# antonburger/FuncTracer

Hardware: AMD Instinct MI355X
Metric: Mrays/s (primary+shadow+reflect) at 1920x1080x16spp; frame ms (higher is better)
Workload: dtype f64

## Files before the change

functracer_amd/__init__.py:

```python
import ctypes as C
import os

import numpy as np

from . import _capi
from ._capi import (CIRCLE, CONE, CUBE, CYLINDER, EXCLUDE, INTERSECT, PLANE, SOLID_CYLINDER, SPHERE, SQUARE, SUBTRACT, UNION,
                    FtError, SceneBuilder, make_camera)

__all__ = ["Context", "PinnedArray", "ParsedScene", "parse_scene", "parse_scene_file", "jitter_pattern", "quantise_rgba8", "write_png",
           "parse_colour", "parse_ply", "FtError", "make_camera", "HIP_LIB", "HOST_LIB", "DEFAULT_SEED"]

HIP_LIB = os.environ.get("FT_HIP_LIB") or os.path.join(_capi.LIB_DIR, "libfunctracer_hip.so")
HOST_LIB = os.environ.get("FT_HOST_LIB") or os.path.join(_capi.LIB_DIR, "libfunctracer_host.so")
DEFAULT_SEED = 20260104
MAX_DEPTH = 8

_hip = None
_host = None


def hip_lib():
    global _hip
    if _hip is None:
        lib = _capi.load_library(HIP_LIB)
# ... 534 lines not shown
                                               _capi.dptr(t), _capi.dptr(p), _capi.dptr(nr), _capi.dptr(col)))
        return hit, t, p, nr, col

    def blocked(self, origins, dirs, max_dist):
        o = _capi.as_f64(origins).reshape(-1, 3)
        d = _capi.as_f64(dirs).reshape(-1, 3)
        m = _capi.as_f64(max_dist).reshape(-1)
        out = np.zeros(o.shape[0], dtype=np.int32)
        self._check(self._lib.ft_debug_blocked(self._ctx, _capi.dptr(o), _capi.dptr(d), _capi.dptr(m), o.shape[0], out.ctypes.data_as(_capi.c_int32_p)))
        return out

    def colour_for_ray(self, origins, dirs, max_depth=MAX_DEPTH):
        o = _capi.as_f64(origins).reshape(-1, 3)
        d = _capi.as_f64(dirs).reshape(-1, 3)
        rgb = np.zeros((o.shape[0], 3))
        self._check(self._lib.ft_debug_colour(self._ctx, _capi.dptr(o), _capi.dptr(d), o.shape[0], max_depth, _capi.dptr(rgb)))
        return rgb

    def devices(self):
        out = (C.c_int32 * 64)()
        n = self._check(self._lib.ft_debug_devices(self._ctx, out, 64))
        return list(out[:n])

    def commit_times(self):
        ms = np.zeros(4)
        self._check(self._lib.ft_get_commit_times(self._ctx, _capi.dptr(ms)))
        return {"flatten_ms": float(ms[0]), "device_bvh_ms": float(ms[1]), "upload_ms": float(ms[2]), "device_bvh_height": int(ms[3])}

    def mesh_trees(self):
        sizes = (C.c_int64 * 12)()
        self._check(self._lib.ft_debug_mesh_trees(self._ctx, sizes, *([None] * 9)))
        n = list(sizes)
        out = {"nodes": np.zeros(n[0], dtype=_capi.BSP_NODE_DTYPE), "bsp_leaves": np.zeros((n[1], 2), dtype=np.uint32), "tris": np.zeros((n[2], 9)),
               "tri_orig": np.zeros(n[3], dtype=np.uint32), "tri_src": np.zeros(n[4], dtype=np.uint32), "wide": np.zeros((n[5], 28)),
               "coarse_boxes": np.zeros((n[6], 6), dtype=np.float32), "meshes": np.zeros((n[7], 6), dtype=np.int32)}
        jobs = np.zeros((n[8], 9), dtype=np.uint32)
        order = ["nodes", "bsp_leaves", "tris", "tri_orig", "tri_src", "wide", "coarse_boxes", "meshes"]
        self._check(self._lib.ft_debug_mesh_trees(self._ctx, sizes, *[out[k].ctypes.data for k in order], jobs.ctypes.data))
        out["jobs"] = [dict(zip(_capi.BVH_JOB_FIELDS, (int(v) for v in row))) for row in jobs]
        out["stack_capacity"], out["from_device"] = int(sizes[9]), bool(sizes[10])
        return out

    def block_lists(self):
        sizes = (C.c_int64 * 4)()
        plane = np.zeros(4)
        fn = self._lib.ft_debug_block_lists
        fn.argtypes = [C.c_void_p, C.POINTER(C.c_int64), C.c_void_p, C.c_void_p, C.c_void_p, C.c_void_p]
        self._check(fn(self._ctx, sizes, None, None, None, None))
        heads, pos_block = np.zeros(sizes[0], dtype=np.uint32), np.zeros(sizes[0], dtype=np.uint32)
        entries = np.zeros(sizes[1], dtype=_capi.LIST_ENTRY_DTYPE)
        self._check(fn(self._ctx, sizes, plane.ctypes.data, heads.ctypes.data, pos_block.ctypes.data, entries.ctypes.data))
        return {"leaf": int(sizes[2]), "heads": heads, "pos_block": pos_block, "entries": entries, "plane": plane, "capacity": int(sizes[3])}

    def classify_reuse(self):
        out = (C.c_int64 * 4)()
        self._check(self._lib.ft_debug_classify_reuse(self._ctx, out))
        return dict(zip(_capi.CLASSIFY_REUSE_FIELDS, (int(v) for v in out)))

    def primary_kernels(self):
        out = (C.c_int64 * 2)()
        self._check(self._lib.ft_debug_primary_kernels(self._ctx, out))
        return {"k_primary": int(out[0]), "k_primary_mesh": int(out[1])}

    def scene_info(self):
        out = (C.c_int64 * 12)()
        self._check(self._lib.ft_debug_scene_info(self._ctx, out))
        keys = ["leaves", "program_words", "meshes", "bsp_nodes", "bsp_leaves", "triangles", "csg_capacity", "stack_capacity", "items", "bounded_items",
                "unbounded", "face_directions"]
        return dict(zip(keys, list(out)))


def rays_handled_by(kernel, st):
    generated = st["rays_primary"] - st["rays_primary_culled"]
    if kernel == "primary":
        return generated + st["rays_shadow_primary"]
    return st["rays_reflect"] + st["rays_shadow"] - st["rays_shadow_primary"]


def debug_slice(p0, n, tri):
    above, below = np.zeros(18), np.zeros(18)
    na, nb = C.c_int32(), C.c_int32()
    tri = _capi.as_f64(tri, (9,))
    rc = hip_lib().ft_debug_slice(_capi.dptr(_capi.as_f64(p0)), _capi.dptr(_capi.as_f64(n)), _capi.dptr(tri), _capi.dptr(above), C.byref(na),
                                  _capi.dptr(below), C.byref(nb))
    if rc < 0:
        raise FtError(rc, "slice")
    return above[:9 * na.value].reshape(-1, 3, 3), below[:9 * nb.value].reshape(-1, 3, 3)
```

functracer_amd/_capi.py:

```python
import ctypes as C
import os

import numpy as np

_HERE = os.path.dirname(os.path.abspath(__file__))
LIB_DIR = os.path.join(_HERE, "lib")

FT_OK = 0
STATUS_NAMES = {0: "FT_OK", -1: "FT_ERR_INVALID", -2: "FT_ERR_NO_DEVICE", -3: "FT_ERR_HIP", -4: "FT_ERR_UNSUPPORTED",
                -5: "FT_ERR_STATE", -6: "FT_ERR_OVERFLOW", -7: "FT_ERR_BUILD"}

CIRCLE, SQUARE, CUBE, SPHERE, PLANE, CONE, SOLID_CYLINDER, CYLINDER = range(8)
UNION, INTERSECT, SUBTRACT, EXCLUDE = range(4)
TRANSLATE, SCALE, ROTATE = range(3)

c_double_p = C.POINTER(C.c_double)
c_int32_p = C.POINTER(C.c_int32)


class FtError(RuntimeError):
    def __init__(self, status, message=""):
        self.status = status
        super().__init__(f"{STATUS_NAMES.get(status, status)}: {message}")

# ... 80 lines not shown
    ("ft_sg_set_transform", C.c_int32, [C.c_void_p, C.c_int32, C.POINTER(ft_transform), C.c_int32]),
    ("ft_scene_commit_moved", C.c_int32, [C.c_void_p]),
    ("ft_debug_leaf_matrices", C.c_int32, [C.c_void_p, C.POINTER(C.c_int64), c_double_p, c_double_p]),
]


DEFORM_SIGNATURES = [
    ("ft_sg_set_mesh_triangles", C.c_int32, [C.c_void_p, C.c_int32, c_double_p, C.c_int64]),
    ("ft_scene_commit_deformed", C.c_int32, [C.c_void_p]),
    ("ft_scene_tree_quality", C.c_int32, [C.c_void_p, C.c_int32, c_double_p]),
]


LIGHT_SIGNATURES = [
    ("ft_scene_set_directional", C.c_int32, [C.c_void_p, C.c_int32, c_double_p, c_double_p]),
    ("ft_scene_set_soft_directional", C.c_int32, [C.c_void_p, C.c_int32, c_double_p, C.c_double, c_double_p]),
    ("ft_scene_set_positional", C.c_int32, [C.c_void_p, C.c_int32, c_double_p, c_double_p, c_double_p]),
    ("ft_scene_commit_lights", C.c_int32, [C.c_void_p]),
]


MESH_TREES_SIGNATURE = [C.c_void_p, C.POINTER(C.c_int64)] + [C.c_void_p] * 9
BSP_NODE_DTYPE = np.dtype([("bmin", np.float64, 3), ("bmax", np.float64, 3), ("left", np.int32), ("right", np.int32), ("axis", np.uint32), ("pad", np.uint32)])
BVH_JOB_FIELDS = ["mesh", "first_global", "n", "node_base", "leaf_base", "tri_base", "wide_base", "coarse_first", "coarse_count"]


class ft_temporal_filter_params(C.Structure):
    _fields_ = [("iterations", C.c_int32), ("demodulate", C.c_int32), ("min_history", C.c_int32), ("to_frame", C.c_int32),
                ("sigma_colour", C.c_double), ("sigma_normal", C.c_double), ("sigma_position", C.c_double),
                ("albedo_floor", C.c_double), ("variance_floor", C.c_double)]


TEMPORAL_FILTER_DEFAULTS = dict(iterations=4, demodulate=1, min_history=4, to_frame=0, sigma_colour=2.0, sigma_normal=0.3, sigma_position=0.0,
                                albedo_floor=1e-3, variance_floor=1e-6)

TEMPORAL_FILTER_SIGNATURE = [C.c_void_p, C.POINTER(ft_camera), C.c_int32, c_double_p, C.c_int32, C.c_uint64, C.POINTER(ft_temporal_filter_params),
                             C.c_int32, C.c_void_p, c_double_p, C.POINTER(ft_stats)]

TEMPORAL_QUEUE_DEPTH = 4
TEMPORAL_QUEUE_SIGNATURES = [
    ("ft_temporal_enqueue", C.c_int32, [C.c_void_p, C.POINTER(ft_camera), C.c_int32, c_double_p, C.c_int32, C.c_uint64, C.POINTER(ft_temporal_params),
                                        C.POINTER(ft_temporal_filter_params), C.c_int32, C.c_void_p]),
    ("ft_temporal_wait", C.c_int32, [C.c_void_p, C.POINTER(ft_stats)]),
]


AOV_CHANNELS = [("t", np.float64, 1, np.inf), ("p", np.float64, 3, 0.0), ("n", np.float64, 3, 0.0), ("colour", np.float64, 3, 0.0),
                ("material", np.float64, 3, 0.0), ("leaf", np.int32, 1, -1), ("node", np.int32, 1, -1), ("triangle", np.int32, 1, -1)]


CLASSIFY_REUSE_FIELDS = ("classified", "reused", "windows_launched", "windows_skipped")
LIST_ENTRY_DTYPE = np.dtype([("tri", np.uint32), ("orig", np.uint32), ("x0", np.float32), ("x1", np.float32), ("y0", np.float32), ("y1", np.float32)])
LIST_NONE = 0xFFFFFFFF


class fth_options(C.Structure):
    _fields_ = [("camera", ft_camera), ("res_h", C.c_int32), ("res_v", C.c_int32), ("samples", C.c_int32), ("corner", C.c_int32)]


BUILDER_SIGNATURES = [
    ("sg_primitive", C.c_int32, [C.c_void_p, C.c_int32]),
    ("sg_triangle", C.c_int32, [C.c_void_p, c_double_p]),
    ("sg_bsp_mesh", C.c_int32, [C.c_void_p, C.c_int32, c_double_p, C.c_int64]),
    ("sg_transform", C.c_int32, [C.c_void_p, C.POINTER(ft_transform), C.c_int32, C.c_int32]),
    ("sg_material", C.c_int32, [C.c_void_p, C.POINTER(ft_material), C.c_int32]),
    ("sg_hue_shift", C.c_int32, [C.c_void_p, C.c_double, C.c_int32]),
    ("sg_ignore_light", C.c_int32, [C.c_void_p, C.c_int32]),
    ("sg_group", C.c_int32, [C.c_void_p, c_int32_p, C.c_int32]),
    ("sg_csg", C.c_int32, [C.c_void_p, C.c_int32, C.c_int32, C.c_int32]),
    ("sg_texture_grid", C.c_int32, [C.c_void_p, c_double_p, c_double_p, c_double_p, C.c_int32, C.c_int32]),
    ("sg_texture_image", C.c_int32, [C.c_void_p, C.POINTER(C.c_uint8), C.c_int32, C.c_int32, c_double_p, C.c_int32, C.c_int32]),
    ("scene_clear", C.c_int32, [C.c_void_p]),
    ("scene_set_objects", C.c_int32, [C.c_void_p, C.c_int32]),
    ("scene_add_directional", C.c_int32, [C.c_void_p, c_double_p, c_double_p]),
    ("scene_add_soft_directional", C.c_int32, [C.c_void_p, c_double_p, C.c_int32, C.c_double, c_double_p]),
    ("scene_add_positional", C.c_int32, [C.c_void_p, c_double_p, c_double_p, c_double_p]),
    ("scene_commit", C.c_int32, [C.c_void_p]),
]


PROGRESSIVE_SIGNATURES = [
    ("ft_progressive_begin", C.c_int32, [C.c_void_p, C.POINTER(ft_camera), C.c_int32, C.c_int32, C.c_int32, C.POINTER(ft_rect), C.c_int32,
                                         C.c_double, C.c_int32]),
    ("ft_progressive_pass", C.c_int32, [C.c_void_p, C.c_int32, c_double_p, C.c_uint64, C.c_int32, C.c_void_p, C.POINTER(ft_stats)]),
    ("ft_progressive_fetch", C.c_int32, [C.c_void_p, c_double_p, c_double_p, C.POINTER(C.c_uint32)]),
    ("ft_progressive_status", C.c_int32, [C.c_void_p, C.POINTER(C.c_int64)]),
    ("ft_progressive_end", C.c_int32, [C.c_void_p]),
]


class fth_builder(C.Structure):
    _fields_ = [(name, C.CFUNCTYPE(res, *args)) for name, res, args in BUILDER_SIGNATURES]


def dptr(a):
    return a.ctypes.data_as(c_double_p)


def as_f64(a, shape=None):
    a = np.ascontiguousarray(a, dtype=np.float64)
    if shape is not None:
        a = a.reshape(shape)
    return a


def vec3(v):
# ... 155 lines not shown
```

functracer_amd/csrc/ft_capi.cpp:

```cpp
#include "ft_context.h"
#include "ft_refit_cost.h"

namespace ftc {

bool need_device(ft_context* c) {
    if (!c) return false;
    if (c->host_only) { c->err = "host-only context: no HIP device bound (there is no CPU fallback for rendering)"; return false; }
    return true;
}

bool need_committed(ft_context* c) {
    if (!c->committed) c->err = "scene not committed (ft_scene_commit)";
    return c->committed;
}

static void norm3(double v[3]) {
    double l = std::sqrt(v[0] * v[0] + v[1] * v[1] + v[2] * v[2]);
    if (!(l < 0.0000001)) { double s = 1.0 / l; v[0] = s * v[0]; v[1] = s * v[1]; v[2] = s * v[2]; }
}
ftk::Camera make_camera(const ft_camera& cam, int res_h, int res_v) {
    ftk::Camera out{};
    double k[3] = {cam.look_at[0] - cam.o[0], cam.look_at[1] - cam.o[1], cam.look_at[2] - cam.o[2]};
    norm3(k);
    const double* u = cam.up;
// ... 98 lines not shown
    if (!c) return;
    for (DeviceWorker* w : c->workers) { w->stop(); delete w; }
    c->workers.clear();
    for (ft_context* p : c->peers) ft_destroy(p);
    c->peers.clear();
    if (!c->host_only) {
        (void)hipSetDevice(c->device);
        (void)drain_frame_streams(c);
        if (c->side) (void)hipStreamSynchronize(c->side);
        for (DeviceBuf& b : c->d_scene) b.release();
        for (DeviceBuf& b : c->d_rays) b.release();
        for (DeviceBuf& b : c->d_acc) b.release();
        for (DeviceBuf* b : {&c->d_out, &c->d_out8, &c->d_out_index, &c->d_pixels, &c->d_jitter, &c->d_wave_counts, &c->d_dbg_in, &c->d_dbg_out}) b->release();
        for (auto& f : c->slots) f.release();
        c->prog.release(); c->aov.release(); c->denoise.release(); c->temporal.release(); c->refit.release(); c->lightspace.release();
        if (c->classified) (void)hipEventDestroy(c->classified);
        for (hipEvent_t& e : c->acc_free) if (e) { (void)hipEventDestroy(e); e = nullptr; }
        if (c->side) (void)hipStreamDestroy(c->side);
        if (c->tail) (void)hipStreamDestroy(c->tail);
        for (hipStream_t m : c->more_mains) if (m) (void)hipStreamDestroy(m);
        if (c->stream) (void)hipStreamDestroy(c->stream);
    }
    delete c;
}

const char* ft_last_error(const ft_context* c) { return c ? c->err.c_str() : "null context"; }

enum { kFlag = 1, kPowerOfTwo = 2, kCommit = 4, kLevelHint = 8, kZeroFill = 16, kOrZero = 32, kClassified = 64 };
struct OptionSpec {
    const char* key;
    int64_t lo, hi;
    int64_t Options::* field;
    void (*to_graph)(fth::SceneGraph&, int64_t);
    int rules;
};
constexpr int64_t kNoLimit = std::numeric_limits<int64_t>::max();
const OptionSpec kOptions[] = {
    {"chunk_samples", 64, kNoLimit, &Options::chunk_samples, nullptr, 0},
    {"wave_samples", 0, 16, &Options::wave_samples, nullptr, kPowerOfTwo},
    {"coherent_waves", 0, 1, &Options::coherent_waves, nullptr, kFlag},
    {"timing", 0, 2, &Options::timing, nullptr, 0},
    {"classify_pixels", 0, 1, &Options::classify_pixels, nullptr, kFlag | kClassified},
    {"follow_below", -1, kNoLimit, &Options::follow_below, nullptr, kLevelHint},
    {"level_hint", 0, 1, &Options::level_hint, nullptr, kFlag},
    {"classify_ahead", 0, 1, &Options::classify_ahead, nullptr, kFlag},
    {"resolve_aside", 0, 1, &Options::resolve_aside, nullptr, kFlag},
    {"zero_fill_skip", 0, 1, &Options::zero_fill_skip, nullptr, kFlag | kZeroFill},
    {"classify_reuse", 0, 1, &Options::classify_reuse, nullptr, kFlag | kClassified},
    {"mains", 1, ft_context::kMains, &Options::mains, nullptr, 0},
    {"bvh_builder", 0, 3, &Options::bvh_builder, nullptr, kCommit},
    {"csg_auto_grow", 0, 1, &Options::csg_auto_grow, nullptr, kFlag},
    {"primary_block_lists", 0, 1, &Options::primary_block_lists, nullptr, kFlag | kClassified},
    {"uniform_surface", 0, 1, &Options::uniform_surface, nullptr, kFlag},
    {"primary_mesh_kernel", 0, 1, &Options::primary_mesh_kernel, nullptr, kFlag},
    {"temporal_follow_deformed", 0, 1, &Options::temporal_follow_deformed, nullptr, kFlag},
    {"refit_rebuild_percent", 100, 1000000, &Options::refit_rebuild_percent, nullptr, kOrZero},
    {"csg_mesh_capacity", 1, 255, nullptr, [](fth::SceneGraph& g, int64_t v) { g.csg_mesh_capacity = (int32_t)v; }, kCommit},
    {"light_space_shadows", std::numeric_limits<int64_t>::min(), kNoLimit, nullptr,
     [](fth::SceneGraph& g, int64_t v) { g.light_space_shadows = v == 0 || v == 1 ? (int32_t)v : 2; }, kCommit},
    {"mesh_unclipped_bvh", 0, 1, nullptr, [](fth::SceneGraph& g, int64_t v) { g.mesh_unclipped_bvh = v != 0; }, kFlag | kCommit},
};

int32_t ft_set_option(ft_context* c, const char* key, int64_t value) {
    if (!c || !key) return FT_ERR_INVALID;
    for (const OptionSpec& o : kOptions) {
        if (std::strcmp(key, o.key)) continue;
        if (o.rules & kFlag) value = value != 0;
        else if (!((o.rules & kOrZero) && value == 0) && (value < o.lo || value > o.hi || ((o.rules & kPowerOfTwo) && (value & (value - 1))))) return FT_ERR_INVALID;
        if (o.to_graph) { o.to_graph(c->graph, value); c->committed = false; c->options_pending = true; return FT_OK; }
        for (ft_context* d : devices(c)) {
            d->opt.*o.field = value;
            for (hipStream_t m : d->more_mains) if (!m) d->opt.mains = 1;
            d->dev_scene.coherent_waves = d->opt.coherent_waves ? 1 : 0;
            d->dev_scene.uniform_surface = d->opt.uniform_surface ? 1 : 0;
            if (!d->opt.temporal_follow_deformed) temporal_drop_snapshots(d);
            if (o.rules & kCommit) { d->committed = false; c->options_pending = true; }
            if (o.rules & kLevelHint) d->staged_hint = -1;
            if (o.rules & kZeroFill) d->zero_signature[0] = d->zero_signature[1] = 0;
            if (o.rules & kClassified) for (auto& F : d->slots) { F.kept.valid = false; F.keeps = false; }
        }
        return FT_OK;
    }
    c->err = std::string("unknown option: ") + key;
    return FT_ERR_INVALID;
}

static ft_node add_node(ft_context* c, fth::GraphNode&& n) { c->graph.nodes.push_back(std::move(n)); c->committed = false; c->restructured = true; return (ft_node)c->graph.nodes.size() - 1; }

ft_node ft_sg_primitive(ft_context* c, int32_t kind) {
    if (!c || kind < 0 || kind > FT_PRIM_CYLINDER) return FT_ERR_INVALID;
    fth::GraphNode n; n.kind = fth::GraphNode::Prim; n.prim = kind; return add_node(c, std::move(n));
}
ft_node ft_sg_triangle(ft_context* c, const double v[9]) {
    if (!c || !v) return FT_ERR_INVALID;
    fth::GraphNode n; n.kind = fth::GraphNode::TriangleP; std::memcpy(n.tri, v, sizeof n.tri); return add_node(c, std::move(n));
}
ft_node ft_sg_bsp_mesh(ft_context* c, int32_t depth, const double* tris, int64_t n_tris) {
    if (!c || n_tris < 0 || (n_tris > 0 && !tris) || depth < 0) return FT_ERR_INVALID;
    fth::GraphNode n; n.kind = fth::GraphNode::Mesh; n.depth = depth; n.tris.assign(tris, tris + 9 * n_tris); return add_node(c, std::move(n));
}
ft_node ft_sg_transform(ft_context* c, const ft_transform* ts, int32_t n_ts, ft_node child) {
    if (!c || !c->graph.valid(child) || !ts || n_ts < 1) return FT_ERR_INVALID;
    fth::GraphNode n; n.kind = fth::GraphNode::Transform;
    for (int i = 0; i < n_ts; ++i) { if (ts[i].kind < FT_TRANSLATE || ts[i].kind > FT_ROTATE) return FT_ERR_INVALID; n.xf.push_back(ts[i]); }
    n.children = {child};
    return add_node(c, std::move(n));
}
int32_t ft_sg_set_transform(ft_context* c, ft_node node, const ft_transform* ts, int32_t n_ts) {
    if (!c) return FT_ERR_INVALID;
    if (!c->graph.valid(node) || c->graph.nodes[node].kind != fth::GraphNode::Transform) { c->err = "ft_sg_set_transform: not a transform node"; return FT_ERR_INVALID; }
    if (!ts || n_ts < 1) { c->err = "ft_sg_set_transform: no transforms"; return FT_ERR_INVALID; }
    for (int i = 0; i < n_ts; ++i) if (ts[i].kind < FT_TRANSLATE || ts[i].kind > FT_ROTATE) { c->err = "ft_sg_set_transform: bad transform kind"; return FT_ERR_INVALID; }
    c->graph.nodes[node].xf.assign(ts, ts + n_ts);
    c->committed = false; c->moved_pending = true;
    return FT_OK;
}
int32_t ft_sg_set_mesh_triangles(ft_context* c, ft_node node, const double* tris, int64_t n_tris) {
    if (!c) return FT_ERR_INVALID;
    if (!c->graph.valid(node) || c->graph.nodes[node].kind != fth::GraphNode::Mesh) { c->err = "ft_sg_set_mesh_triangles: not a bspMesh node"; return FT_ERR_INVALID; }
    if (!tris) { c->err = "ft_sg_set_mesh_triangles: no triangles"; return FT_ERR_INVALID; }
    fth::GraphNode& n = c->graph.nodes[node];
    if (n_tris < 0 || (uint64_t)n_tris != n.tris.size() / 9) { c->err = "ft_sg_set_mesh_triangles: the triangle count differs from the node's"; return FT_ERR_INVALID; }
    n.tris.assign(tris, tris + 9 * n_tris);
    n.deformed = true;
    c->committed = false;
    return FT_OK;
}
// ... 116 lines not shown
        float lf = (float)len; while ((double)lf < len) lf = std::nextafter(lf, std::numeric_limits<float>::infinity());
        v.push_back((float)f.cull_rows[k]); v.push_back((float)f.cull_rows[k + 1]); v.push_back((float)f.cull_rows[k + 2]); v.push_back(lf);
    }
}

static ftk::LbvhTarget lbvh_target(ft_context* c, const fth::FlatScene::BvhJob& j) {
    const DeviceBuf* B = c->d_scene;
    return ftk::LbvhTarget{B[kTris].as<double>(), j.first_global, j.n, B[kNodes].as<ftd::BspNode>(), j.node_base, B[kBspLeaves].as<ftd::BspLeaf>(), j.leaf_base,
                           B[kTriOrig].as<uint32_t>(), j.tri_base, B[kWide].as<double>(), j.wide_base, B[kCoarse].as<float>() + 6 * (size_t)j.coarse_first, j.coarse_count,
                           B[kTriSrc].as<uint32_t>()};
}

static int32_t fit_stacks(ft_context* c, uint32_t height) {
    if ((int32_t)height + 1 > c->flat.stack_capacity) c->flat.stack_capacity = (int32_t)height + 1;
    return lds_fits(c);
}

static bool mesh_kernel_scene(const fth::FlatScene& f, int variant) {
    if (variant != 4 || f.item_pc.size() != 2 || f.leaves.size() != 1 || f.any_reflective) return false;
    size_t pc = f.item_pc[0] & 0x7FFFFFFFu;
    if (pc < f.program.size() && (f.program[pc] & 0xFFu) == ftd::OP_CULL) pc += 2;
    if (pc + 1 >= f.program.size() || f.program[pc] != (uint32_t)ftd::OP_LEAF_FOLD || (f.program[pc + 1] & 0xFFu) != ftd::OP_END) return false;
    const ftd::Leaf& L = f.leaves[0];
    if (L.kind != ftd::LK_MESH || !(L.flags & ftd::LF_LIT) || L.mesh >= f.meshes.size() || f.meshes[L.mesh].bvh_root < 0) return false;
    for (auto& l : f.lights) if (l.kind != ftd::LT_DIRECTIONAL) return false;
    for (auto& m : f.materials) if (m.reflectance > 0.0) return false;
    return true;
}

static void derive_launch_shape(ft_context* c) {
    const fth::FlatScene& f = c->flat;
    ftk::DevScene& S = c->dev_scene;
    S.coherent_waves = c->opt.coherent_waves ? 1 : 0;
    S.uniform_surface = c->opt.uniform_surface ? 1 : 0;
    S.n_simd = c->n_cu * 4;
    S.n_items = (int32_t)f.item_pc.size() - 1; S.n_cull_rows = f.cull_bundle ? (int32_t)(f.cull_rows.size() / 3) : -1;
    S.n_leaves = (int32_t)f.leaves.size(); S.n_lights = (int32_t)f.lights.size();
    S.csg_cap = f.csg_capacity; S.stack_cap = f.stack_capacity;
    S.lane_fold = lane_fold_for(f); S.csg_rows = (f.csg_capacity + S.lane_fold - 1) / S.lane_fold;
    S.shadow_rays_per_hit = 0;
    for (auto& l : f.lights) S.shadow_rays_per_hit += (l.kind == ftd::LT_SOFT) ? l.samples : 1;
    c->variant = 0;
    for (auto& m : f.materials) if (needs_fancy(m)) c->variant |= 1;
    for (auto& l : f.lights) if (l.kind == ftd::LT_SOFT) c->variant |= 2;
    if (!f.meshes.empty()) c->variant |= 4;
    const size_t lds = lds_bytes_for(c->flat);
    c->variant_primary = c->variant;
    c->blocks_primary = ftk::occupancy_blocks_primary(lds, &c->variant_primary);
    c->blocks_bounce = ftk::occupancy_blocks_bounce(lds, c->variant);
    c->blocks_resolve = ftk::occupancy_blocks_resolve();
    c->blocks_aov = ftk::occupancy_blocks_aov(lds, c->variant);
    c->mesh_kernel_scene = mesh_kernel_scene(f, c->variant);
    c->blocks_primary_mesh = ftk::occupancy_blocks_primary_mesh();
}

static int32_t upload_scene(ft_context* c) {
    int32_t rc;
    FT_HIP(c, hipSetDevice(c->device));
    if (any_queued(c)) { if ((rc = retire_queued(c)) != FT_OK) return rc; c->accum_open = false; }
    const fth::FlatScene& f = c->flat;
    if ((rc = lds_fits(c)) != FT_OK) return rc;
    c->refit.ready = false;
    c->lightspace.reset();
    ftk::DevScene& S = c->dev_scene;
    rc = FT_OK;
    auto put = [&](SceneArray k, const auto& v, auto*& ptr) {
        if (rc == FT_OK) rc = upload(c, c->d_scene[k], v);
        ptr = static_cast<std::remove_reference_t<decltype(ptr)>>(c->d_scene[k].p);
    };
    put(kLeaves, f.leaves, S.leaves); put(kM2w, f.m2w, S.m2w); put(kMaterials, f.materials, S.materials); put(kLights, f.lights, S.lights);
    put(kTextures, f.textures, S.textures); put(kTexPixels, f.tex_pixels, S.tex_pixels); put(kProgram, f.program, S.program);
    put(kMeshes, f.meshes, S.meshes); put(kNodes, f.nodes, S.nodes); put(kBspLeaves, f.bsp_leaves, S.bsp_leaves); put(kTris, f.tris, S.tris);
    put(kCulls, f.culls, S.culls);
    cull_items_image(f, c->cull_items_and_rows);
    put(kCullItems, c->cull_items_and_rows, S.cull_items);
    put(kCullRows, f.cull_rows, S.cull_rows); put(kItemPc, f.item_pc, S.item_pc); put(kWide, f.wide, S.wide); put(kMeshWide, f.mesh_wide, S.mesh_wide);
    put(kCoarse, f.coarse_boxes, S.coarse_boxes); put(kTriOrig, f.tri_orig, S.tri_orig);
    put(kLsPairs, f.ls_pairs, S.ls_pairs); put(kLsNodes, f.ls_nodes, S.ls_nodes); put(kLsTris, f.ls_tris, S.ls_tris);
    if (rc == FT_OK) rc = upload(c, c->d_scene[kTriSrc], f.tri_src);
    if (rc == FT_OK) rc = upload(c, c->d_scene[kRunNodes], f.run_nodes);
    if (rc != FT_OK) return rc;
    for (auto& F : c->slots) { if ((rc = ensure(c, F.d_fc, sizeof(ftk::SlotCounters))) != FT_OK) return rc; F.fc_clean = false; }
    c->zero_signature[0] = c->zero_signature[1] = 0;
    FT_HIP(c, hipStreamSynchronize(c->stream));
    {
        const auto t0 = std::chrono::steady_clock::now();
        uint32_t tallest = 0;
        for (const fth::FlatScene::BvhJob& j : f.bvh_jobs) {
            uint32_t height = 0;
            FT_HIP(c, ftk::build_lbvh(c->stream, lbvh_target(c, j), &height, c->opt.bvh_builder == 1 ? 0 : 1));
            if (height == 0 || height > 40) { c->err = "device BVH build refused (non-finite vertex or a tree deeper than 40 levels): the host builder takes over"; return FT_ERR_BUILD; }
            tallest = std::max(tallest, height);
        }
        if (!f.bvh_jobs.empty()) {
            c->commit_ms[1] = std::chrono::duration<double, std::milli>(std::chrono::steady_clock::now() - t0).count();
            c->commit_ms[3] = tallest;
            if ((rc = fit_stacks(c, tallest)) != FT_OK) return rc;
        }
    }
    derive_launch_shape(c);
    c->committed = true;
    ++c->commit_serial; c->staged_hint = -1;
    return FT_OK;
}

int32_t commit_scene(ft_context* c) {
    using clock = std::chrono::steady_clock;
    auto ms_since = [](clock::time_point t0) { return std::chrono::duration<double, std::milli>(clock::now() - t0).count(); };
    for (double& v : c->commit_ms) v = 0.0;
    const bool held = c->holds_commit;
    const auto done = [c](int32_t rc) {
        if (rc == FT_OK) { c->holds_commit = true; c->restructured = false; c->moved_pending = false; c->options_pending = false; c->lights_pending = false; for (fth::GraphNode& n : c->graph.nodes) n.deformed = false; }
        return rc;
    };
    for (int attempt = 0; attempt < 2; ++attempt) {
        c->graph.device_bvh = !c->host_only && c->opt.bvh_builder >= 1 && attempt == 0;
        c->graph.device_bvh_min_tris = c->opt.bvh_builder == 2 ? kDeviceBvhMinTris : 0;
        auto t0 = clock::now();
        fth::FlatScene fresh;
        int32_t rc = c->graph.flatten(fresh, c->err);
        if (rc == FT_OK && !c->host_only && lane_fold_for(fresh) == 0) { rc = FT_ERR_UNSUPPORTED; c->err = kLdsRefusal; }
        c->commit_ms[0] += ms_since(t0);
        if (rc != FT_OK) {
            if (attempt == 0 && held) for (ft_context* d : devices(c)) d->committed = true;
            return rc;
        }
        c->holds_commit = false;
        c->tree_quality.clear();
        c->flat = std::move(fresh);
        if (c->host_only) { c->committed = true; return done(FT_OK); }
        t0 = clock::now();
        rc = upload_scene(c);
        for (ft_context* p : c->peers) {
            if (rc != FT_OK) break;
            p->flat = c->flat;
            if ((rc = upload_scene(p)) != FT_OK) c->err = p->err;
            c->commit_ms[1] += p->commit_ms[1];
        }
        c->commit_ms[2] += ms_since(t0) - c->commit_ms[1];
        if (rc == FT_ERR_BUILD && c->graph.device_bvh) continue;
        return done(rc);
    }
    return FT_ERR_BUILD;
}

struct DeformedMesh { uint32_t mesh; int32_t node; fth::MeshScan scan; };

using ftk::refit::refit_ranges;

static bool refittable(const fth::FlatScene& f, uint32_t mesh) { return f.meshes[mesh].root < 0 && f.meshes[mesh].bvh_root != INT32_MIN; }
static const fth::FlatScene::BvhJob* job_of(const fth::FlatScene& f, uint32_t mesh) {
    for (const fth::FlatScene::BvhJob& j : f.bvh_jobs) if (j.mesh == mesh) return &j;
// ... 330 lines not shown
        for (const LightJob& j : jobs) {
            if (!j.grid) continue;
            const size_t own = 4 * (size_t)j.nu * j.nv + 5 * (size_t)j.entries;
            words = std::max(words, (size_t)j.at + (own + ftd::kLsNodeWords - 1) / ftd::kLsNodeWords * ftd::kLsNodeWords);
            doubles = std::max(doubles, 9 * ((size_t)j.tri_at + j.entries));
        }
        if (words == T.base_node_words && doubles == T.base_tri_doubles && words == L.node_words && doubles == L.tri_doubles) regrid = false;
    }
    if (regrid) {
        DeviceBuf nodes, tris;
        if ((rc = ensure(c, nodes, words * 4)) != FT_OK || (rc = ensure(c, tris, doubles * 8)) != FT_OK) { nodes.release(); tris.release(); return rc; }
        const auto fail = [&](int32_t code) { nodes.release(); tris.release(); return code; };
        if (hipMemcpyAsync(nodes.p, B[kLsNodes].p, T.base_node_words * 4, hipMemcpyDeviceToDevice, c->stream) != hipSuccess ||
            hipMemcpyAsync(tris.p, B[kLsTris].p, T.base_tri_doubles * 8, hipMemcpyDeviceToDevice, c->stream) != hipSuccess ||
            (words > T.base_node_words && hipMemsetAsync(nodes.as<uint32_t>() + T.base_node_words, 0, (words - T.base_node_words) * 4, c->stream) != hipSuccess) ||
            (doubles > T.base_tri_doubles && hipMemsetAsync(tris.as<double>() + T.base_tri_doubles, 0, (doubles - T.base_tri_doubles) * 8, c->stream) != hipSuccess)) {
            c->err = "ft_scene_commit_lights: copying the light-space arrays failed"; return fail(FT_ERR_HIP);
        }
        for (const LightJob& j : jobs) {
            if (!j.grid) continue;
            const uint32_t n = j.pair->n_tris, cells = j.nu * j.nv;
            const double* mesh = B[kTris].as<double>() + 9 * (size_t)j.pair->first_tri;
            size_t scan_bytes = 0;
            if (ftk::ls_grid_scan(c->stream, nullptr, nullptr, cells, nullptr, &scan_bytes) != hipSuccess) { c->err = "ft_scene_commit_lights: sizing the scan failed"; return fail(FT_ERR_HIP); }
            DeviceBuf& ebox = L.d_ebox[j.slot];
            DeviceBuf& counts = L.d_counts[j.slot];
            if ((rc = ensure(c, ebox, (size_t)n * 20)) != FT_OK || (rc = ensure(c, counts, (size_t)cells * 4)) != FT_OK || (rc = ensure(c, L.d_first, (size_t)cells * 4)) != FT_OK ||
                (rc = ensure(c, L.d_cursor, (size_t)cells * 4)) != FT_OK || (rc = ensure(c, L.d_idx, (size_t)j.entries * 4)) != FT_OK || (rc = ensure(c, L.d_scan, scan_bytes)) != FT_OK) return fail(rc);
            if (hipMemsetAsync(L.d_cursor.p, 0, (size_t)cells * 4, c->stream) != hipSuccess) { c->err = "ft_scene_commit_lights: hipMemsetAsync failed"; return fail(FT_ERR_HIP); }
            if (!lead) {
                if (hipMemsetAsync(counts.p, 0, (size_t)cells * 4, c->stream) != hipSuccess) { c->err = "ft_scene_commit_lights: hipMemsetAsync failed"; return fail(FT_ERR_HIP); }
                ftk::ls_grid_entries(c->stream, mesh, n, j.frame, ebox.as<float>(), nullptr);
                ftk::ls_grid_cell_counts(c->stream, ebox.as<float>(), n, j.s, j.nu, j.nv, counts.as<uint32_t>(), nullptr);
            }
            if (ftk::ls_grid_scan(c->stream, counts.as<uint32_t>(), L.d_first.as<uint32_t>(), cells, L.d_scan.p, &scan_bytes) != hipSuccess) { c->err = "ft_scene_commit_lights: the scan failed"; return fail(FT_ERR_HIP); }
            ftk::ls_grid_emit(c->stream, ebox.as<float>(), mesh, n, j.s, j.nu, j.nv, counts.as<uint32_t>(), L.d_first.as<uint32_t>(), L.d_cursor.as<uint32_t>(), L.d_idx.as<uint32_t>(),
                              j.entries, nodes.as<uint32_t>(), j.at, tris.as<double>(), j.tri_at);
        }
        if (hipGetLastError() != hipSuccess || hipStreamSynchronize(c->stream) != hipSuccess) { c->err = "ft_scene_commit_lights: the grid kernels failed"; return fail(FT_ERR_HIP); }
        B[kLsNodes].release(); B[kLsTris].release();
        B[kLsNodes] = nodes; B[kLsTris] = tris;
        ftk::DevScene& S = c->dev_scene;
        S.ls_nodes = static_cast<std::remove_reference_t<decltype(S.ls_nodes)>>(nodes.p);
        S.ls_tris = static_cast<std::remove_reference_t<decltype(S.ls_tris)>>(tris.p);
        L.node_words = words; L.tri_doubles = doubles;
        L.rewritten = true;
    }
    FT_HIP(c, hipStreamSynchronize(c->stream));
    ms[1] += since(t1);
    const auto t2 = clock::now();
    if ((rc = upload(c, B[kLsPairs], f.ls_pairs)) != FT_OK) return rc;
    FT_HIP(c, hipStreamSynchronize(c->stream));
    ms[0] += since(t2);
    c->zero_signature[0] = c->zero_signature[1] = 0;
    c->committed = true;
    ++c->commit_serial; c->staged_hint = -1;
    return FT_OK;
}

}

extern "C" {

int32_t ft_scene_commit(ft_context* c) {
    if (!c) return FT_ERR_INVALID;
    progressive_close(c);
    temporal_close(c);
    return commit_scene(c);
}

int32_t ft_scene_commit_moved(ft_context* c) {
    if (!c) return FT_ERR_INVALID;
    if (!c->holds_commit) { c->err = "ft_scene_commit_moved: no committed scene to move (ft_scene_commit)"; return FT_ERR_STATE; }
    if (c->restructured) { c->err = "ft_scene_commit_moved: the graph, the root or the lights changed since the commit (ft_scene_commit)"; return FT_ERR_STATE; }
    progressive_close(c);
    const int32_t rc = commit_scene(c);
    if (rc == FT_OK) ++c->pose_serial;
    return rc;
}

int32_t ft_scene_commit_deformed(ft_context* c) {
    if (!c) return FT_ERR_INVALID;
    if (!c->holds_commit) { c->err = "ft_scene_commit_deformed: no committed scene to deform (ft_scene_commit)"; return FT_ERR_STATE; }
    if (c->restructured) { c->err = "ft_scene_commit_deformed: the graph, the root or the lights changed since the commit (ft_scene_commit)"; return FT_ERR_STATE; }
    if (c->moved_pending) { c->err = "ft_scene_commit_deformed: an ft_sg_set_transform is pending (ft_scene_commit_moved first)"; return FT_ERR_STATE; }
    if (c->options_pending) { c->err = "ft_scene_commit_deformed: a commit-time option changed since the commit (ft_scene_commit)"; return FT_ERR_STATE; }
    if (c->lights_pending) { c->err = "ft_scene_commit_deformed: a light setter is pending (ft_scene_commit_lights first)"; return FT_ERR_STATE; }
    using clock = std::chrono::steady_clock;
    const auto t0 = clock::now();
    fth::FlatScene& f = c->flat;
    std::vector<DeformedMesh> edits;
    for (uint32_t m = 0; m < (uint32_t)f.meshes.size(); ++m) {
        const int32_t id = f.mesh_node[m];
        if (id < 0 || !c->graph.valid(id) || !c->graph.nodes[(size_t)id].deformed) continue;
        const fth::GraphNode& n = c->graph.nodes[(size_t)id];
        const bool refuse_depth = n.depth > 0 && !c->graph.mesh_unclipped_bvh;
        const fth::MeshScan scan = refuse_depth ? fth::MeshScan{} : fth::scan_mesh(n.tris.data(), (int64_t)(n.tris.size() / 9));
        if (refuse_depth || !scan.finite || f.meshes[m].root >= 0) {
            c->err = refuse_depth || f.meshes[m].root >= 0 ? "ft_scene_commit_deformed: an edited mesh has depth above 0 - its clipped BSP depends on the positions (ft_scene_commit)"
                                                            : "ft_scene_commit_deformed: an edited mesh holds a non-finite coordinate (ft_scene_commit)";
            c->committed = true;
            return FT_ERR_UNSUPPORTED;
        }
        edits.push_back(DeformedMesh{m, id, scan});
    }
    if (c->host_only) {
// ... 225 lines not shown
```

functracer_amd/csrc/ft_context.h:

```cpp
#pragma once
#include <hip/hip_runtime.h>

#include <chrono>
#include <condition_variable>
#include <mutex>
#include <cmath>
#include <cstddef>
#include <cstdio>
#include <cstring>
#include <functional>
#include <limits>
#include <string>
#include <thread>
#include <type_traits>
#include <vector>

#include "../../include/functracer_hip.h"
#include "ft_device.h"
#include "ft_scene.h"

struct DeviceBuf {
    void* p = nullptr; size_t bytes = 0;
    template <class T> T* as() const { return reinterpret_cast<T*>(p); }
    void release() { if (p) (void)hipFree(p); p = nullptr; bytes = 0; }
// ... 8 lines not shown
};

enum { kStageOther = 0, kStageClosest = 1, kStageShade = 2, kStageResolve = 3, kStagePrimary = 4, kStages = 5 };
static_assert(sizeof(ftk::FrameCounters) % 16 == 0 && offsetof(ftk::RenderCounters, ref_equiv) == 32, "the hand-over at the end of a frame copies words and clears 16 bytes at a time");

struct DeviceWorker {
    std::thread th;
    std::mutex m;
    std::condition_variable cv;
    std::function<void()> job;
    bool has_job = false, done = true, quit = false;
    void start() {
        th = std::thread([this] {
            std::unique_lock<std::mutex> lk(m);
            for (;;) {
                cv.wait(lk, [this] { return has_job || quit; });
                if (quit) return;
                std::function<void()> fn = std::move(job);
                has_job = false;
                lk.unlock();
                fn();
                lk.lock();
                done = true;
                cv.notify_all();
            }
        });
    }
    void post(std::function<void()> fn) { std::lock_guard<std::mutex> lk(m); job = std::move(fn); has_job = true; done = false; cv.notify_all(); }
    void wait() { std::unique_lock<std::mutex> lk(m); cv.wait(lk, [this] { return done; }); }
    void stop() { { std::lock_guard<std::mutex> lk(m); quit = true; cv.notify_all(); } if (th.joinable()) th.join(); }
};

constexpr int64_t kDeviceBvhMinTris = 4096;

struct Options {
    int64_t chunk_samples = 16ll << 20;
    int64_t wave_samples = 0;
    int64_t coherent_waves = 1;
    int64_t timing = 1;
    int64_t classify_pixels = 1;
    int64_t follow_below = -1;
    int64_t level_hint = 1;
    int64_t classify_ahead = 1;
    int64_t resolve_aside = 1;
    int64_t zero_fill_skip = 1;
    int64_t classify_reuse = 1;
    int64_t mains = 2;
    int64_t bvh_builder = 2;
    int64_t csg_auto_grow = 1;
    int64_t primary_block_lists = 1;
    int64_t refit_rebuild_percent = 0;
    int64_t temporal_follow_deformed = 0;
    int64_t primary_mesh_kernel = 1;
    int64_t uniform_surface = 1;
};

enum SceneArray { kLeaves, kM2w, kMaterials, kLights, kTextures, kTexPixels, kProgram, kMeshes, kNodes, kBspLeaves, kTris, kCulls, kCullItems,
                  kCullRows, kItemPc, kWide, kMeshWide, kCoarse, kTriOrig, kLsPairs, kLsNodes, kLsTris,
                  kTriSrc, kRunNodes,
                  kSceneArrays };

struct Brackets {
    std::vector<hipEvent_t> events; size_t used = 0;
    struct Span { hipEvent_t a, b; int kind; };
    std::vector<Span> spans;
    hipStream_t ms = nullptr;
    int timing = 1;
    hipEvent_t ev0 = nullptr, ev1 = nullptr;
    hipEvent_t boundary = nullptr;
    bool fresh = false;
    void begin(hipStream_t s, int t) { used = 0; spans.clear(); ms = s; timing = t; ev0 = ev1 = boundary = nullptr; fresh = false; }
    hipEvent_t next() {
        if (used == events.size()) { hipEvent_t e; if (hipEventCreate(&e) != hipSuccess) return nullptr; events.push_back(e); }
        return events[used++];
    }
    hipEvent_t record(hipStream_t s) { hipEvent_t e = next(); if (e) (void)hipEventRecord(e, s); return e; }
    void open() { if (ev0) return; ev0 = record(ms); boundary = ev0; fresh = true; }
    template <class Fn> void timed(int kind, Fn&& fn) {
        const bool bracket = timing >= 2 || (timing == 1 && (kind == kStageClosest || kind == kStageShade || kind == kStagePrimary));
        open();
        if (bracket && !fresh) boundary = record(ms);
        fn();
        if (!bracket) { fresh = false; return; }
        hipEvent_t b = record(ms);
        if (boundary && b) spans.push_back(Span{boundary, b, kind});
        boundary = b; fresh = true;
    }
    void release() { for (hipEvent_t e : events) (void)hipEventDestroy(e); events.clear(); used = 0; }
};

struct ClassifyKey {
    uint64_t commit_serial = 0;
    int32_t res_h = 0, res_v = 0, list_leaf = -1;
    double jitter_extent = 0.0;
    ftk::Camera cam{};
    std::vector<ft_rect> rects;
    bool operator==(const ClassifyKey& o) const {
        return commit_serial == o.commit_serial && res_h == o.res_h && res_v == o.res_v && list_leaf == o.list_leaf &&
               std::memcmp(&jitter_extent, &o.jitter_extent, sizeof jitter_extent) == 0 && std::memcmp(&cam, &o.cam, sizeof cam) == 0 &&
               rects.size() == o.rects.size() && (rects.empty() || std::memcmp(rects.data(), o.rects.data(), rects.size() * sizeof(ft_rect)) == 0);
    }
};

struct ft_context {
    static constexpr int kMains = 3;
    static constexpr int kAcc = kMains;
    static constexpr int kSlots = kMains + 1;
    std::vector<ft_context*> peers;
    std::vector<DeviceWorker*> workers;
    bool host_only = false;
    int device = -1;
    int n_cu = 0;
    hipStream_t stream = nullptr;
    hipStream_t more_mains[kMains - 1] = {};
    std::string err;
    Options opt;

    fth::SceneGraph graph;
    fth::FlatScene flat;
    std::vector<float> cull_items_and_rows;
    bool committed = false;
    bool holds_commit = false, restructured = false;
    bool moved_pending = false, options_pending = false;
    bool lights_pending = false;
    uint64_t pose_serial = 0;
    double commit_ms[4] = {0, 0, 0, 0};

    DeviceBuf d_scene[kSceneArrays];
    hipStream_t side = nullptr;
    int variant = 0, variant_primary = 0, blocks_primary = 1, blocks_bounce = 1, blocks_resolve = 2, blocks_aov = 1;
    bool mesh_kernel_scene = false;
    int blocks_primary_mesh = 1;
    hipEvent_t classified = nullptr;
    ftk::DevScene dev_scene{};
    DeviceBuf d_rays[2 * kMains], d_acc[kAcc], d_out, d_out8, d_out_index, d_pixels, d_jitter, d_wave_counts, d_dbg_in, d_dbg_out;
    struct Aov {
        DeviceBuf d_pixels, d_jitter, d_out, d_ctr;
        bool ctr_clean = false;
        TimedLaunch timer;
        void release() { for (DeviceBuf* b : {&d_pixels, &d_jitter, &d_out, &d_ctr}) b->release(); timer.release(); }
    } aov;
    struct Denoise {
        DeviceBuf d_guides, d_u[2], d_out8;
        TimedLaunch timer;
        void release() { for (DeviceBuf* b : {&d_guides, &d_u[0], &d_u[1], &d_out8}) b->release(); timer.release(); }
    } denoise;
    int acc_turn = 0;
    hipStream_t tail = nullptr;
    hipEvent_t acc_free[kAcc] = {};
    bool acc_busy[kAcc] = {};
    uint64_t zero_signature[2] = {0, 0};
    uint32_t classify_epoch = 0;
    int64_t ray_capacity = 0, acc_capacity = 0;
    struct FrameSlot {
        DeviceBuf d_block_pos, d_pos_block, d_fc;
        DeviceBuf d_list_heads, d_list_pool;
        int32_t list_leaf = -1;
        ftk::Camera list_cam{};
        struct Classified { bool valid = false; ClassifyKey key; int64_t n_active = 0; uint64_t culled = 0; } kept;
        bool keeps = false, reuses = false;
        bool fc_clean = false;
        Brackets ev;
        bool simple = false;
        int main_ix = 0;
        ftk::FrameReport* h_report = nullptr;
        ftk::FrameReport* d_report = nullptr;
        uint64_t signature = 0;
        bool pending = false;
        uint64_t rays_primary = 0; int64_t n_pix_total = 0; int32_t spp = 0, n_launches = 0, n_chunks = 0, format = 0; bool classify = false;
        std::chrono::steady_clock::time_point wall0;
        void release() {
            d_block_pos.release(); d_pos_block.release(); d_fc.release(); d_list_heads.release(); d_list_pool.release();
            if (h_report) (void)hipHostFree(h_report);
            h_report = nullptr; d_report = nullptr;
            ev.release();
        }
    };
    FrameSlot slots[kSlots];
    struct Refit {
        DeviceBuf d_verts, d_parent_node, d_parent_leaf, d_arrived, d_leaf_boxes, d_wide_node;
        DeviceBuf d_cost;
        bool ready = false;
        void release() { for (DeviceBuf* b : {&d_verts, &d_parent_node, &d_parent_leaf, &d_arrived, &d_leaf_boxes, &d_wide_node, &d_cost}) b->release(); ready = false; }
    } refit;
    struct LightSpace {
        struct Pair {
            uint32_t rec, leaf, light; int32_t root; double c[3], R; uint32_t first_tri, n_tris; double v0[3], rec0[ftd::kLsPairDoubles];
            std::vector<std::pair<uint32_t, uint32_t>> levels;
        };
        std::vector<Pair> pairs;
        std::vector<uint32_t> order;
        size_t base_node_words = 0, base_tri_doubles = 0;
        bool ready = false;
        DeviceBuf d_order, d_first, d_cursor, d_idx, d_small, d_scan;
        std::vector<DeviceBuf> d_ebox, d_counts;
        size_t node_words = 0, tri_doubles = 0;
        bool order_uploaded = false, rewritten = false;
        void reset() { pairs.clear(); order.clear(); ready = order_uploaded = rewritten = false; node_words = tri_doubles = base_node_words = base_tri_doubles = 0; }
        void release() {
            for (DeviceBuf* b : {&d_order, &d_first, &d_cursor, &d_idx, &d_small, &d_scan}) b->release();
            for (DeviceBuf& b : d_ebox) b.release();
            for (DeviceBuf& b : d_counts) b.release();
            d_ebox.clear(); d_counts.clear(); reset();
        }
    } lightspace;
    struct TreeQuality { double cost_built = 0.0; bool known = false; uint32_t rebuilds = 0; };
    std::vector<TreeQuality> tree_quality;
    int slot_turn = 0;
    int64_t reuse_counts[4] = {0, 0, 0, 0};
    int64_t primary_launches[2] = {0, 0};
    int last_classified_slot = -1;
    int staged_hint = -1;
    uint64_t staged_signature = 0;
    int ray_sets = 0;
    uint64_t commit_serial = 0;
    bool accum_open = false;
    std::vector<uint32_t> pixels;
    std::vector<double> jitter_on_device;
    std::vector<ft_rect> pixel_rects;
    bool pixels_corner = false, pixels_tiled = false;
    int last_format = 0;
    int64_t last_n_pix = 0;
    int32_t last_res_h = 0, last_res_v = 0;
    double k_ms[kStages] = {0, 0, 0, 0, 0};
    int32_t k_launches[kStages] = {0, 0, 0, 0, 0};
    int64_t last_active_pix = 0;
    struct Progressive {
        bool open = false;
        ft_camera cam{};
        int32_t res_h = 0, res_v = 0, max_depth = 0, min_samples = 0;
        double tolerance = 0.0;
        std::vector<ft_rect> tiles;
        int64_t n_pix = 0, n_blocks = 0, passes = 0, samples = 0, traced = 0;
        DeviceBuf d_sum[2], d_sq[2], d_blk[2];
        int cur = 0;
        void release() { for (int k = 0; k < 2; ++k) { d_sum[k].release(); d_sq[k].release(); d_blk[k].release(); } *this = Progressive(); }
    } prog;
    struct Temporal {
        bool open = false;
        int32_t res_h = 0, res_v = 0;
        std::vector<ft_rect> rects;
        int64_t n_pix = 0, calls = 0, with_history = 0, at_max = 0;
        ftk::Camera cam{};
        DeviceBuf d_set[2], d_rgb, d_rgba8, d_ctr;
        TimedLaunch timer;
        int prev = 0;
        uint64_t pose = 0;
        std::vector<double> h_m2w, h_w2m;
        DeviceBuf d_motion;
        struct Snapshot { uint32_t mesh, first, n; };
        std::vector<Snapshot> snaps;
        size_t snap_used = 0;
        DeviceBuf d_snap, d_deform;
// ... 127 lines not shown
```

functracer_amd/csrc/ft_debug.cpp:

```cpp
#include "ft_context.h"
using namespace ftc;

extern "C" {

static int32_t debug_rays_in(ft_context* c, const double* origins, const double* dirs, const double* max_dist, int64_t n, size_t out_bytes) {
    if (!need_device(c)) return FT_ERR_NO_DEVICE;
    if (!c->committed) { c->err = "scene not committed"; return FT_ERR_STATE; }
    if (n == 0) return FT_OK;
    FT_HIP(c, hipSetDevice(c->device));
    int32_t rc;
    const size_t N = (size_t)n;
    if ((rc = ensure(c, c->d_dbg_in, N * (max_dist ? 56 : 48))) != FT_OK) return rc;
    if ((rc = ensure(c, c->d_dbg_out, N * out_bytes)) != FT_OK) return rc;
    double* din = c->d_dbg_in.as<double>();
    FT_HIP(c, hipMemcpyAsync(din, origins, N * 24, hipMemcpyHostToDevice, c->stream));
    FT_HIP(c, hipMemcpyAsync(din + 3 * N, dirs, N * 24, hipMemcpyHostToDevice, c->stream));
    if (max_dist) FT_HIP(c, hipMemcpyAsync(din + 6 * N, max_dist, N * 8, hipMemcpyHostToDevice, c->stream));
    c->slots[0].fc_clean = false;
    FT_HIP(c, hipMemsetAsync(c->slots[0].d_fc.p, 0, sizeof(unsigned long long), c->stream));
    return FT_OK;
}
static int32_t debug_rays_done(ft_context* c) {
    unsigned long long n_overflow = 0;
    FT_HIP(c, hipMemcpyAsync(&n_overflow, c->slots[0].d_fc.p, sizeof n_overflow, hipMemcpyDeviceToHost, c->stream));
// ... 161 lines not shown
        if (rc != FT_OK) return rc;
    }
    auto get = [&](void* dst, SceneArray k, const void* host, size_t bytes) -> int32_t {
        if (!dst || bytes == 0) return FT_OK;
        if (c->host_only) { std::memcpy(dst, host, bytes); return FT_OK; }
        if (c->d_scene[k].bytes < bytes) { c->err = "ft_debug_mesh_trees: a scene array in device memory is smaller than the flattened one"; return FT_ERR_STATE; }
        FT_HIP(c, hipMemcpy(dst, c->d_scene[k].p, bytes, hipMemcpyDeviceToHost));
        return FT_OK;
    };
    int32_t rc;
    if ((rc = get(nodes, kNodes, f.nodes.data(), f.nodes.size() * sizeof(ftd::BspNode))) != FT_OK) return rc;
    if ((rc = get(bsp_leaves, kBspLeaves, f.bsp_leaves.data(), f.bsp_leaves.size() * sizeof(ftd::BspLeaf))) != FT_OK) return rc;
    if ((rc = get(tris, kTris, f.tris.data(), f.tris.size() * sizeof(double))) != FT_OK) return rc;
    if ((rc = get(tri_orig, kTriOrig, f.tri_orig.data(), f.tri_orig.size() * sizeof(uint32_t))) != FT_OK) return rc;
    if ((rc = get(tri_src, kTriSrc, f.tri_src.data(), f.tri_src.size() * sizeof(uint32_t))) != FT_OK) return rc;
    if ((rc = get(wide, kWide, f.wide.data(), f.wide.size() * sizeof(double))) != FT_OK) return rc;
    if ((rc = get(coarse_boxes, kCoarse, f.coarse_boxes.data(), f.coarse_boxes.size() * sizeof(float))) != FT_OK) return rc;
    if (meshes) for (size_t m = 0; m < f.meshes.size(); ++m) {
        int32_t* r = meshes + 6 * m;
        r[0] = f.meshes[m].root; r[1] = f.meshes[m].bvh_root; r[2] = (int32_t)f.meshes[m].n_source_tris; r[3] = f.mesh_wide[m];
        r[4] = (int32_t)f.mesh_coarse[2 * m]; r[5] = (int32_t)f.mesh_coarse[2 * m + 1];
    }
    static_assert(sizeof(fth::FlatScene::BvhJob) == 9 * sizeof(uint32_t), "a job goes out as nine words");
    if (jobs && !f.bvh_jobs.empty()) std::memcpy(jobs, f.bvh_jobs.data(), f.bvh_jobs.size() * sizeof(fth::FlatScene::BvhJob));
    return FT_OK;
}

int32_t ft_debug_block_lists(ft_context* c, int64_t sizes[4], double plane[4], uint32_t* heads, uint32_t* pos_block, uint32_t* entries) {
    if (!c || !sizes) return FT_ERR_INVALID;
    if (c->host_only) return FT_ERR_NO_DEVICE;
    sizes[0] = sizes[1] = sizes[3] = 0; sizes[2] = -1;
    if (c->last_classified_slot < 0) return FT_OK;
    FT_HIP(c, hipSetDevice(c->device));
    int32_t rc = retire_queued(c);
    if (rc != FT_OK) return rc;
    if ((rc = drain_frame_streams(c)) != FT_OK) return rc;
    const ft_context::FrameSlot& F = c->slots[c->last_classified_slot];
    if (F.list_leaf < 0 || !F.h_report) return FT_OK;
    const size_t n_active = std::min<size_t>(F.h_report->n_pix_active / 64u, F.d_list_heads.bytes / 4);
    std::vector<uint32_t> h(n_active);
    if (n_active) FT_HIP(c, hipMemcpy(h.data(), F.d_list_heads.p, n_active * 4, hipMemcpyDeviceToHost));
    size_t used = 0;
    for (uint32_t v : h) if (v != ftk::kListNone) used = std::max<size_t>(used, (size_t)(v >> 7) + (v & 127u));
    const size_t cap = F.d_list_pool.bytes / (ftk::kListEntryWords * 4);
    if (used > cap) { c->err = "ft_debug_block_lists: a header points past the pool"; return FT_ERR_STATE; }
    sizes[0] = (int64_t)n_active; sizes[1] = (int64_t)used; sizes[2] = F.list_leaf; sizes[3] = (int64_t)cap;
    if (plane) { plane[0] = F.list_cam.tlx; plane[1] = F.list_cam.tly; plane[2] = F.list_cam.pw; plane[3] = F.list_cam.ph; }
    if (heads && n_active) std::memcpy(heads, h.data(), n_active * 4);
    if (pos_block && n_active) FT_HIP(c, hipMemcpy(pos_block, F.d_pos_block.p, n_active * 4, hipMemcpyDeviceToHost));
    if (entries && used) FT_HIP(c, hipMemcpy(entries, F.d_list_pool.p, used * ftk::kListEntryWords * 4, hipMemcpyDeviceToHost));
    return FT_OK;
}

int32_t ft_debug_classify_reuse(ft_context* c, int64_t out[4]) {
    if (!c || !out) return FT_ERR_INVALID;
    if (c->host_only) return FT_ERR_NO_DEVICE;
    for (int k = 0; k < 4; ++k) out[k] = 0;
    for (const ft_context* d : devices(c)) for (int k = 0; k < 4; ++k) out[k] += d->reuse_counts[k];
    return FT_OK;
}

int32_t ft_debug_primary_kernels(ft_context* c, int64_t out[2]) {
    if (!c || !out) return FT_ERR_INVALID;
    if (c->host_only) return FT_ERR_NO_DEVICE;
    out[0] = out[1] = 0;
    for (const ft_context* d : devices(c)) for (int k = 0; k < 2; ++k) out[k] += d->primary_launches[k];
    return FT_OK;
}

int32_t ft_debug_slice(const double p0[3], const double n[3], const double tri[9], double above[18], int32_t* n_above, double below[18], int32_t* n_below) {
    if (!p0 || !n || !tri || !above || !below || !n_above || !n_below) return FT_ERR_INVALID;
    std::vector<double> a, b; std::string err;
    int32_t rc = fth::slice_triangle(p0, n, tri, a, b, err);
    if (rc != FT_OK) return rc;
    *n_above = (int32_t)(a.size() / 9); *n_below = (int32_t)(b.size() / 9);
    if (!a.empty()) std::memcpy(above, a.data(), a.size() * 8);
    if (!b.empty()) std::memcpy(below, b.data(), b.size() * 8);
    return FT_OK;
}

int32_t ft_debug_devices(ft_context* c, int32_t* ordinals, int32_t capacity) {
    if (!c || capacity < 0 || (capacity > 0 && !ordinals)) return FT_ERR_INVALID;
    if (c->host_only) return 0;
    int32_t n = 0;
    if (n < capacity) ordinals[n] = c->device;
    ++n;
    for (ft_context* p : c->peers) { if (n < capacity) ordinals[n] = p->device; ++n; }
    return n;
}

}
```

functracer_amd/csrc/ft_device.h:

```cpp
#ifndef FT_DEVICE_H
#define FT_DEVICE_H
#include <hip/hip_runtime_api.h>
#include <stdint.h>

#include "ft_flat.h"

namespace ftk {

constexpr int kBlock = 256;
constexpr int kMaxBounce = 16;
constexpr int kWorkGroups = 64;

struct DevScene {
    const double* leaves;
    const double* m2w;
    const ftd::Material* materials;
    const ftd::Light* lights;
    const ftd::Texture* textures;
    const uint32_t* program;
    const ftd::Mesh* meshes;
    const ftd::BspNode* nodes;
    const ftd::BspLeaf* bsp_leaves;
    const double* tris;
    const double* culls;
    const uint32_t* tri_orig;
    const double* wide;
    const int32_t* mesh_wide;
    const double* ls_pairs;
    const uint32_t* ls_nodes;
    const double* ls_tris;
    const uint8_t* tex_pixels;
    const float* cull_items;
    const float* coarse_boxes;
    const uint32_t* item_pc;
    const double* cull_rows;
    int32_t n_leaves, n_lights, csg_cap, stack_cap;
    int32_t shadow_rays_per_hit;
    int32_t n_items, n_cull_rows;
    int32_t csg_rows, lane_fold;
    int32_t n_simd;
    int32_t coherent_waves;
    int32_t uniform_surface;
};

struct RayBuf { double *ox, *oy, *oz, *dx, *dy, *dz, *w; uint32_t* slot; };
constexpr uint64_t kRayRecBytes = 60;
constexpr uint64_t kPixelIdBytes = 4, kAccBytes = 24;

struct PixCount { uint32_t n_pix, pad[3]; };
struct ChunkCounters {
    uint32_t n_rays[kMaxBounce + 2];
    uint32_t pad[14];
    uint32_t work_trace[kMaxBounce + 2][kWorkGroups * 16];
};
struct RenderCounters {
    unsigned long long rays_shadow, rays_reflect, hits_primary, csg_overflow;
    double ref_equiv;
    unsigned long long hits_total;
    unsigned long long unused[3];
    unsigned long long pixels_culled;
    unsigned long long rays_shadow_primary, rays_reflect_primary;
    unsigned long long pad[4];
};
constexpr int kStatStripes = 64;
struct FrameCounters {
    ChunkCounters cc;
    RenderCounters stats[kStatStripes];
    uint32_t classify_ticket;
    uint32_t classify_error;
    uint32_t report_ticket;
    uint32_t list_cursor;
    uint32_t report_stripe[64];
};
struct SlotCounters { FrameCounters fc; PixCount kept; };
struct FrameReport {
    RenderCounters total;
    uint32_t n_rays[kMaxBounce + 2];
    uint32_t n_pix_active;
    uint32_t classify_error;
    uint32_t pad[12];
};
static_assert(sizeof(FrameReport) == 256, "FrameReport is written as 64 words");

struct Camera {
    double o[3], k[3], i[3], j[3];
    double pw, ph, tlx, tly;
    double focal_length, tan_half_aperture;
    int32_t res_h, res_v;
    int32_t has_focus, pad;
};

struct Launch {
    hipStream_t stream;
    int grid;
    size_t lds_bytes;
    int variant;
};

struct Primary {
    Camera cam;
    const uint32_t* pixel_ids;
    const double* jitter;
    uint32_t pix_base, n_pix;
    int32_t spp;
    uint32_t stride;
    unsigned long long seed;
    double inv_n_pix, inv_stride;
    const PixCount* counts;
    const uint32_t* block_map;
    int32_t group_log2;
    const uint32_t* list_heads; const uint32_t* list_pool; int32_t list_leaf;
};
void launch_primary(const Launch& L, const DevScene& S, const Primary& gen, RayBuf next, double* acc, uint32_t acc_stride, int max_depth, FrameCounters* fc);
int occupancy_blocks_primary(size_t lds_bytes, int* variant);
constexpr int kVariantMeshKernel = 16;
int occupancy_blocks_primary_mesh();
void launch_bounce(const Launch& L, const DevScene& S, const Primary& gen, RayBuf rays, RayBuf next, double* acc, uint32_t acc_stride, int bounce, int max_depth, bool follow, FrameCounters* fc);
int occupancy_blocks_bounce(size_t lds_bytes, int variant);
struct ClassifyOut { int32_t* block_pos; uint32_t* pos_block; uint32_t* wave_counts; PixCount* kept; };
constexpr int32_t kBlockRetired = -2;
void launch_classify(const Launch& L, const DevScene& S, const Primary& gen_list, const ClassifyOut& out, double jitter_extent, uint32_t epoch, FrameCounters* fc,
                     const uint32_t* retired = nullptr, bool mask_only = false);
constexpr uint32_t kListNone = 0xFFFFFFFFu, kListCap = 64, kListEntryWords = 6;
struct BlockLists { uint32_t* heads; uint32_t* pool; uint32_t pool_entries; int32_t leaf; };
void launch_block_lists(const Launch& L, const DevScene& S, const Primary& gen_list, const uint32_t* pos_block, const BlockLists& out, double jitter_extent, FrameCounters* fc, const PixCount* counts);
struct ResolveArgs {
    const double* acc; uint32_t acc_stride; const PixCount* counts; uint32_t first, n_pix_host; int32_t spp;
    const uint32_t* pos_block;
    const int32_t* block_pos;
    uint32_t n_blocks_total;
    const uint32_t* pixel_ids;
    double* out_rgb; uint8_t* out_rgba;
    uint32_t group_log2;
    FrameCounters* fc; FrameReport* report;
};
void launch_resolve(const Launch& L, const ResolveArgs& a);
int occupancy_blocks_resolve();
struct ProgressiveArgs {
    const double* sum_in; double* sum_out;
    const double* sq_in; double* sq_out;
    const uint32_t* blk_in; uint32_t* blk_out;
    uint32_t n_list, min_samples;
    double tolerance;
};
constexpr uint32_t kRetired = 0x80000000u;
void launch_resolve_progressive(const Launch& L, const ResolveArgs& a, const ProgressiveArgs& pa);
void launch_report(const Launch& L, FrameCounters* fc, FrameReport* report);
void launch_resolve_corner(const Launch& L, const double* acc, uint32_t acc_stride, uint32_t w, uint32_t h, const uint32_t* out_index, double* out_rgb, uint8_t* out_rgba);
struct LbvhTarget {
    double* tris; uint32_t first_global, n;
    ftd::BspNode* nodes; uint32_t node_base;
    ftd::BspLeaf* leaves; uint32_t leaf_base;
    uint32_t* tri_orig; uint32_t tri_base;
    double* wide; uint32_t wide_base;
    float* coarse; uint32_t coarse_count;
    uint32_t* tri_src;
};
hipError_t build_lbvh(hipStream_t stream, const LbvhTarget& t, uint32_t* height, int kind = 1);

struct RefitArrays {
    double* tris; ftd::BspNode* nodes; const ftd::BspLeaf* leaves; const uint32_t* tri_orig; double* wide; float* coarse;
    const int32_t* wide_node; int32_t* parent_node; int32_t* parent_leaf; uint32_t* arrived; double* leaf_boxes;
};
struct RefitMesh {
    uint32_t first_global, n;
    uint32_t node_first, node_count, leaf_first, leaf_count, tri_first, tri_count, wide_first, wide_count;
    int32_t bvh_root;
    uint32_t device_built;
    uint32_t coarse_first, coarse_count;
    double pad;
};
void refit_parents(hipStream_t stream, const RefitArrays& A, const RefitMesh& m);
void refit_mesh(hipStream_t stream, const RefitArrays& A, const RefitMesh& m, const double* verts);
inline uint32_t refit_cost_blocks(const RefitMesh& m) { return (m.node_count + 255u) / 256u; }
void refit_cost(hipStream_t stream, const RefitArrays& A, const RefitMesh& m, double* partials, double* cost);

struct LsFrame { double U[3], V[3], D[3], c[3], pad; };
void ls_refit_level(hipStream_t stream, uint32_t* ls_nodes, uint32_t n_nodes, const double* ls_tris, uint32_t n_tris, const uint32_t* order, uint32_t count, const LsFrame& F);
struct LsGridCandidates { int n; float s[8]; uint32_t nu[8], nv[8]; };
void ls_grid_entries(hipStream_t stream, const double* tris, uint32_t n, const LsFrame& F, float* ebox, uint32_t* ruv);
void ls_grid_count(hipStream_t stream, const float* ebox, uint32_t n, const LsGridCandidates& C, unsigned long long* sums);
void ls_grid_cell_counts(hipStream_t stream, const float* ebox, uint32_t n, float s, uint32_t nu, uint32_t nv, uint32_t* counts, uint32_t* max_count);
hipError_t ls_grid_scan(hipStream_t stream, const uint32_t* counts, uint32_t* first, uint32_t n_cells, void* tmp, size_t* tmp_bytes);
void ls_grid_emit(hipStream_t stream, const float* ebox, const double* tris, uint32_t n, float s, uint32_t nu, uint32_t nv, const uint32_t* counts, const uint32_t* first,
                  uint32_t* cursor, uint32_t* idx, uint32_t n_entries, uint32_t* ls_nodes, uint32_t at, double* ls_tris, uint32_t tri_at);

struct AovOut {
    double *t, *p, *n, *colour, *material;
    int32_t *leaf, *node, *triangle;
    uint32_t stride;
};
struct AovSource { const uint32_t* tri_src; const int32_t* run_nodes; };
void launch_aov(const Launch& L, const DevScene& S, const Primary& gen, uint32_t sample, const AovSource& src, const AovOut& out, unsigned long long* counters);
int occupancy_blocks_aov(size_t lds_bytes, int variant);

struct GuideWindow { const int32_t* triangle; const uint32_t* pixel_ids; uint32_t first, n; const double *p_plane, *n_plane, *colour; const int32_t* leaf; uint32_t stride; };

enum : uint8_t { kDenoiseMiss = 0, kDenoiseHit = 1, kDenoiseOutside = 2 };
struct DenoiseGuides { double* n[3]; double* p[3]; double* d[3]; double* v; uint8_t* cls; };
constexpr size_t kDenoiseGuideBytes = 10 * 8 + 1;
struct DenoiseScatterArgs {
    GuideWindow win;
    const double* frame; double* u0;
    DenoiseGuides g;
    int32_t demodulate; double albedo_floor;
    const double *sum, *sq; const uint32_t* blk; uint32_t n_list; double variance_floor;
};
void launch_denoise_scatter(hipStream_t stream, const DenoiseScatterArgs& a);
struct DenoiseArgs {
    const double* u_in; double* u_out; uint8_t* out8;
    DenoiseGuides g;
    int32_t res_h, res_v, step;
    double inv_sn2, inv_sp2, inv_sc2;
};
void launch_denoise(hipStream_t stream, const DenoiseArgs& a, bool last);
void launch_denoise_quantise(hipStream_t stream, const double* rgb, uint8_t* out8, uint32_t n_px);

struct TemporalSet { double* m[3]; double* q[3]; double* len; double* p[3]; double* n[3]; int32_t* leaf; };
constexpr size_t kTemporalSetBytes = 13 * 8 + 4;
constexpr double kTemporalMinWeight = 1.0 / 16.0;
constexpr int kTemporalMotionDoubles = 24;
struct TemporalDeformLeaf { double W[12], H[12], Wh[9]; uint32_t first_live, snap_first, n, pad; };
struct TemporalBox { double* lo[3]; double* hi[3]; };
constexpr size_t kTemporalBoxBytes = 6 * 8;
constexpr int kTemporalClampMaxRadius = 3;
struct TemporalArgs {
    GuideWindow win;
    const double* frame;
    TemporalSet prev, cur;
    double o[3], i[3], j[3], k[3], tlx, tly, pw, ph;
    int32_t res_h, res_v, has_prev;
    double max_history, min_normal_dot, tol_scale;
    double* out_rgb; uint8_t* out8;
    unsigned long long* counters;
    const double* motion; uint32_t n_leaves;
    const TemporalDeformLeaf* deform; const double *tris, *snap;
    TemporalBox box; double clamped_history;
};
// ... 40 lines not shown
```

functracer_amd/csrc/ft_flat.h:

```cpp
#ifndef FT_FLAT_H
#define FT_FLAT_H
#include <stdint.h>

namespace ftd {

enum LeafKind : uint32_t {
    LK_SPHERE = 0,
    LK_PLANE = 1,
    LK_SQUARE = 2,
    LK_CIRCLE = 3,
    LK_CUBE = 4,
    LK_CONE = 5,
    LK_CYLINDER = 6,
    LK_SOLIDCYL = 7,
    LK_MESH = 8
};

enum LeafFlags : uint32_t {
    LF_FLIP = 1u,
    LF_XFORM = 2u,
    LF_LIT = 4u
};

struct Leaf {
    double w2m[12];
    uint32_t kind;
    uint32_t flags;
    uint32_t material;
    uint32_t mesh;
    uint32_t ls_pairs;
    uint32_t pad[3];

};

struct Material {
    double colour[3];
    double roughness, reflectance, shineyness;
    uint32_t apply_lighting;
    int32_t texture;
    uint32_t hue_rot;
    uint32_t pad;
};

constexpr int kMaxUvOps = 13;
struct Texture {
    double c1[3], c2[3];
    double n_ops;
    double kind;
    double pixel_base;
    double ops[kMaxUvOps][3];
};

constexpr bool small_whole_exponent(double s) { return s <= 64.0 && s == __builtin_floor(s); }

enum LightKind : uint32_t { LT_DIRECTIONAL = 0, LT_SOFT = 1, LT_POINT = 2 };
struct Light {
    double v[3];
    double falloff[3];
    double colour[3];
    double scatter;
    uint32_t kind;
    int32_t samples;
    double tan_half_scatter;
};

struct Mesh {
    int32_t root;
    uint32_t n_source_tris;
    uint32_t max_depth;
    int32_t bvh_root;
};
constexpr int kWideNodeDoubles = 28;
constexpr int kLsPairDoubles = 16;
constexpr int kLsNodeWords = 24;
constexpr uint32_t kLsMaxPairs = 64;
constexpr uint32_t kLsMaxTris = 1u << 20;
constexpr uint64_t kLsMaxBytes = 256ull << 20;
constexpr uint32_t kLsGridEntriesPerTri = 16;
constexpr uint32_t kLsGridMaxCell = 256;
constexpr uint32_t kLsGridWaveCells = 4;
struct BspNode {
    double bmin[3], bmax[3];
    int32_t left, right;
    uint32_t axis;
    uint32_t pad;
};
struct BspLeaf { uint32_t first_tri, n_tris; };

enum Op : uint32_t {
    OP_END = 0,
    OP_LEAF_FOLD = 1,
    OP_LEAF_PUSH = 2,
    OP_MARK = 3,
    OP_CSG = 4,
    OP_FOLD_LIST = 5,
    OP_CULL = 6,
    OP_SKIP_IF_EMPTY = 7,
    OP_CSG_PAIR = 8
};

struct CullRecord {
    double centre[3];
    double radius2;
    double n_rows;
    double rows[6][3];
    double pad;
};
inline uint32_t make_op(uint32_t op, uint32_t arg) { return op | (arg << 8); }

enum : uint32_t { ID_LEAF_MASK = 0x00FFFFFFu, ID_SUB_SHIFT = 24, ID_SUB_MASK = 0x7u, ID_LIT = 1u << 29, ID_FLIP = 1u << 30, ID_SIDE_B = 1u << 31, ID_MISS = 0xFFFFFFFFu };

}
#endif
```

functracer_amd/csrc/ft_frame.cpp:

```cpp
#include "ft_context.h"

namespace ftc {

ftk::RayBuf ray_view(const DeviceBuf& b, int64_t cap) {
    double* d = b.as<double>();
    ftk::RayBuf r;
    r.ox = d; r.oy = d + cap; r.oz = d + 2 * cap; r.dx = d + 3 * cap; r.dy = d + 4 * cap; r.dz = d + 5 * cap; r.w = d + 6 * cap;
    r.slot = reinterpret_cast<uint32_t*>(d + 7 * cap);
    return r;
}

int32_t ensure_frame_buffers(ft_context* c, int64_t cap, bool reflective) {
    int32_t rc;
    if (cap > c->acc_capacity) { for (int k = 0; k < ft_context::kAcc; ++k) if ((rc = ensure(c, c->d_acc[k], (size_t)cap * 24)) != FT_OK) return rc; c->acc_capacity = cap; }
    if (!reflective || (cap <= c->ray_capacity && c->ray_sets >= c->opt.mains)) return FT_OK;
    const int64_t want = std::max(cap, c->ray_capacity);
    for (int i = 0; i < 2 * c->opt.mains; ++i) if ((rc = ensure(c, c->d_rays[i], (size_t)want * (7 * 8 + 4))) != FT_OK) return rc;
    c->ray_capacity = want; c->ray_sets = (int)c->opt.mains;
    return FT_OK;
}


std::vector<std::vector<ft_rect>> band_shares(const RenderRequest& q, size_t n_devs) {
    std::vector<std::vector<ft_rect>> share(n_devs);
// ... 234 lines not shown
        p.key.commit_serial = c->commit_serial; p.key.res_h = q.res_h; p.key.res_v = q.res_v; p.key.list_leaf = p.list_leaf;
        p.key.jitter_extent = p.jitter_extent; p.key.cam = p.cam; p.key.rects = p.rects;
        p.reuse = c->opt.classify_reuse && !F.pending && F.kept.valid && F.kept.key == p.key;
    }
    if (p.reuse) {
        const int64_t n_active = std::max<int64_t>(F.kept.n_active, std::min<int64_t>(64, n_pix_total));
        int64_t per = p.pix_per_chunk;
        if (per > 64) {
            const int64_t n_chunks = (n_active + per - 1) / per;
            per = std::min(per, ((n_active + n_chunks - 1) / n_chunks + 63) / 64 * 64);
        }
        p.jobs.clear();
        for (int64_t p0 = 0; p0 < n_active; p0 += per) {
            const uint32_t n = (uint32_t)std::min<int64_t>(per, n_active - p0);
            p.jobs.push_back(FramePlan::Job{(uint32_t)p0, n, 0, 0, (uint32_t)p0, n});
        }
    }
    p.simple = defer && c->opt.resolve_aside && !p.corner && c->opt.timing < 2 && p.jobs.size() == 1;
}

static int32_t upload_frame_inputs(ft_context* c, const RenderRequest& q, const FramePlan& p, bool& queued) {
    int32_t rc;
    if ((rc = ensure_frame_buffers(c, p.cap, p.last_bounce > 0)) != FT_OK) return rc;
    DeviceBuf& ob = q.format == 1 ? c->d_out8 : c->d_out;
    const void* before = ob.p;
    if ((rc = ensure(c, ob, (size_t)q.res_h * (size_t)q.res_v * (q.format == 1 ? 4 : 24))) != FT_OK) return rc;
    if (ob.p != before) c->zero_signature[q.format] = 0;
    const bool new_jitter = p.jitter != c->jitter_on_device;
    queued = p.corner || !p.same_list || new_jitter;
    if (queued && any_pending(c) && (rc = retire_pending(c, nullptr)) != FT_OK) return rc;
    if (p.corner) {
        if ((rc = upload(c, c->d_pixels, p.corner_ids)) != FT_OK) return rc;
        if ((rc = upload(c, c->d_out_index, c->pixels)) != FT_OK) return rc;
    } else if (!p.same_list && (rc = upload(c, c->d_pixels, c->pixels)) != FT_OK) return rc;
    if (new_jitter) {
        c->jitter_on_device = p.jitter;
        if ((rc = upload(c, c->d_jitter, c->jitter_on_device)) != FT_OK) return rc;
    }
    return FT_OK;
}

static int32_t queue_classify(ft_context* c, const RenderRequest& q, const FramePlan& p, ft_context::FrameSlot& F, bool ahead) {
    const ftk::Primary all{p.cam, c->d_pixels.as<uint32_t>(), c->d_jitter.as<double>(), 0u, (uint32_t)p.n_pix_total, p.spp, (uint32_t)q.res_h,
                           (unsigned long long)q.seed, 1.0 / (double)p.n_pix_total, 1.0 / (double)q.res_h, nullptr, nullptr};
    ftk::PixCount* const kept = &F.d_fc.as<ftk::SlotCounters>()->kept;
    const ftk::ClassifyOut cls{F.d_block_pos.as<int32_t>(), F.d_pos_block.as<uint32_t>(), c->d_wave_counts.as<uint32_t>(), kept};
    const uint32_t* retired = p.progressive ? c->prog.d_blk[c->prog.cur].as<uint32_t>() : nullptr;
    auto* fc = F.d_fc.as<ftk::FrameCounters>();
    const uint32_t epoch = ++c->classify_epoch;
    const hipStream_t cs = ahead ? c->side : F.ev.ms;
    const ftk::Launch Lg{cs, c->n_cu * 8, 0, 0};
    if (!c->classified) FT_HIP(c, hipEventCreateWithFlags(&c->classified, hipEventDisableTiming));
    else FT_HIP(c, hipStreamWaitEvent(cs, c->classified, 0));
    const ftk::BlockLists lists{F.d_list_heads.as<uint32_t>(), F.d_list_pool.as<uint32_t>(), (uint32_t)(F.d_list_pool.bytes / (ftk::kListEntryWords * 4)), p.list_leaf};
    auto queue_lists = [&] { if (p.list_leaf >= 0) ftk::launch_block_lists(Lg, c->dev_scene, all, cls.pos_block, lists, p.jitter_extent, fc, kept); };
    if (ahead) {
        ftk::launch_classify(Lg, c->dev_scene, all, cls, p.jitter_extent, epoch, fc, retired, p.mask_only);
        queue_lists();
        FT_HIP(c, hipEventRecord(c->classified, c->side));
        FT_HIP(c, hipStreamWaitEvent(F.ev.ms, c->classified, 0));
    } else {
        F.ev.timed(kStageOther, [&] { ftk::launch_classify(Lg, c->dev_scene, all, cls, p.jitter_extent, epoch, fc, retired, p.mask_only); queue_lists(); });
        FT_HIP(c, hipEventRecord(c->classified, F.ev.ms));
    }
    F.ev.fresh = false;
    return FT_OK;
}

static int32_t queue_chunks(ft_context* c, const RenderRequest& q, const FramePlan& p, ft_context::FrameSlot& F, int main_ix, int32_t& n_launches) {
    Brackets& E = F.ev;
    const hipStream_t ms = E.ms;
    auto* fc = F.d_fc.as<ftk::FrameCounters>();
    const ftk::PixCount* const kept = &F.d_fc.as<ftk::SlotCounters>()->kept;
    const size_t lds = lds_bytes_for(c->flat);
    const ftk::Launch Lp{ms, c->n_cu * c->blocks_primary, lds, c->variant_primary};
    const ftk::Launch Lb{ms, c->n_cu * c->blocks_bounce, lds, c->variant};
    const ftk::Launch Lg{ms, c->n_cu * 8, 0, 0};
    const ftk::Launch Lr{ms, c->n_cu * c->blocks_resolve, 0, 0};
    const ftk::RayBuf rb[2] = {ray_view(c->d_rays[2 * main_ix], c->ray_capacity), ray_view(c->d_rays[2 * main_ix + 1], c->ray_capacity)};
    const bool zeros_in_place = p.classify && !p.progressive && c->opt.zero_fill_skip && c->zero_signature[q.format] == p.zsig;
    c->zero_signature[q.format] = p.classify && !p.progressive ? p.zsig : 0;
    double* const out_rgb = q.format == 1 ? nullptr : c->d_out.as<double>();
    uint8_t* const out_rgba = q.format == 1 ? c->d_out8.as<uint8_t>() : nullptr;
    const uint32_t stride = (uint32_t)(p.corner ? q.res_h + 1 : q.res_h);
    const bool hinted = c->opt.level_hint && c->staged_hint >= 0 && c->staged_signature == p.signature;
    const int n_levels = hinted ? std::min(p.last_bounce, c->staged_hint + 1) : p.last_bounce;
    for (const FramePlan::Job& job : p.jobs) {
        const bool first = &job == &p.jobs.front(), last = &job == &p.jobs.back();
        const uint32_t n_pix = job.n_ids, n_samples = n_pix * (uint32_t)p.spp;
        if (!first) E.timed(kStageOther, [&] { (void)hipMemsetAsync(&fc->cc, 0, sizeof(ftk::ChunkCounters), ms); });
        ftk::Primary gen{p.cam, c->d_pixels.as<uint32_t>(), c->d_jitter.as<double>(), job.id_base, n_pix, p.spp, stride, (unsigned long long)q.seed,
                         1.0 / (double)n_pix, 1.0 / (double)stride, nullptr, nullptr};
        if (p.classify) { gen.counts = kept; gen.block_map = F.d_pos_block.as<uint32_t>(); }
        if (p.list_leaf >= 0) { gen.list_heads = F.d_list_heads.as<uint32_t>(); gen.list_pool = F.d_list_pool.as<uint32_t>(); gen.list_leaf = p.list_leaf; }
        gen.group_log2 = (n_pix % 64u == 0u) ? p.group_log2 : 0;
        const int at = c->acc_turn;
        double* const acc = c->d_acc[at].as<double>();
        if (c->acc_busy[at]) { FT_HIP(c, hipStreamWaitEvent(ms, c->acc_free[at], 0)); c->acc_busy[at] = false; E.fresh = false; }
        const bool mesh_kernel = c->opt.primary_mesh_kernel && c->mesh_kernel_scene && c->opt.coherent_waves && c->opt.uniform_surface && !p.progressive && !p.corner &&
                                 gen.group_log2 > 0 && !p.cam.has_focus;
        ftk::Launch Lj = Lp;
        if (mesh_kernel) { Lj.grid = c->n_cu * c->blocks_primary_mesh; Lj.lds_bytes = 0; Lj.variant |= ftk::kVariantMeshKernel; }
        ++c->primary_launches[mesh_kernel ? 1 : 0];
        E.timed(kStagePrimary, [&] { ftk::launch_primary(Lj, c->dev_scene, gen, rb[1], acc, n_samples, q.max_depth, fc); });
        auto bounce = [&](int b) { ftk::launch_bounce(Lb, c->dev_scene, gen, rb[b & 1], rb[(b + 1) & 1], acc, n_samples, b, q.max_depth, b == n_levels && n_levels < p.last_bounce, fc); };
        if (E.timing >= 2) for (int b = 1; b <= n_levels; ++b) E.timed(kStageShade, [&] { bounce(b); });
        else if (n_levels >= 1) E.timed(kStageShade, [&] { for (int b = 1; b <= n_levels; ++b) bounce(b); });
        n_launches += 2 + n_levels;
        if (!p.simple) for (int k = 0; k < ft_context::kAcc; ++k) if (c->acc_busy[k]) {
            FT_HIP(c, hipStreamWaitEvent(ms, c->acc_free[k], 0)); c->acc_busy[k] = false; E.fresh = false;
        }
        if (p.corner) { E.timed(kStageResolve, [&] { ftk::launch_resolve_corner(Lg, acc, n_samples, job.w, job.h, c->d_out_index.as<uint32_t>() + job.out_base, out_rgb, out_rgba); }); continue; }
        const ftk::ResolveArgs ra{acc, n_samples, p.classify ? kept : nullptr, job.id_base, n_pix, p.spp,
                                  p.classify ? F.d_pos_block.as<uint32_t>() : nullptr, (p.classify && first && !zeros_in_place) ? F.d_block_pos.as<int32_t>() : nullptr,
                                  (uint32_t)(p.n_pix_total / 64), c->d_pixels.as<uint32_t>(), out_rgb, out_rgba, (uint32_t)gen.group_log2, fc, last ? F.d_report : nullptr};
        if (p.progressive) {
            ft_context::Progressive& P = c->prog;
            const int in = P.cur, out = P.cur ^ 1;
            const ftk::ProgressiveArgs pa{P.d_sum[in].as<double>(), P.d_sum[out].as<double>(), P.d_sq[in].as<double>(), P.d_sq[out].as<double>(),
                                          P.d_blk[in].as<uint32_t>(), P.d_blk[out].as<uint32_t>(), (uint32_t)P.n_pix, (uint32_t)P.min_samples, P.tolerance};
            ftk::ResolveArgs rp = ra;
            rp.block_pos = p.classify && first ? F.d_block_pos.as<int32_t>() : nullptr;
            E.timed(kStageResolve, [&] { ftk::launch_resolve_progressive(Lr, rp, pa); });
        } else if (p.simple) {
            hipEvent_t traced = E.fresh ? E.boundary : nullptr;
            if (!traced) { if (!(traced = E.next())) { c->err = "hipEventCreate failed"; return FT_ERR_HIP; } FT_HIP(c, hipEventRecord(traced, ms)); }
            FT_HIP(c, hipStreamWaitEvent(c->tail, traced, 0));
            ftk::Launch La = Lr; La.stream = c->tail;
            ftk::launch_resolve(La, ra);
            if (!c->acc_free[at]) FT_HIP(c, hipEventCreateWithFlags(&c->acc_free[at], hipEventDisableTiming));
            FT_HIP(c, hipEventRecord(c->acc_free[at], c->tail));
            c->acc_busy[at] = true;
            c->acc_turn = (c->acc_turn + 1) % ft_context::kAcc;
            E.fresh = false;
        } else E.timed(kStageResolve, [&] { ftk::launch_resolve(Lr, ra); });
        if (last) F.fc_clean = true;
    }
    if (!F.fc_clean) { ftk::launch_report(Lg, fc, F.d_report); F.fc_clean = true; }
    n_launches += (p.n_planned - (int32_t)p.jobs.size()) * (2 + n_levels);
    return FT_OK;
}

static int32_t queue_frame(ft_context* c, const RenderRequest& q, const FramePlan& p, void* out, ft_stats* stats, bool defer,
                           std::chrono::steady_clock::time_point wall0) {
    int32_t rc;
    bool uploads_queued = false;
    if ((rc = upload_frame_inputs(c, q, p, uploads_queued)) != FT_OK) return rc;
    if (!defer && (rc = retire_pending(c, nullptr)) != FT_OK) return rc;
    const int turn = c->slot_turn;
    ft_context::FrameSlot& F = c->slots[turn];
    if (!defer || !c->accum_open) { for (int k = 0; k < kStages; ++k) { c->k_ms[k] = 0; c->k_launches[k] = 0; } c->accum_open = defer; }
    F.keeps = p.keepable && !p.reuse; F.reuses = p.reuse;
    if (!p.reuse) F.kept.valid = false;
    if (F.keeps) F.kept.key = p.key;
    c->reuse_counts[p.reuse ? 1 : 0] += p.classify ? 1 : 0;
    c->reuse_counts[2] += (int64_t)p.jobs.size(); c->reuse_counts[3] += p.n_planned - (int64_t)p.jobs.size();
    if (p.reuse) {
        F.list_leaf = p.list_leaf; F.list_cam = p.cam;
        c->last_classified_slot = turn;
    } else if (p.classify) {
        const size_t n_blocks = (size_t)p.n_pix_total / 64, n_waves = (n_blocks + 255) / 256;
        if ((rc = ensure(c, F.d_block_pos, n_blocks * 4)) != FT_OK) return rc;
        if ((rc = ensure(c, F.d_pos_block, n_blocks * 4)) != FT_OK) return rc;
        if (p.list_leaf >= 0) {
            if ((rc = ensure(c, F.d_list_heads, n_blocks * 4)) != FT_OK) return rc;
            if ((rc = ensure(c, F.d_list_pool, (16 * n_blocks + 4096) * ftk::kListEntryWords * 4)) != FT_OK) return rc;
        }
        F.list_leaf = p.list_leaf; F.list_cam = p.cam;
        c->last_classified_slot = turn;
        if (c->d_wave_counts.bytes < n_waves * 4 || c->classify_epoch >= 0x3FFFFEu) {
            if ((rc = ensure(c, c->d_wave_counts, std::max<size_t>(n_waves * 4, 4096) + 4096 * 4 + 2048 * 64)) != FT_OK) return rc;
            FT_HIP(c, hipStreamSynchronize(c->side));
            FT_HIP(c, hipMemsetAsync(c->d_wave_counts.p, 0, c->d_wave_counts.bytes, c->stream));
            c->classify_epoch = 0;
            uploads_queued = true;
        }
    } else {
        F.list_leaf = -1;
        c->last_classified_slot = -1;
    }
    const ft_context::FrameSlot& prev = c->slots[(turn + ft_context::kSlots - 1) % ft_context::kSlots];
    if (!p.simple && any_pending(c, true) && (rc = retire_pending(c, nullptr)) != FT_OK) return rc;
    const int main_ix = (p.simple && c->opt.mains > 1 && !uploads_queued && prev.pending && prev.simple) ? (prev.main_ix + 1) % (int)c->opt.mains : 0;
    const hipStream_t ms = main_ix ? c->more_mains[main_ix - 1] : c->stream;
    if (c->temporal.fork_owed && q.format == 0) {
        FT_HIP(c, hipStreamWaitEvent(p.simple ? c->tail : ms, c->temporal.fork, 0));
        c->temporal.fork_owed = false;
    }
    if (!F.fc_clean) { FT_HIP(c, hipMemsetAsync(F.d_fc.p, 0, sizeof(ftk::FrameCounters), ms)); uploads_queued = true; }
    F.fc_clean = false;
    F.ev.begin(ms, (int)c->opt.timing);
    if (p.classify && !p.reuse && (rc = queue_classify(c, q, p, F, defer && c->opt.classify_ahead && !uploads_queued)) != FT_OK) return rc;
    if (!F.h_report) {
        FT_HIP(c, hipHostMalloc(reinterpret_cast<void**>(&F.h_report), sizeof(ftk::FrameReport), hipHostMallocDefault));
        FT_HIP(c, hipHostGetDevicePointer(reinterpret_cast<void**>(&F.d_report), F.h_report, 0));
    }
    int32_t n_launches = p.classify ? 1 : 0;
    if ((rc = queue_chunks(c, q, p, F, main_ix, n_launches)) != FT_OK) return rc;
    c->last_n_pix = p.n_pix_total; c->last_res_h = q.res_h; c->last_res_v = q.res_v; c->last_format = q.format;
    if (defer && out) {
        if ((rc = copy_frame_out(c, out, q.format, p.simple ? c->tail : ms)) != FT_OK) return rc;
        F.ev.fresh = false;
    }
    F.ev.open();
    if (p.simple) F.ev.ev1 = F.ev.record(c->tail);
    else F.ev.ev1 = F.ev.fresh ? F.ev.boundary : F.ev.record(ms);
    FT_HIP(c, hipGetLastError());
    F.signature = p.signature; F.simple = p.simple; F.main_ix = main_ix;
    F.pending = true; F.wall0 = wall0;
    F.rays_primary = 0;
    if (p.corner) for (auto& j : p.jobs) F.rays_primary += (uint64_t)j.n_ids * (uint64_t)p.spp;
    else F.rays_primary = (uint64_t)p.n_pix_total * (uint64_t)p.spp;
    F.n_pix_total = p.n_pix_total; F.spp = p.spp; F.n_launches = n_launches; F.n_chunks = p.n_planned; F.classify = p.classify; F.format = q.format;
    c->slot_turn = (c->slot_turn + 1) % ft_context::kSlots;
    if (defer) return FT_OK;
    if ((rc = retire_frame(c, F, stats)) != FT_OK) return rc;
    if (out && (rc = fetch_single(c, out, q.format)) != FT_OK) return rc;
    if (stats) stats->wall_ms = std::chrono::duration<double, std::milli>(std::chrono::steady_clock::now() - wall0).count();
    return FT_OK;
// ... 146 lines not shown
```

functracer_amd/csrc/ft_kernels.hip:

```cpp
#define FT_UNIT_MESH_FRAME 1
#define FT_UNIT_PRIMARY 2
#define FT_UNIT_BOUNCE 4
#ifndef FT_UNIT
#define FT_UNIT 7
#endif
#include <hip/hip_runtime.h>
#include <math.h>
#include <stdint.h>

#include "ft_device.h"
#include "ft_filter.h"

using namespace ftd;

namespace ftk {
namespace {

#define FT_DEV __device__ __forceinline__

constexpr double kEps = 0.0000001;
constexpr int kDone = INT32_MIN;

#define FT_CONST __attribute__((address_space(4)))
typedef const FT_CONST double* cdp;
typedef const FT_CONST uint32_t* cup;
typedef const FT_CONST int32_t* cip;
template <class T> FT_DEV const FT_CONST T* to_const_as(const T* p) {
#pragma clang diagnostic push
#pragma clang diagnostic ignored "-Wold-style-cast"
    return (const FT_CONST T*)p;
#pragma clang diagnostic pop
}
FT_DEV uint32_t opaque_zero() { uint32_t z; asm volatile("s_mov_b32 %0, 0" : "=s"(z)); return z; }
template <class T> FT_DEV const FT_CONST T* kernel_args() {
#pragma clang diagnostic push
#pragma clang diagnostic ignored "-Wold-style-cast"
    return (const FT_CONST T*)__builtin_amdgcn_kernarg_segment_ptr();
#pragma clang diagnostic pop
}
template <class T> FT_DEV const FT_CONST T* fresh(const FT_CONST T* p) {
#pragma clang diagnostic push
#pragma clang diagnostic ignored "-Wold-style-cast"
    return (const FT_CONST T*)((const FT_CONST char*)p + opaque_zero());
#pragma clang diagnostic pop
}
typedef const FT_CONST Primary* PrimaryArg;

struct Scene {
    cdp leaves;
    cdp m2w;
    cdp materials;
    cdp lights;
    cdp textures;
    cup program;
    cip meshes;
    cdp nodes;
    cup bsp_leaves;
    cdp tris;
    cdp culls;
    cup tri_orig;
    cdp wide;
    cip mesh_wide;
    cdp ls_pairs;
    cup ls_nodes;
    cdp ls_tris;
    const uint8_t* tex_pixels;
    const float* cull_items;
    const float* coarse_boxes;
    cdp cull_rows;
    cup item_pc;
    int32_t n_leaves, n_lights, csg_cap, stack_cap, n_items, n_cull_rows, csg_rows, lane_fold, n_simd;
};
static_assert(sizeof(Texture) == 384 && sizeof(CullRecord) == 192 && sizeof(Leaf) == 128 && sizeof(Material) == 64 && sizeof(Light) == 96 && sizeof(Mesh) == 16 && sizeof(BspNode) == 64 && sizeof(BspLeaf) == 8, "flat layout");
template <class DS> FT_DEV Scene scene_view(const DS& g) {
    Scene s;
    s.leaves = to_const_as(g.leaves); s.m2w = to_const_as(g.m2w);
    s.materials = to_const_as(reinterpret_cast<const double*>(g.materials)); s.lights = to_const_as(reinterpret_cast<const double*>(g.lights));
    s.textures = to_const_as(reinterpret_cast<const double*>(g.textures));
    s.program = to_const_as(g.program); s.meshes = to_const_as(reinterpret_cast<const int32_t*>(g.meshes));
    s.nodes = to_const_as(reinterpret_cast<const double*>(g.nodes)); s.bsp_leaves = to_const_as(reinterpret_cast<const uint32_t*>(g.bsp_leaves));
    s.tris = to_const_as(g.tris); s.culls = to_const_as(g.culls); s.tri_orig = to_const_as(g.tri_orig); s.wide = to_const_as(g.wide); s.mesh_wide = to_const_as(g.mesh_wide);
    s.ls_pairs = to_const_as(g.ls_pairs); s.ls_nodes = to_const_as(g.ls_nodes); s.ls_tris = to_const_as(g.ls_tris);
    s.tex_pixels = g.tex_pixels; s.cull_items = g.cull_items; s.coarse_boxes = g.coarse_boxes; s.cull_rows = to_const_as(g.cull_rows); s.item_pc = to_const_as(g.item_pc); s.n_items = g.n_items; s.n_cull_rows = g.n_cull_rows;
    s.n_leaves = g.n_leaves; s.n_lights = g.n_lights; s.csg_cap = g.csg_cap; s.stack_cap = g.stack_cap; s.csg_rows = g.csg_rows; s.lane_fold = g.lane_fold; s.n_simd = g.n_simd;
    return s;
}
struct MaterialV { double colour[3]; double roughness, reflectance, shineyness; uint32_t apply_lighting; int32_t texture; uint32_t hue_rot; };
FT_DEV MaterialV material_at(const Scene& S, uint32_t i) {
    cdp m = S.materials + 8ull * i;
    MaterialV v;
    v.colour[0] = m[0]; v.colour[1] = m[1]; v.colour[2] = m[2]; v.roughness = m[3]; v.reflectance = m[4]; v.shineyness = m[5];
    v.apply_lighting = reinterpret_cast<cup>(m + 6)[0]; v.texture = reinterpret_cast<cip>(m + 6)[1]; v.hue_rot = reinterpret_cast<cup>(m + 7)[0];
    return v;
}
FT_DEV bool material_lit(const Scene& S, uint32_t i) { return reinterpret_cast<cup>(S.materials + 8ull * i + 6)[0] != 0; }
FT_DEV int32_t material_texture(const Scene& S, uint32_t i) { return reinterpret_cast<cip>(S.materials + 8ull * i + 6)[1]; }
FT_DEV uint32_t light_kind(const Scene& S, uint32_t l) { return reinterpret_cast<cup>(S.lights + 12ull * l + 10)[0]; }
FT_DEV int32_t light_samples(const Scene& S, uint32_t l) { return reinterpret_cast<cip>(S.lights + 12ull * l + 10)[1]; }

struct Ray { double ox, oy, oz, dx, dy, dz; };
struct V3 { double x, y, z; };

FT_DEV double dot3(double ax, double ay, double az, double bx, double by, double bz) { return ax * bx + ay * by + az * bz; }
FT_DEV V3 normalise(V3 v) {
    const double l2 = v.x * v.x + v.y * v.y + v.z * v.z;
    if (!(l2 >= kEps * kEps) || !(l2 < 1e300)) {
        const double l = sqrt(l2);
        if (l < kEps) return v;
        const double s = 1.0 / l;
        return {s * v.x, s * v.y, s * v.z};
    }
    double y = __builtin_amdgcn_rsq(l2);
    const double h = 0.5 * l2;
    y = __builtin_fma(y, __builtin_fma(-(h * y), y, 0.5), y);
    y = __builtin_fma(y, __builtin_fma(-(h * y), y, 0.5), y);
    return {y * v.x, y * v.y, y * v.z};
}
FT_DEV double fs_max(double a, double b) { return (a != a || b != b) ? __builtin_nan("") : (a < b ? b : a); }
FT_DEV double fs_min(double a, double b) { return (a != a || b != b) ? __builtin_nan("") : (a < b ? a : b); }

FT_DEV uint32_t lane_id() { return __lane_id(); }
FT_DEV double uniform_f64(double v) {
    const unsigned long long b = (unsigned long long)__double_as_longlong(v);
    const uint32_t lo = (uint32_t)__builtin_amdgcn_readfirstlane((int)(uint32_t)b), hi = (uint32_t)__builtin_amdgcn_readfirstlane((int)(uint32_t)(b >> 32));
    return __longlong_as_double((long long)(((unsigned long long)hi << 32) | lo));
}
FT_DEV uint32_t lanes_below(unsigned long long mask) { return __builtin_amdgcn_mbcnt_hi((uint32_t)(mask >> 32), __builtin_amdgcn_mbcnt_lo((uint32_t)mask, 0u)); }

constexpr uint32_t kClkWaves = 8192, kClkWords = 48, kClkSection = 16, kClkWalk = kClkSection + 28;
#ifdef FT_ITEM_COUNTS
__device__ unsigned long long g_clk[kClkWaves * kClkWords];
#define FT_CLK_SLOT() (((blockIdx.x * (kBlock / 64) + threadIdx.x / 64) & (kClkWaves - 1u)) * kClkWords)
#define FT_LANE0_ADD(base, k, v) if (lane_id() == 0) atomicAdd(&g_clk[FT_CLK_SLOT() + (base) + (k)], (v))
#define FT_SLOT_ADD(base, k, v) do { const unsigned long long v_ = (unsigned long long)(v); FT_LANE0_ADD(base, k, v_); } while (0)
#define FT_CLK_NOW() __builtin_amdgcn_s_memtime()
// ... 661 lines not shown
            st.push(ch[3], m[3]); st.push(ch[2], m[2]); st.push(ch[1], m[1]);
            if (m[0]) { cur = ch[0]; continue; }
        } else {
            const uint32_t first = (uint32_t)(~cur) >> 3, count = (uint32_t)(~cur) & 7u;
            const unsigned long long clk_leaf = FT_WALK_NOW();
            any_hit_leaf(S.ls_tris, first, count, r, bound, q, alive);
            b.wL = alive ? b.wL : __builtin_inff();
            FT_WALK_ADD(1, count); FT_WALK_ADD(2, FT_WALK_NOW() - clk_leaf);
            if (!__any(alive)) break;
        }
        if (!st.pop(cur)) break;
    }
}

FT_DEV void mesh_shadow_packet(const Scene& S, cdp P, const Ray& r, Query<true>& q) {
    bool alive = q.active && !q.blocked;
    if (!__any(alive)) return;
    LsLane b = ls_project(P, r, alive);
    FT_WALK_ADD(3, 1);
    ls_tree_walk(S, reinterpret_cast<cip>(P + 14)[0], b, r, q, alive);
}

FT_DEV uint32_t ls_cell(float x, float s, uint32_t n) {
    const float f = __builtin_floorf(__builtin_fmaf(x, s, 0.5f * (float)n));
    return (uint32_t)__builtin_amdgcn_readfirstlane((int)(uint32_t)fminf(fmaxf(f, 0.0f), (float)(n - 1)));
}
FT_DEV void mesh_shadow_grid(const Scene& S, cdp P, const Ray& r, Query<true>& q) {
    bool alive = q.active && !q.blocked;
    if (!__any(alive)) return;
    LsLane b = ls_project(P, r, alive);
    FT_WALK_ADD(3, 1);
    const uint32_t cells = reinterpret_cast<cup>(P + 14)[1], dims = reinterpret_cast<cup>(P + 15)[1];
    const float s = __uint_as_float(reinterpret_cast<cup>(P + 15)[0]);
    const uint32_t nu = dims & 0xFFFFu, nv = dims >> 16;
    const float inf = __builtin_inff();
    const float u_min = wave_min(alive ? b.uL : inf), u_max = wave_max(alive ? b.uH : -inf);
    const float v_min = wave_min(alive ? b.vL : inf), v_max = wave_max(alive ? b.vH : -inf);
    const uint32_t i0 = ls_cell(u_min, s, nu), i1 = ls_cell(u_max, s, nu), j0 = ls_cell(v_min, s, nv), j1 = ls_cell(v_max, s, nv);
    if ((i1 - i0 + 1) * (j1 - j0 + 1) > kLsGridWaveCells) { ls_tree_walk(S, reinterpret_cast<cip>(P + 14)[0], b, r, q, alive); return; }
    const double bound = q.max_dist;
    for (uint32_t j = j0; j <= j1; ++j) {
        for (uint32_t i = i0; i <= i1; ++i) {
            FT_WALK_ADD(0, 1);
            cup C = S.ls_nodes + cells + 4u * (j * nu + i);
            const uint32_t first = C[0], count = C[2];
            const FT_CONST float* bx = reinterpret_cast<const FT_CONST float*>(S.ls_nodes + C[1]);
            const float w_min = wave_min(b.wL);
            const unsigned long long clk_leaf = FT_WALK_NOW();
            uint32_t tested = 0;
            for (uint32_t base = 0; base < count; base += 64) {
                const uint32_t e = base + lane_id();
                const FT_CONST float* eb = bx + 5u * min(e, count - 1u);
                const float eu0 = eb[0], eu1 = eb[1], ev0 = eb[2], ev1 = eb[3], ew = eb[4];
                unsigned long long m = __ballot((e < count) & (eu0 <= u_max) & (eu1 >= u_min) & (ev0 <= v_max) & (ev1 >= v_min) & (ew >= w_min));
                while (m) {
                    const int k = (int)__builtin_ctzll(m);
                    m &= m - 1ull;
                    const float bu0 = __int_as_float(__builtin_amdgcn_readlane(__float_as_int(eu0), k)), bu1 = __int_as_float(__builtin_amdgcn_readlane(__float_as_int(eu1), k));
                    const float bv0 = __int_as_float(__builtin_amdgcn_readlane(__float_as_int(ev0), k)), bv1 = __int_as_float(__builtin_amdgcn_readlane(__float_as_int(ev1), k));
                    const float bw = __int_as_float(__builtin_amdgcn_readlane(__float_as_int(ew), k));
                    if (!__any((bu0 <= b.uH) & (bu1 >= b.uL) & (bv0 <= b.vH) & (bv1 >= b.vL) & (bw >= b.wL))) continue;
                    any_hit_leaf(S.ls_tris, first + base + (uint32_t)k, 1, r, bound, q, alive);
                    b.wL = alive ? b.wL : inf;
                    ++tested;
                    if (!__any(alive)) break;
                }
                if (!__any(alive)) break;
            }
            FT_WALK_ADD(1, tested); FT_WALK_ADD(2, FT_WALK_NOW() - clk_leaf);
            if (!__any(alive)) return;
        }
    }
}

struct ListQuery { const uint32_t* pool; uint32_t head; uint32_t leaf; float x0, x1, y0, y1; };
FT_DEV void mesh_list_closest(const Scene& S, const ListQuery& Lq, const Ray& r, Query<false>& q, uint32_t leaf, bool lit) {
    const bool alive = q.active;
    const uint32_t count = Lq.head & 127u, first = Lq.head >> 7;
    FT_LIST_ADD(7, 1); FT_LIST_ADD(2, count);
    if (count == 0u || !__any(alive)) return;
    const uint32_t* E = Lq.pool + (size_t)kListEntryWords * (first + min(lane_id(), count - 1u));
    const uint32_t tri_v = E[0], orig_v = E[1];
    const float ex0 = __uint_as_float(E[2]), ex1 = __uint_as_float(E[3]), ey0 = __uint_as_float(E[4]), ey1 = __uint_as_float(E[5]);
    unsigned long long m = __ballot((lane_id() < count) & (ex0 <= Lq.x1) & (ex1 >= Lq.x0) & (ey0 <= Lq.y1) & (ey1 >= Lq.y0));
    FT_LIST_ADD(3, __popcll(m));
    double reach = alive ? q.best_t : -__builtin_inf();
    uint32_t best_tri = 0xFFFFFFFFu;
    bool found = false;
    while (m) {
        const int k = (int)__builtin_ctzll(m);
        m &= m - 1ull;
        const uint32_t tri = (uint32_t)__builtin_amdgcn_readlane((int)tri_v, k);
        double t = 0.0;
        const bool h = tri_hit_wave(S.tris + 9ull * tri, r, alive, t);
        if (__any(h)) {
            const uint32_t orig = (uint32_t)__builtin_amdgcn_readlane((int)orig_v, k);
            const bool nearer = h & ((t < reach) | (found & (t == reach) & (orig < best_tri)));
            reach = nearer ? t : reach; best_tri = nearer ? orig : best_tri; found = found | nearer;
        }
    }
    if (found) q.hit(reach, leaf, best_tri, lit);
}

constexpr int kSparseLanes = 8;
struct ItemMask { unsigned long long lo, hi; bool valid; };
struct Cone { float ax, ay, az, cx, cy, cz, cos_t, sin_t, rho; uint32_t par_rows; float far; };
FT_DEV bool cone_may_reach(float ix, float iy, float iz, float radius, uint32_t rows, const Cone& B, float origin_mag) {
    const float vx = ix - B.cx, vy = iy - B.cy, vz = iz - B.cz;
    const float slack = 1e-5f * (1.0f + origin_mag + fabsf(ix) + fabsf(iy) + fabsf(iz));
    const float reach = radius * 1.0001f + B.rho + slack;
    const float h = vx * B.ax + vy * B.ay + vz * B.az;
    const float v2 = vx * vx + vy * vy + vz * vz;
    const float w = sqrtf(fmaxf(0.0f, v2 - h * h));
    const float out_of_range = B.far + reach;
    if (v2 > out_of_range * out_of_range * 1.0001f && !((rows & B.par_rows) != 0u)) return false;
    const float beyond = h > 0.0f ? w * B.cos_t - h * B.sin_t : fmaxf(w * B.cos_t, -h);
    return !(beyond > reach) || (rows & B.par_rows) != 0u;
}
struct ItemRecs { float x[2], y[2], z[2], r[2]; uint32_t rows[2]; };
FT_DEV ItemRecs item_recs(const Scene& S) {
    ItemRecs R{{0.0f, 0.0f}, {0.0f, 0.0f}, {0.0f, 0.0f}, {0.0f, 0.0f}, {0u, 0u}};
    const int n_pass = S.n_items > 64 ? 2 : 1;
    for (int pass = 0; pass < n_pass; ++pass) {
        const int item = pass * 64 + (int)lane_id();
        if (item < S.n_items) {
            const float* I = S.cull_items + 8 * (item + (int)opaque_zero());
            R.x[pass] = I[0]; R.y[pass] = I[1]; R.z[pass] = I[2]; R.r[pass] = I[3]; R.rows[pass] = __float_as_uint(I[4]);
        }
    }
    return R;
}
FT_DEV ItemMask items_in_cone(const Scene& S, const Cone& B, const ItemRecs& R) {
    ItemMask M{~0ull, ~0ull, true};
    const float origin_mag = fabsf(B.cx) + fabsf(B.cy) + fabsf(B.cz);
    const int n_pass = S.n_items > 64 ? 2 : 1;
    for (int pass = 0; pass < n_pass; ++pass) {
        const int item = pass * 64 + (int)lane_id();
        bool keep = true;
// ... 662 lines not shown
    return to_const_as(Kx->gen.list_heads)[blk];
}
FT_DEV Ray offset_ray(const Ray& r) { return {r.ox + 0.0001 * r.dx, r.oy + 0.0001 * r.dy, r.oz + 0.0001 * r.dz, r.dx, r.dy, r.dz}; }
FT_DEV void wave_rect(ListQuery& lq, const double (&jxy)[2], bool active) {
    const float inf = __builtin_inff();
    const float fx = (float)jxy[0], fy = (float)jxy[1], sx = 2.4e-7f * fabsf(fx) + 1e-37f, sy = 2.4e-7f * fabsf(fy) + 1e-37f;
    lq.x0 = wave_min(active ? fx - sx : inf); lq.x1 = wave_max(active ? fx + sx : -inf);
    lq.y0 = wave_min(active ? fy - sy : inf); lq.y1 = wave_max(active ? fy + sy : -inf);
}
FT_DEV void store_first(const FT_CONST PrimaryArgs* Ka, uint32_t i, double cr, double cg, double cb) {
    double* acc = Ka->acc; const uint32_t acc_stride = Ka->acc_stride;
    acc[i] = 1.0 * cr; acc[(size_t)acc_stride + i] = 1.0 * cg; acc[2 * (size_t)acc_stride + i] = 1.0 * cb;
}
template <bool FANCY, bool SOFT, bool MESH, int BLOCKS>
__global__ __launch_bounds__(kBlock, BLOCKS) void k_primary(PrimaryArgs) {
    extern __shared__ __attribute__((aligned(16))) uint32_t lds[];
    const FT_CONST PrimaryArgs* K = kernel_args<PrimaryArgs>();
    const Scene S = scene_view(K->S);
    ChunkCounters* cc = &K->fc->cc;
    const Pix px = pix_count(&K->gen);
    const uint32_t n_pix = px.n;
    const uint32_t n = n_pix * (uint32_t)K->gen.spp;
    const int n_lights = S.n_lights;
    unsigned long long n_shadow_wave = 0, n_refl_wave = 0, n_ovf_wave = 0, n_hit_wave = 0;
    const uint32_t B = px.group_log2 ? 64u : batch_lanes_for(n, S.lane_fold, S.n_simd);
    const uint32_t n_batches = (n + B - 1) / B;
    const bool coherent = K->S.coherent_waves != 0;
    constexpr bool kOneLeaf = MESH && !FANCY && !SOFT;
    auto at_of = [&](uint32_t batch) -> SlotAt { return px.group_log2 ? slot_at(px, batch, lane_id()) : slot_at(px, batch * B + lane_id()); };
    BatchCursor cursor(&cc->work_trace[0][0]);
    uint32_t bi = cursor.grab(), bi_next = cursor.grab();
    uint32_t pid_next = 0;
    if (bi < n_batches && bi * B + lane_id() < n && lane_id() < B) pid_next = primary_pixel(&K->gen, at_of(bi));
    const bool use_lists = MESH && coherent && px.group_log2 != 0u && K->gen.list_heads != nullptr;
    uint32_t head_next = kListNone;
    if (use_lists && bi < n_batches) head_next = list_head_of(K, px, bi);
    for (; bi < n_batches; bi = bi_next, bi_next = cursor.grab()) {
        const uint32_t i = bi * B + lane_id();
        const uint32_t pid = pid_next;
        ListQuery lq{nullptr, head_next, 0u, 0.f, 0.f, 0.f, 0.f};
        const bool active = i < n && lane_id() < B;
        const unsigned long long clk_batch = FT_CLK_NOW();
        Ray ro{0, 0, 0, 0, 0, 0};
        bool empty = false;
        {
            const FT_CONST PrimaryArgs* Kb = fresh(K);
            if (bi_next < n_batches && bi_next * B + lane_id() < n && lane_id() < B) pid_next = primary_pixel(&Kb->gen, at_of(bi_next));
            if (use_lists && bi_next < n_batches) head_next = list_head_of(Kb, px, bi_next);
            empty = use_lists && lq.head != kListNone && (lq.head & 127u) == 0u && Kb->S.uniform_surface != 0 && Kb->S.n_items == 1 && Kb->gen.cam.has_focus == 0;
            double jxy[2] = {0.0, 0.0};
            if (active && !empty) ro = offset_ray(primary_ray_from(&Kb->gen, at_of(bi).s, pid, jxy));
            if (MESH && lq.head != kListNone && !empty) {
                wave_rect(lq, jxy, active);
                lq.pool = Kb->gen.list_pool; lq.leaf = (uint32_t)Kb->gen.list_leaf;
            }
        }
        Query<false> q = Query<false>::closest(active);
        bool overflow = false;
        const unsigned long long clk_a = FT_CLK_NOW();
        FT_CLK_ADD(22, clk_batch);
        if (!empty) trace<false, MESH>(S, ro, q, lds, overflow, coherent, nullptr, -1, MESH ? &lq : nullptr);
        else FT_LIST_ADD(6, 1);
        FT_CLK_ADD(23, clk_a);
        n_ovf_wave += (unsigned long long)__popcll(__ballot(overflow && active));
        const bool hit = active && q.id0 != ID_MISS;
        const unsigned long long hit_mask = __ballot(hit);
        double cr = 0.0, cg = 0.0, cb = 0.0;
        if (hit_mask) {
            Surface sf{{0, 0, 0}, {0, 1, 0}, 0, 0.0, 0.0};
            bool lit = false;
            unsigned long long sample = 0ull;
            const unsigned long long clk_s = FT_CLK_NOW();
            bool one_leaf = false;
            uint32_t wave_leaf = 0u;
            if (kOneLeaf && coherent && fresh(K)->S.uniform_surface != 0) {
                wave_leaf = (uint32_t)__builtin_amdgcn_readlane((int)(q.id0 & ID_LEAF_MASK), (int)__builtin_ctzll(hit_mask));
                one_leaf = __ballot(hit && (q.id0 & ID_LEAF_MASK) != wave_leaf) == 0ull;
                if (one_leaf) FT_CLK_INC(27);
            }
            if (hit) {
                if (kOneLeaf && one_leaf) {
                    sf = surface_at<FANCY, true>(S, ro, q.best_t, q.id0, q.id1, wave_leaf);
                    lit = material_lit(S, leaf_head(S, wave_leaf).material);
                } else {
                    sf = surface_at<FANCY>(S, ro, q.best_t, q.id0, q.id1);
                    lit = material_lit(S, sf.material);
                }
                if (SOFT) sample = (unsigned long long)pid * (unsigned long long)fresh(K)->gen.spp + at_of(bi).s;
            }
            unsigned long long vis_lo, vis_hi;
            const unsigned long long clk_b = FT_CLK_NOW();
            FT_CLK_ADD(10, clk_s);
            light_visibility<SOFT, MESH>(S, sf, lit, sample, [&]() { return fresh(K)->gen.seed; }, 0, coherent, lds, vis_lo, vis_hi, n_shadow_wave, n_ovf_wave);
            FT_CLK_ADD(24, clk_b);
            const bool uniform = coherent && fresh(K)->S.uniform_surface != 0;
            const uint32_t wave_mat = (uint32_t)__builtin_amdgcn_readlane((int)sf.material, (int)__builtin_ctzll(hit_mask));
            MaterialV mat;
            if (kOneLeaf && uniform && __ballot(hit && sf.material != wave_mat) == 0ull) mat = material_at(S, wave_mat);
            else mat = material_at(S, sf.material);
            if (FANCY) { if (hit && mat.texture >= 0) textured_colour(S, mat, sf.u, sf.v, mat.colour); }
            const FT_CONST PrimaryArgs* K2 = fresh(K);
            const bool spawn = lit && mat.reflectance > 0.0 && 0 < K2->max_depth;
            const bool reads_view = spawn || (lit && (mat.shineyness > 0.0 || (FANCY && mat.roughness != 0.0)));
            Ray rv{0, 0, 0, 0, 0, 0};
            if (!uniform || __any(reads_view)) { if (hit) rv = primary_ray_from(&K2->gen, at_of(bi).s, pid); }
            shade_lights<FANCY, SOFT, !FANCY>(S, sf, mat, rv, hit, lit, vis_lo, vis_hi, cr, cg, cb, uniform);
            const unsigned long long m = __ballot(spawn);
// ... 17 lines not shown
        }
        if (active) store_first(fresh(K), i, cr, cg, cb);
        FT_CLK_ADD(25, clk_batch); FT_CLK_INC(26);
    }
    RenderCounters* mine = my_stats(fresh(K)->fc);
    wave_add(&mine->rays_shadow, n_shadow_wave);
    wave_add(&mine->rays_shadow_primary, n_shadow_wave);
    wave_add(&mine->rays_reflect, n_refl_wave);
    wave_add(&mine->rays_reflect_primary, n_refl_wave);
    wave_add(&mine->hits_total, n_hit_wave);
    wave_add(&mine->hits_primary, n_hit_wave);
    wave_add(&mine->csg_overflow, n_ovf_wave);
    wave_add(&mine->ref_equiv, uniform_f64((double)fresh(K)->S.shadow_rays_per_hit * (double)n_hit_wave + (double)n_lights * (double)n_refl_wave));
}

template <int BLOCKS>
__global__ __launch_bounds__(kBlock, BLOCKS) void k_primary_mesh(PrimaryArgs) {
    const FT_CONST PrimaryArgs* K = kernel_args<PrimaryArgs>();
    constexpr uint32_t kLeaf = 0u;
    Pix px = pix_count(&K->gen);
    {
        const unsigned long long b = (unsigned long long)__double_as_longlong(px.inv_blocks);
        const uint32_t veil = lane_id() * opaque_zero();
        const uint32_t lo = (uint32_t)__builtin_amdgcn_readfirstlane((int)((uint32_t)b + veil)), hi = (uint32_t)__builtin_amdgcn_readfirstlane((int)((uint32_t)(b >> 32) + veil));
        px.inv_blocks = __longlong_as_double((long long)(((unsigned long long)hi << 32) | lo));
    }
    const uint32_t n = px.n * (uint32_t)K->gen.spp;
    const uint32_t n_batches = (n + 63u) / 64u;
    unsigned long long n_shadow_wave = 0, n_hit_wave = 0;
    BatchCursor cursor(&K->fc->cc.work_trace[0][0]);
    uint32_t bi = cursor.grab(), bi_next = cursor.grab();
    uint32_t pid_next = 0;
    if (bi < n_batches && bi * 64u + lane_id() < n) pid_next = primary_pixel(&K->gen, slot_at(px, bi, lane_id()));
    const bool use_lists = px.group_log2 != 0u && K->gen.list_heads != nullptr;
    uint32_t head_next = kListNone;
    if (use_lists && bi < n_batches) head_next = list_head_of(K, px, bi);
    for (; bi < n_batches; bi = bi_next, bi_next = cursor.grab()) {
        const uint32_t i = bi * 64u + lane_id();
        const uint32_t pid = pid_next;
        ListQuery lq{nullptr, head_next, kLeaf, 0.f, 0.f, 0.f, 0.f};
        const bool active = i < n;
        const unsigned long long clk_batch = FT_CLK_NOW();
        Ray ro{0, 0, 0, 0, 0, 0};
        bool empty = false;
        {
            const FT_CONST PrimaryArgs* Kb = fresh(K);
            if (bi_next < n_batches && bi_next * 64u + lane_id() < n) pid_next = primary_pixel(&Kb->gen, slot_at(px, bi_next, lane_id()));
            if (use_lists && bi_next < n_batches) head_next = list_head_of(Kb, px, bi_next);
            empty = use_lists && lq.head != kListNone && (lq.head & 127u) == 0u;
            double jxy[2] = {0.0, 0.0};
            if (active && !empty) ro = offset_ray(primary_ray_from(&Kb->gen, slot_at(px, bi, lane_id()).s, pid, jxy));
            if (lq.head != kListNone && !empty) {
                wave_rect(lq, jxy, active);
                lq.pool = Kb->gen.list_pool;
            }
        }
        Query<false> q = Query<false>::closest(active);
        const unsigned long long clk_a = FT_CLK_NOW();
        FT_CLK_ADD(22, clk_batch);
        if (!empty) {
            const Scene S = scene_view(fresh(K)->S);
            const LeafHead H = leaf_head(S, kLeaf);
            Ray rm;
            to_model(S.leaves + 16ull * kLeaf, (H.flags & LF_XFORM) != 0, ro, rm);
            FT_MESH_COUNT(0, 0, 1); FT_MESH_COUNT(0, 1, 1); FT_MESH_COUNT(0, 2, __popcll(__ballot(active))); FT_MESH_COUNT(0, 3, 1);
            if (lq.head != kListNone) mesh_list_closest(S, lq, rm, q, kLeaf, (H.flags & LF_LIT) != 0);
            else mesh_bvh_packet<false>(S, S.mesh_wide[H.mesh], rm, q, kLeaf, (H.flags & LF_LIT) != 0);
            FT_CLK_ADD(1, clk_a);
        } else FT_LIST_ADD(6, 1);
        FT_CLK_ADD(23, clk_a);
        const bool hit = active && q.id0 != ID_MISS;
        const unsigned long long hit_mask = __ballot(hit);
        double cr = 0.0, cg = 0.0, cb = 0.0;
        if (hit_mask) {
            Surface sf{{0, 0, 0}, {0, 1, 0}, 0, 0.0, 0.0};
            bool lit = false;
            const unsigned long long clk_s = FT_CLK_NOW();
            FT_CLK_INC(27);
            if (hit) {
                const Scene S = scene_view(fresh(K)->S);
                sf = surface_at<false, true>(S, ro, q.best_t, q.id0, q.id1, kLeaf);
                lit = material_lit(S, leaf_head(S, kLeaf).material);
            }
            unsigned long long vis_lo = 0ull, vis_hi = 0ull;
            const unsigned long long clk_b = FT_CLK_NOW();
            FT_CLK_ADD(10, clk_s);
            {
                const Scene S = scene_view(fresh(K)->S);
                const int n_lights = S.n_lights;
                for (int l = 0; l < n_lights; ++l) {
                    cdp lp = S.lights + 12ull * (uint32_t)l;
                    const double sox = sf.p.x + 0.0001 * sf.n.x, soy = sf.p.y + 0.0001 * sf.n.y, soz = sf.p.z + 0.0001 * sf.n.z;
                    Query<true> qs = Query<true>::any(lit, 1.7976931348623157e308);
                    if (__any(lit)) {
                        const unsigned long long clk_q = FT_CLK_NOW();
                        FT_MESH_COUNT(2, 0, 1); FT_MESH_COUNT(2, 1, 1); FT_MESH_COUNT(2, 2, __popcll(__ballot(lit))); FT_MESH_COUNT(2, 3, 1);
                        const LeafHead H = leaf_head(S, kLeaf);
                        const Ray sr{sox, soy, soz, -lp[0], -lp[1], -lp[2]};
                        Ray rm;
                        to_model(S.leaves + 16ull * kLeaf, (H.flags & LF_XFORM) != 0, sr, rm);
                        const uint32_t pairs = reinterpret_cast<cup>(S.leaves + 16ull * kLeaf + 12)[4];
                        cdp P = S.ls_pairs + (unsigned long long)kLsPairDoubles * (pairs + (uint32_t)l);
                        if (pairs != ~0u && reinterpret_cast<cip>(P + 14)[0] != INT32_MIN) {
                            if (reinterpret_cast<cup>(P + 15)[1] != 0u) mesh_shadow_grid(S, P, rm, qs);
                            else mesh_shadow_packet(S, P, rm, qs);
                        } else mesh_bvh_packet<true>(S, S.mesh_wide[H.mesh], rm, qs, kLeaf, true);
                        FT_CLK_ADD(9, clk_q);
// ... 297 lines not shown
    const uint32_t n_keep = (uint32_t)__popcll(km);
    if (lane_id() == 0) sh_wave_keep[wave] = n_keep;
    __syncthreads();
    uint32_t n_keep_wg = 0, before_wave = 0;
    for (uint32_t w = 0; w < kClassifyBlock / 64; ++w) { if (w < wave) before_wave += sh_wave_keep[w]; n_keep_wg += sh_wave_keep[w]; }
    const uint32_t epoch = K->epoch;
    if (threadIdx.x == 0) __hip_atomic_store(&out.wave_counts[ticket], (epoch << 10) | (n_keep_wg + 1u), __ATOMIC_RELAXED, __HIP_MEMORY_SCOPE_AGENT);
    if (wave == 0) {
        uint32_t before = 0;
        bool timed_out = false;
        for (uint32_t j0 = 0; j0 < ticket; j0 += 64u) {
            const uint32_t j = j0 + lane_id();
            uint32_t v = (epoch << 10) | 1u;
            if (j < ticket) {
                uint32_t polls = 0;
                for (;;) {
                    v = __hip_atomic_load(&out.wave_counts[j], __ATOMIC_RELAXED, __HIP_MEMORY_SCOPE_AGENT);
                    if ((v >> 10) == epoch || ++polls > kClassifyPollLimit) break;
                    __builtin_amdgcn_s_sleep(2);
                }
                if ((v >> 10) != epoch) { timed_out = true; v = (epoch << 10) | 1u; }
            }
            uint32_t c = (v & 0x3FFu) - 1u;
            for (int off = 32; off > 0; off >>= 1) c += __shfl_xor(c, off);
            before += c;
        }
        if (__any(timed_out) && lane_id() == 0) atomicOr(&K->fc->classify_error, 1u);
        if (lane_id() == 0) sh_before = before;
    }
    __syncthreads();
    FT_STAMP(4);
    const uint32_t before = sh_before + before_wave;
    const uint32_t pos = before + lanes_below(km);
    if (valid) out.block_pos[blk] = keep ? (int32_t)pos : (gone ? kBlockRetired : -1);
    if (keep) out.pos_block[pos] = blk;
    if (threadIdx.x == 0 && (ticket + 1u) * kClassifyBlock >= n_blocks && ticket * kClassifyBlock < n_blocks)
        out.kept->n_pix = 64u * (sh_before + n_keep_wg);
    const unsigned long long n_valid = (unsigned long long)__popcll(__ballot(valid));
    wave_add(&K->fc->stats[(ticket * (kClassifyBlock / 64) + wave) % (uint32_t)kStatStripes].pixels_culled, 64ull * (n_valid - (unsigned long long)n_keep));
    FT_STAMP(5);
}

struct BlockListArgs {
    DevScene S; Primary gen;
    const uint32_t* pos_block; BlockLists out; FrameCounters* fc;
    double jitter_extent;
    const PixCount* counts;
};
constexpr double kProjEps = 1e-12;
FT_DEV float round_down(double x) { return (float)(x - (2.4e-7 * fabs(x) + 1e-37)); }
FT_DEV float round_up(double x) { return (float)(x + (2.4e-7 * fabs(x) + 1e-37)); }
__global__ __launch_bounds__(kBlock) void k_block_lists(BlockListArgs) {
    __shared__ uint32_t sh_entries[kBlock / 64][kListCap * kListEntryWords];
    const FT_CONST BlockListArgs* K = kernel_args<BlockListArgs>();
    const Scene S = scene_view(K->S);
    const PrimaryArg g = &K->gen;
    const uint32_t wave = (uint32_t)__builtin_amdgcn_readfirstlane((int)(threadIdx.x / 64u));
    uint32_t* mine = sh_entries[wave];
    const uint32_t n_active = to_const_as(K->counts)->n_pix / 64u;
    const uint32_t leaf = (uint32_t)K->out.leaf;
    const LeafHead Hm = leaf_head(S, leaf);
    cdp Mw = S.leaves + 16ull * leaf;
    const bool xform = (Hm.flags & LF_XFORM) != 0;
    const int32_t root = S.mesh_wide[Hm.mesh];
    Ray mk, mi, mj;
    to_model(Mw, xform, Ray{g->cam.o[0], g->cam.o[1], g->cam.o[2], g->cam.k[0], g->cam.k[1], g->cam.k[2]}, mk);
    to_model(Mw, xform, Ray{g->cam.o[0], g->cam.o[1], g->cam.o[2], g->cam.i[0], g->cam.i[1], g->cam.i[2]}, mi);
    to_model(Mw, xform, Ray{g->cam.o[0], g->cam.o[1], g->cam.o[2], g->cam.j[0], g->cam.j[1], g->cam.j[2]}, mj);
    const double c0x = mi.dy * mj.dz - mi.dz * mj.dy, c0y = mi.dz * mj.dx - mi.dx * mj.dz, c0z = mi.dx * mj.dy - mi.dy * mj.dx;
    const double c1x = mj.dy * mk.dz - mj.dz * mk.dy, c1y = mj.dz * mk.dx - mj.dx * mk.dz, c1z = mj.dx * mk.dy - mj.dy * mk.dx;
    const double c2x = mk.dy * mi.dz - mk.dz * mi.dy, c2y = mk.dz * mi.dx - mk.dx * mi.dz, c2z = mk.dx * mi.dy - mk.dy * mi.dx;
    const double det = mk.dx * c0x + mk.dy * c0y + mk.dz * c0z, inv_det = 1.0 / det;
    const double r0x = c0x * inv_det, r0y = c0y * inv_det, r0z = c0z * inv_det, r1x = c1x * inv_det, r1y = c1y * inv_det, r1z = c1z * inv_det,
                 r2x = c2x * inv_det, r2y = c2y * inv_det, r2z = c2z * inv_det;
    const double omx = mk.ox, omy = mk.oy, omz = mk.oz;
    const bool usable = root != INT32_MIN && fabs(det) > 1e-300 &&
                        fabs(r0x) + fabs(r0y) + fabs(r0z) + fabs(r1x) + fabs(r1y) + fabs(r1z) + fabs(r2x) + fabs(r2y) + fabs(r2z) + fabs(omx) + fabs(omy) + fabs(omz) < 1e300;
    const uint32_t side = lane_id() & 3u, child = (lane_id() >> 2) & 3u;
    for (uint32_t pos = blockIdx.x * (kBlock / 64u) + wave; pos < n_active; pos += gridDim.x * (kBlock / 64u)) {
        const uint32_t blk = to_const_as(K->pos_block)[pos];
        const uint32_t pid0 = to_const_as(g->pixel_ids)[(size_t)blk * 64u], pid1 = to_const_as(g->pixel_ids)[(size_t)blk * 64u + 63u];
        const uint32_t y0 = div_by(pid0, g->inv_stride), x0 = pid0 - y0 * g->stride, y1 = div_by(pid1, g->inv_stride), x1 = pid1 - y1 * g->stride;
        const BlockRect R = block_rect(g, x0, y0, x1, y1, K->jitter_extent);
        double d[5][3];
        block_corner_dirs(g, R, d);
        const Pyramid Py = block_pyramid(Mw, xform, g, d);
        const float bx0 = round_down(R.jxa), bx1 = round_up(R.jxb), by0 = round_down(R.jya), by1 = round_up(R.jyb);
        const float nx = side == 0u ? Py.pn[0][0] : side == 1u ? Py.pn[1][0] : side == 2u ? Py.pn[2][0] : Py.pn[3][0];
        const float ny = side == 0u ? Py.pn[0][1] : side == 1u ? Py.pn[1][1] : side == 2u ? Py.pn[2][1] : Py.pn[3][1];
        const float nz = side == 0u ? Py.pn[0][2] : side == 1u ? Py.pn[1][2] : side == 2u ? Py.pn[2][2] : Py.pn[3][2];
        const bool sided = ((Py.sided >> side) & 1u) != 0u;
        bool whole = usable && Py.sided == 0xFu && bx0 <= bx1 && by0 <= by1;
        uint32_t n = 0;
        WaveStack st;
        int cur = root;
        while (whole) {
            cur = __builtin_amdgcn_readfirstlane(cur);
            st.sp = __builtin_amdgcn_readfirstlane(st.sp);
            if (cur >= 0) {
                cdp nd = S.wide + (unsigned long long)kWideNodeDoubles * (uint32_t)cur;
                const int32_t ch[4] = {reinterpret_cast<cip>(nd + 24)[0], reinterpret_cast<cip>(nd + 24)[1], reinterpret_cast<cip>(nd + 24)[2], reinterpret_cast<cip>(nd + 24)[3]};
                cdp bx = nd + 6u * child;
                const float qx = (float)((nx > 0.0f ? bx[3] : bx[0]) - Py.ox), qy = (float)((ny > 0.0f ? bx[4] : bx[1]) - Py.oy), qz = (float)((nz > 0.0f ? bx[5] : bx[2]) - Py.oz);
                const uint32_t cut = (uint32_t)(__ballot(lane_id() < 16u && beyond_side(nx, ny, nz, sided, qx, qy, qz)) & 0xFFFFull);
#pragma unroll
                for (int c = 3; c >= 0; --c) st.push(ch[c], __builtin_amdgcn_ballot_w64(ch[c] != INT32_MIN && ((cut >> (4 * c)) & 0xFu) == 0u));
            } else {
                const uint32_t first = S.bsp_leaves[2 * (~cur)], count = S.bsp_leaves[2 * (~cur) + 1];
                for (uint32_t base = 0; base < count && whole; base += 64u) {
                    const uint32_t k = base + lane_id(), tri = first + (k < count ? k : count - 1u);
                    cdp T = S.tris + 9ull * tri;
                    const double vx[3] = {T[0], T[0] + T[3], T[0] + T[6]}, vy[3] = {T[1], T[1] + T[4], T[1] + T[7]}, vz[3] = {T[2], T[2] + T[5], T[2] + T[8]};
                    double xl = __builtin_inf(), xh = -__builtin_inf(), yl = __builtin_inf(), yh = -__builtin_inf();
                    bool bounded = true;
#pragma unroll
                    for (int v = 0; v < 3; ++v) {
                        const double px = vx[v] - omx, py = vy[v] - omy, pz = vz[v] - omz;
                        const double mx = fabs(vx[v]) + fabs(omx), my = fabs(vy[v]) + fabs(omy), mz = fabs(vz[v]) + fabs(omz);
                        const double a = r0x * px + r0y * py + r0z * pz, b = r1x * px + r1y * py + r1z * pz, c = r2x * px + r2y * py + r2z * pz;
                        const double ea = kProjEps * (fabs(r0x) * mx + fabs(r0y) * my + fabs(r0z) * mz), eb = kProjEps * (fabs(r1x) * mx + fabs(r1y) * my + fabs(r1z) * mz),
                                     ec = kProjEps * (fabs(r2x) * mx + fabs(r2y) * my + fabs(r2z) * mz);
                        const double am = a - ea;
                        const double jx = b / a, jy = c / a, ex = (eb + fabs(jx) * ea) / am, ey = (ec + fabs(jy) * ea) / am;
                        bounded = bounded && am > 0.0 && fabs(jx) + fabs(jy) + ex + ey < 1e300;
                        xl = fmin(xl, jx - ex); xh = fmax(xh, jx + ex); yl = fmin(yl, jy - ey); yh = fmax(yh, jy + ey);
                    }
                    const double grow = 1e-3 * ((xh - xl) + (yh - yl));
                    const float inf = __builtin_inff();
                    const float tx0 = bounded ? round_down(xl - grow) : -inf, tx1 = bounded ? round_up(xh + grow) : inf;
                    const float ty0 = bounded ? round_down(yl - grow) : -inf, ty1 = bounded ? round_up(yh + grow) : inf;
                    const bool keep = k < count && tx0 <= bx1 && tx1 >= bx0 && ty0 <= by1 && ty1 >= by0;
                    const unsigned long long km = __ballot(keep);
                    const uint32_t n_keep = (uint32_t)__popcll(km);
                    if (n + n_keep > kListCap) { whole = false; break; }
                    if (keep) {
                        uint32_t* e = mine + kListEntryWords * (n + lanes_below(km));
                        e[0] = tri; e[1] = S.tri_orig[tri]; e[2] = __float_as_uint(tx0); e[3] = __float_as_uint(tx1); e[4] = __float_as_uint(ty0); e[5] = __float_as_uint(ty1);
                    }
                    n += n_keep;
                }
            }
            if (!st.pop(cur)) break;
        }
        uint32_t head = kListNone;
        if (whole) {
            uint32_t at = 0;
            if (lane_id() == 0 && n) at = atomicAdd(&K->fc->list_cursor, n);
            at = (uint32_t)__builtin_amdgcn_readfirstlane((int)at);
            if (at <= K->out.pool_entries && n <= K->out.pool_entries - at && at + n < (1u << 25)) {
                __builtin_amdgcn_wave_barrier();
                uint32_t* dst = K->out.pool + (size_t)kListEntryWords * at;
                for (uint32_t w = lane_id(); w < kListEntryWords * n; w += 64u) dst[w] = mine[w];
                head = (at << 7) | n;
            }
        }
        if (lane_id() == 0) K->out.heads[pos] = head;
        __builtin_amdgcn_wave_barrier();
    }
}

FT_DEV void write_pixel(double* out_rgb, uint8_t* out_rgba, size_t o, double r, double g, double b) {
    if (out_rgb) { out_rgb[3 * o] = r; out_rgb[3 * o + 1] = g; out_rgb[3 * o + 2] = b; }
    if (out_rgba) store_rgba8(out_rgba, o, r, g, b);
}

FT_DEV void hand_over_frame(FrameCounters* fc, const PixCount* counts, FrameReport* report, unsigned long long* cells) {
    __shared__ uint32_t last;
    const uint32_t t = threadIdx.x;
    __syncthreads();
    if (t == 0) {
        const uint32_t stripe = blockIdx.x & 63u, in_stripe = (gridDim.x - stripe + 63u) / 64u, n_stripes = gridDim.x < 64u ? gridDim.x : 64u;
        last = 0u;
        if (atomicAdd(&fc->report_stripe[stripe], 1u) == in_stripe - 1u) last = atomicAdd(&fc->report_ticket, 1u) == n_stripes - 1u ? 1u : 0u;
    }
    __syncthreads();
    if (!last) return;
    __builtin_amdgcn_fence(__ATOMIC_ACQUIRE, "agent");
    static_assert(sizeof(RenderCounters) == 128 && kStatStripes * 16 == 4 * kBlock, "the stripes are read as 4 x 256 eight-byte cells");
    const unsigned long long* src = reinterpret_cast<const unsigned long long*>(&fc->stats[0]);
    for (uint32_t k = 0; k < 4; ++k) cells[k * kBlock + t] = src[k * kBlock + t];
    unsigned long long* rep = cells;
    __syncthreads();
    unsigned long long sum = 0ull;
    if (t < 16) {
        if (t == 4) { double s = 0.0; for (int k = 0; k < kStatStripes; ++k) s += __longlong_as_double((long long)cells[16 * k + 4]); sum = (unsigned long long)__double_as_longlong(s); }
        else for (int k = 0; k < kStatStripes; ++k) sum += cells[16 * k + t];
    }
    uint32_t word = 0u;
    if (t >= 64 && t < 64 + kMaxBounce + 2) word = fc->cc.n_rays[t - 64];
    else if (t == 128) word = counts ? counts->n_pix : 0u;
    else if (t == 129) word = fc->classify_error;
    __syncthreads();
    uint32_t* words = reinterpret_cast<uint32_t*>(rep);
    if (t < 16) rep[t] = sum;
    else if (t >= 64 && t < 64 + kMaxBounce + 2) words[32 + (t - 64)] = word;
    else if (t == 128 || t == 129) words[32 + kMaxBounce + 2 + (t - 128)] = word;
    else if (t >= 130 && t < 142) words[34 + kMaxBounce + 2 + (t - 130)] = 0u;
    __syncthreads();
    if (t < 64) reinterpret_cast<uint32_t*>(report)[t] = words[t];
    __syncthreads();
    uint4* z = reinterpret_cast<uint4*>(fc);
    for (uint32_t w = threadIdx.x; w < sizeof(FrameCounters) / 16; w += kBlock) z[w] = uint4{0u, 0u, 0u, 0u};
}
__global__ __launch_bounds__(kBlock) void k_report(FrameCounters* fc, FrameReport* report) {
    __shared__ unsigned long long cells[kStatStripes * 16];
// ... 376 lines not shown
```

functracer_amd/csrc/ft_lightspace.hip:

```cpp
#include <hip/hip_runtime.h>
#include <rocprim/device/device_scan.hpp>

#include <math.h>
#include <stdint.h>

#include "ft_device.h"

using namespace ftd;

namespace ftk {
namespace {

__device__ __forceinline__ float f_down(double v) { float f = (float)v; if ((double)f > v) f = __uint_as_float(f > 0.0f ? __float_as_uint(f) - 1u : (f < 0.0f ? __float_as_uint(f) + 1u : 0x80000001u)); return f; }
__device__ __forceinline__ float f_up(double v) { return -f_down(-v); }
__device__ __forceinline__ double dot_lr(const double p[3], const double a[3]) { return __dadd_rn(__dadd_rn(__dmul_rn(p[0], a[0]), __dmul_rn(p[1], a[1])), __dmul_rn(p[2], a[2])); }

__device__ __forceinline__ void grow_by_tri(const double* __restrict__ T, const LsFrame& F, double lo[2], double hi[2], double& wmax) {
    for (int v = 0; v < 3; ++v) {
        double p[3];
        for (int q = 0; q < 3; ++q) p[q] = __dadd_rn(__dsub_rn(T[q], F.c[q]), v == 1 ? T[3 + q] : v == 2 ? T[6 + q] : 0.0);
        const double pu = dot_lr(p, F.U), pv = dot_lr(p, F.V), pw = dot_lr(p, F.D);
        lo[0] = fmin(lo[0], pu); hi[0] = fmax(hi[0], pu);
        lo[1] = fmin(lo[1], pv); hi[1] = fmax(hi[1], pv);
        wmax = fmax(wmax, pw);
    }
}
__device__ __forceinline__ void round_box(const double lo[2], const double hi[2], double wmax, double pad, float box[5]) {
    box[0] = f_down(lo[0] - pad); box[1] = f_up(hi[0] + pad);
    box[2] = f_down(lo[1] - pad); box[3] = f_up(hi[1] + pad);
    box[4] = f_up(wmax + pad);
}

__global__ __launch_bounds__(256) void k_ls_refit(uint32_t* __restrict__ nodes, uint32_t n_nodes, const double* __restrict__ tris, uint32_t n_tris,
                                                  const uint32_t* __restrict__ order, uint32_t count, LsFrame F) {
    const uint32_t i = blockIdx.x * 256u + threadIdx.x;
    if (i >= count) return;
    const uint32_t n = order[i];
    if (n >= n_nodes) return;
    uint32_t* N = nodes + (size_t)kLsNodeWords * n;
    for (int c = 0; c < 4; ++c) {
        const int32_t child = (int32_t)N[20 + c];
        if (child == INT32_MIN) continue;
        float box[5];
        if (child >= 0) {
            if ((uint32_t)child >= n_nodes) continue;
            const float* B = reinterpret_cast<const float*>(nodes + (size_t)kLsNodeWords * (uint32_t)child);
            box[0] = box[2] = INFINITY; box[1] = box[3] = box[4] = -INFINITY;
            for (int k = 0; k < 4; ++k) {
                box[0] = fminf(box[0], B[5 * k]); box[1] = fmaxf(box[1], B[5 * k + 1]);
                box[2] = fminf(box[2], B[5 * k + 2]); box[3] = fmaxf(box[3], B[5 * k + 3]);
                box[4] = fmaxf(box[4], B[5 * k + 4]);
            }
        } else {
            const uint32_t first = (uint32_t)~child >> 3, cnt = (uint32_t)~child & 7u;
            if ((uint64_t)first + cnt > n_tris) continue;
            double lo[2] = {INFINITY, INFINITY}, hi[2] = {-INFINITY, -INFINITY}, wmax = -INFINITY;
            for (uint32_t t = 0; t < cnt; ++t) grow_by_tri(tris + 9ull * (first + t), F, lo, hi, wmax);
            round_box(lo, hi, wmax, F.pad, box);
        }
// ... 30 lines not shown
    }
}

template <bool FILL>
__global__ __launch_bounds__(256) void k_ls_cells(const float* __restrict__ ebox, uint32_t n, float s, uint32_t nu, uint32_t nv, uint32_t* __restrict__ counts,
                                                  const uint32_t* __restrict__ first, uint32_t* __restrict__ idx, uint32_t n_idx) {
    const uint32_t k = blockIdx.x * 256u + threadIdx.x;
    if (k >= n) return;
    const float* e = ebox + 5ull * k;
    const uint32_t i0 = ls_cell(e[0], s, nu), i1 = ls_cell(e[1], s, nu), j0 = ls_cell(e[2], s, nv), j1 = ls_cell(e[3], s, nv);
    for (uint32_t j = j0; j <= j1 && j < nv; ++j)
        for (uint32_t i = i0; i <= i1 && i < nu; ++i) {
            const uint32_t cell = j * nu + i;
            const uint32_t at = atomicAdd(&counts[cell], 1u);
            if (FILL) { const uint32_t p = first[cell] + at; if (p < n_idx) idx[p] = k; }
        }
}

__global__ __launch_bounds__(256) void k_ls_max(const uint32_t* __restrict__ counts, uint32_t n_cells, uint32_t* __restrict__ out) {
    const uint32_t c = blockIdx.x * 256u + threadIdx.x;
    if (c < n_cells && counts[c] > 0u) atomicMax(out, counts[c]);
}

__global__ __launch_bounds__(256) void k_ls_emit(const float* __restrict__ ebox, const double* __restrict__ tris, uint32_t n, const uint32_t* __restrict__ idx,
                                                 const uint32_t* __restrict__ counts, const uint32_t* __restrict__ first, uint32_t n_cells, uint32_t n_entries,
                                                 uint32_t* __restrict__ ls_nodes, uint32_t at, double* __restrict__ ls_tris, uint32_t tri_at) {
    __shared__ uint32_t s_idx[4][kLsGridMaxCell];
    __shared__ float s_w[4][kLsGridMaxCell];
    const uint32_t wave = threadIdx.x >> 6, lane = threadIdx.x & 63u;
    const uint32_t cell = blockIdx.x * 4u + wave;
    const bool live = cell < n_cells;
    const uint32_t f0 = live ? first[cell] : 0u;
    uint32_t cnt = live ? counts[cell] : 0u;
    if (cnt > kLsGridMaxCell) cnt = kLsGridMaxCell;
    if ((uint64_t)f0 + cnt > n_entries) cnt = 0u;
    const uint32_t box0 = at + 4u * n_cells;
    if (live && lane == 0u) { uint32_t* W = ls_nodes + at + 4ull * cell; W[0] = tri_at + f0; W[1] = box0 + 5u * f0; W[2] = cnt; W[3] = 0u; }
    for (uint32_t k = lane; k < cnt; k += 64u) {
        uint32_t t = idx[f0 + k];
        if (t >= n) t = 0u;
        s_idx[wave][k] = t; s_w[wave][k] = ebox[5ull * t + 4];
    }
    __syncthreads();
    for (uint32_t k = lane; k < cnt; k += 64u) {
        const uint32_t t = s_idx[wave][k]; const float w = s_w[wave][k];
        uint32_t rank = 0;
        for (uint32_t j = 0; j < cnt; ++j) { const float wj = s_w[wave][j]; rank += (wj > w || (wj == w && s_idx[wave][j] < t)) ? 1u : 0u; }
        const uint32_t e = f0 + rank;
        for (int q = 0; q < 5; ++q) ls_nodes[box0 + 5ull * e + q] = __float_as_uint(ebox[5ull * t + q]);
        for (int q = 0; q < 9; ++q) ls_tris[9ull * (tri_at + e) + q] = tris[9ull * t + q];
    }
}

}

void ls_grid_entries(hipStream_t stream, const double* tris, uint32_t n, const LsFrame& F, float* ebox, uint32_t* ruv) {
    hipLaunchKernelGGL(k_ls_entries, dim3((n + 255u) / 256u), dim3(256), 0, stream, tris, n, F, ebox, ruv);
}
void ls_grid_count(hipStream_t stream, const float* ebox, uint32_t n, const LsGridCandidates& C, unsigned long long* sums) {
    hipLaunchKernelGGL(k_ls_count, dim3((n + 255u) / 256u), dim3(256), 0, stream, ebox, n, C, sums);
}
void ls_grid_cell_counts(hipStream_t stream, const float* ebox, uint32_t n, float s, uint32_t nu, uint32_t nv, uint32_t* counts, uint32_t* max_count) {
    hipLaunchKernelGGL(k_ls_cells<false>, dim3((n + 255u) / 256u), dim3(256), 0, stream, ebox, n, s, nu, nv, counts, (const uint32_t*)nullptr, (uint32_t*)nullptr, 0u);
    if (max_count) hipLaunchKernelGGL(k_ls_max, dim3((nu * nv + 255u) / 256u), dim3(256), 0, stream, counts, nu * nv, max_count);
}
hipError_t ls_grid_scan(hipStream_t stream, const uint32_t* counts, uint32_t* first, uint32_t n_cells, void* tmp, size_t* tmp_bytes) {
    return rocprim::exclusive_scan(tmp, *tmp_bytes, counts, first, 0u, (size_t)n_cells, rocprim::plus<uint32_t>(), stream);
}
void ls_grid_emit(hipStream_t stream, const float* ebox, const double* tris, uint32_t n, float s, uint32_t nu, uint32_t nv, const uint32_t* counts, const uint32_t* first,
                  uint32_t* cursor, uint32_t* idx, uint32_t n_entries, uint32_t* ls_nodes, uint32_t at, double* ls_tris, uint32_t tri_at) {
    hipLaunchKernelGGL(k_ls_cells<true>, dim3((n + 255u) / 256u), dim3(256), 0, stream, ebox, n, s, nu, nv, cursor, first, idx, n_entries);
    hipLaunchKernelGGL(k_ls_emit, dim3((nu * nv + 3u) / 4u), dim3(256), 0, stream, ebox, tris, n, idx, counts, first, nu * nv, n_entries, ls_nodes, at, ls_tris, tri_at);
}

void ls_refit_level(hipStream_t stream, uint32_t* nodes, uint32_t n_nodes, const double* tris, uint32_t n_tris, const uint32_t* order, uint32_t count, const LsFrame& F) {
    if (count == 0u) return;
    hipLaunchKernelGGL(k_ls_refit, dim3((count + 255u) / 256u), dim3(256), 0, stream, nodes, n_nodes, tris, n_tris, order, count, F);
}

}
```

include/functracer_hip.h:

```cpp
#ifndef FUNCTRACER_HIP_H
#define FUNCTRACER_HIP_H

#include <stddef.h>
#include <stdint.h>

#ifdef __cplusplus
extern "C" {
#endif

#define FT_ABI_VERSION 2

typedef struct ft_context ft_context;
typedef int32_t ft_node;

typedef enum ft_status {
    FT_OK = 0,
    FT_ERR_INVALID = -1,
    FT_ERR_NO_DEVICE = -2,
    FT_ERR_HIP = -3,
    FT_ERR_UNSUPPORTED = -4,
    FT_ERR_STATE = -5,
    FT_ERR_OVERFLOW = -6,
    FT_ERR_BUILD = -7
} ft_status;
// ... 139 lines not shown
int32_t ft_denoise(ft_context* ctx, const ft_camera* cam, int32_t res_h, int32_t res_v, int32_t spp,
                   const double* jitter_xy, int32_t sample, uint64_t seed, const ft_rect* tiles, int32_t n_tiles,
                   const ft_denoise_params* params, int32_t rgba8, void* out, ft_stats* stats);

#define FT_TEMPORAL_MIN_WEIGHT 0.0625
typedef struct ft_temporal_params { int32_t max_history, to_frame; double min_normal_dot, position_tolerance_px; } ft_temporal_params;
int32_t ft_temporal_begin(ft_context* ctx, int32_t res_h, int32_t res_v, const ft_rect* tiles, int32_t n_tiles);
int32_t ft_temporal_accumulate(ft_context* ctx, const ft_camera* cam, int32_t spp, const double* jitter_xy, int32_t sample, uint64_t seed,
                               const ft_temporal_params* params, int32_t rgba8, void* out, ft_stats* stats);
int32_t ft_temporal_fetch(ft_context* ctx, double* mean_rgb, double* stderr_rgb, double* length);
int32_t ft_temporal_status(ft_context* ctx, int64_t out[4]);
typedef struct ft_temporal_clamp_params { int32_t radius, clamped_history; double gamma, floor; } ft_temporal_clamp_params;
int32_t ft_temporal_set_clamp(ft_context* ctx, const ft_temporal_clamp_params* params);
int32_t ft_temporal_clamp_status(ft_context* ctx, int64_t out[2]);
int32_t ft_temporal_end(ft_context* ctx);

typedef struct ft_temporal_filter_params { int32_t iterations, demodulate, min_history, to_frame;
    double sigma_colour, sigma_normal, sigma_position, albedo_floor, variance_floor; } ft_temporal_filter_params;
int32_t ft_temporal_filter(ft_context* ctx, const ft_camera* cam, int32_t spp, const double* jitter_xy, int32_t sample, uint64_t seed,
                           const ft_temporal_filter_params* params, int32_t rgba8, void* out, double* out_variance, ft_stats* stats);

#define FT_TEMPORAL_QUEUE_DEPTH 4
int32_t ft_temporal_enqueue(ft_context* ctx, const ft_camera* cam, int32_t spp, const double* jitter_xy, int32_t sample, uint64_t seed,
                            const ft_temporal_params* params, const ft_temporal_filter_params* filter ,
                            int32_t rgba8, void* host_out);
int32_t ft_temporal_wait(ft_context* ctx, ft_stats* stats);

int32_t ft_scene_commit_moved(ft_context* ctx);
int32_t ft_sg_set_mesh_triangles(ft_context* ctx, ft_node node, const double* tris, int64_t n_tris);
int32_t ft_scene_commit_deformed(ft_context* ctx);
int32_t ft_scene_tree_quality(ft_context* ctx, ft_node mesh_node, double out[4]);
int32_t ft_scene_set_directional(ft_context* ctx, int32_t light, const double dir[3], const double colour[3]);
int32_t ft_scene_set_soft_directional(ft_context* ctx, int32_t light, const double dir[3], double scatter_rad, const double colour[3]);
int32_t ft_scene_set_positional(ft_context* ctx, int32_t light, const double pos[3], const double falloff[3], const double colour[3]);
int32_t ft_scene_commit_lights(ft_context* ctx);

int32_t ft_debug_leaf_matrices(ft_context* ctx, int64_t* n_leaves, double* m2w, double* w2m);

int32_t ft_debug_closest(ft_context* ctx, const double* origins, const double* dirs, int64_t n,
                         int32_t* hit, double* t, double* p, double* nrm, double* colour);
int32_t ft_debug_blocked(ft_context* ctx, const double* origins, const double* dirs,
                         const double* max_dist, int64_t n, int32_t* blocked);

int32_t ft_debug_colour(ft_context* ctx, const double* origins, const double* dirs, int64_t n, int32_t max_depth, double* rgb);

int32_t ft_create_host_only(ft_context** out);
int32_t ft_debug_scene_info(ft_context* ctx, int64_t out[12]);
int32_t ft_debug_slice(const double p0[3], const double n[3], const double tri[9],
                       double above[18], int32_t* n_above, double below[18], int32_t* n_below);
int32_t ft_debug_light_space(ft_context* ctx, int64_t sizes[4], double* pairs, uint32_t* nodes, double* tris, uint32_t* leaf_pairs);
int32_t ft_debug_mesh_trees(ft_context* ctx, int64_t sizes[12], void* nodes, uint32_t* bsp_leaves, double* tris, uint32_t* tri_orig, uint32_t* tri_src,
                            double* wide, float* coarse_boxes, int32_t* meshes, uint32_t* jobs);
int32_t ft_debug_block_lists(ft_context* ctx, int64_t sizes[4], double plane[4], uint32_t* heads, uint32_t* pos_block, uint32_t* entries);
int32_t ft_debug_classify_reuse(ft_context* ctx, int64_t out[4]);
int32_t ft_debug_primary_kernels(ft_context* ctx, int64_t out[2]);
int32_t ft_get_kernel_times(ft_context* ctx, double ms[5], int32_t launches[5]);

int32_t ft_debug_devices(ft_context* ctx, int32_t* ordinals, int32_t capacity);

int32_t ft_quantise_rgba8(const double* rgb, int64_t n_pixels, uint8_t* out_rgba);

#ifdef __cplusplus
}
#endif
#endif
```

Baseline: 42100.

## Add conservative edge-function culling for light-space grid and block-list triangles

Precomputes per-triangle float edge-plane records (three conservative half-planes with error margins) for light-space grid cells and for primary block lists. During traversal, a candidate triangle whose edge records show it lies entirely outside the ray's rectangle is rejected before the double-precision intersection test. This is meant to cut wasted ray-triangle tests for triangles whose bounding boxes overlap the query but whose area does not. In exchange it adds build-time kernels, extra device and LDS memory, and a per-candidate float check, and it depends on the conservative margins to avoid dropping real hits.

After: 46110, median of 6. 9.5% higher.

```diff
diff --git a/functracer_amd/__init__.py b/functracer_amd/__init__.py
--- a/functracer_amd/__init__.py
+++ b/functracer_amd/__init__.py
@@ -610,6 +610,16 @@
         self._check(fn(self._ctx, sizes, plane.ctypes.data, heads.ctypes.data, pos_block.ctypes.data, entries.ctypes.data))
         return {"leaf": int(sizes[2]), "heads": heads, "pos_block": pos_block, "entries": entries, "plane": plane, "capacity": int(sizes[3])}
 
+    def edge_records(self):
+        sizes = (C.c_int64 * 2)()
+        fn = self._lib.ft_debug_edge_records
+        fn.restype, fn.argtypes = C.c_int32, [C.c_void_p, C.POINTER(C.c_int64), C.c_void_p, C.c_void_p]
+        self._check(fn(self._ctx, sizes, None, None))
+        grid = np.zeros((sizes[0],) + _capi.EDGE_RECORD_SHAPE, dtype=np.float32)
+        lists = np.zeros((sizes[1],) + _capi.EDGE_RECORD_SHAPE, dtype=np.float32)
+        self._check(fn(self._ctx, sizes, grid.ctypes.data, lists.ctypes.data))
+        return {"grid": grid[:sizes[0]], "lists": lists[:sizes[1]]}
+
     def classify_reuse(self):
         out = (C.c_int64 * 4)()
         self._check(self._lib.ft_debug_classify_reuse(self._ctx, out))
diff --git a/functracer_amd/_capi.py b/functracer_amd/_capi.py
--- a/functracer_amd/_capi.py
+++ b/functracer_amd/_capi.py
@@ -156,6 +156,7 @@
 CLASSIFY_REUSE_FIELDS = ("classified", "reused", "windows_launched", "windows_skipped")
 LIST_ENTRY_DTYPE = np.dtype([("tri", np.uint32), ("orig", np.uint32), ("x0", np.float32), ("x1", np.float32), ("y0", np.float32), ("y1", np.float32)])
 LIST_NONE = 0xFFFFFFFF
+EDGE_RECORD_SHAPE = (3, 3)
 
 
 class fth_options(C.Structure):
diff --git a/functracer_amd/csrc/ft_capi.cpp b/functracer_amd/csrc/ft_capi.cpp
--- a/functracer_amd/csrc/ft_capi.cpp
+++ b/functracer_amd/csrc/ft_capi.cpp
@@ -174,6 +174,7 @@
     {"csg_auto_grow", 0, 1, &Options::csg_auto_grow, nullptr, kFlag},
     {"primary_block_lists", 0, 1, &Options::primary_block_lists, nullptr, kFlag | kClassified},
     {"uniform_surface", 0, 1, &Options::uniform_surface, nullptr, kFlag},
+    {"edge_cull", 0, 1, &Options::edge_cull, nullptr, kFlag},
     {"primary_mesh_kernel", 0, 1, &Options::primary_mesh_kernel, nullptr, kFlag},
     {"temporal_follow_deformed", 0, 1, &Options::temporal_follow_deformed, nullptr, kFlag},
     {"refit_rebuild_percent", 100, 1000000, &Options::refit_rebuild_percent, nullptr, kOrZero},
@@ -195,6 +196,7 @@
             for (hipStream_t m : d->more_mains) if (!m) d->opt.mains = 1;
             d->dev_scene.coherent_waves = d->opt.coherent_waves ? 1 : 0;
             d->dev_scene.uniform_surface = d->opt.uniform_surface ? 1 : 0;
+            d->dev_scene.ls_edges = d->opt.edge_cull ? d->lightspace.d_edges.as<float>() : nullptr;
             if (!d->opt.temporal_follow_deformed) temporal_drop_snapshots(d);
             if (o.rules & kCommit) { d->committed = false; c->options_pending = true; }
             if (o.rules & kLevelHint) d->staged_hint = -1;
@@ -417,6 +419,37 @@
     c->blocks_aov = ftk::occupancy_blocks_aov(lds, c->variant);
     c->mesh_kernel_scene = mesh_kernel_scene(f, c->variant);
     c->blocks_primary_mesh = ftk::occupancy_blocks_primary_mesh();
+}
+
+static int32_t build_ls_edges(ft_context* c, const std::vector<double>& pairs, size_t node_words, size_t tri_doubles) {
+    ft_context::LightSpace& L = c->lightspace;
+    ftk::DevScene& S = c->dev_scene;
+    S.ls_edges = nullptr;
+    const size_t n_recs = tri_doubles / 9, bytes = n_recs * ftk::kEdgeFloats * sizeof(float);
+    bool grids = false;
+    for (size_t r = 0; r + 1 <= pairs.size() / ftd::kLsPairDoubles; ++r) {
+        uint32_t w[2];
+        std::memcpy(w, &pairs[ftd::kLsPairDoubles * r + 15], sizeof w);
+        grids = grids || w[1] != 0u;
+    }
+    if (!grids || n_recs == 0 || bytes > ftd::kLsEdgeMaxBytes || node_words > 0xFFFFFFFFull || n_recs > 0xFFFFFFFFull) { L.d_edges.release(); return FT_OK; }
+    int32_t rc;
+    if ((rc = ensure(c, L.d_edges, bytes)) != FT_OK) return rc;
+    FT_HIP(c, hipMemsetAsync(L.d_edges.p, 0, bytes, c->stream));
+    const DeviceBuf* B = c->d_scene;
+    for (size_t r = 0; r + 1 <= pairs.size() / ftd::kLsPairDoubles; ++r) {
+        uint32_t w[2];
+        std::memcpy(w, &pairs[ftd::kLsPairDoubles * r + 15], sizeof w);
+        int32_t root;
+        std::memcpy(&root, &pairs[ftd::kLsPairDoubles * r + 14], 4);
+        if (w[1] == 0u || root == INT32_MIN) continue;
+        ftk::ls_edge_records(c->stream, B[kLsPairs].as<double>() + ftd::kLsPairDoubles * r, B[kLsNodes].as<uint32_t>(), (uint32_t)node_words, B[kLsTris].as<double>(),
+                             (uint32_t)n_recs, (w[1] & 0xFFFFu) * (w[1] >> 16), L.d_edges.as<float>());
+    }
+    FT_HIP(c, hipGetLastError());
+    FT_HIP(c, hipStreamSynchronize(c->stream));
+    S.ls_edges = c->opt.edge_cull ? L.d_edges.as<float>() : nullptr;
+    return FT_OK;
 }
 
 static int32_t upload_scene(ft_context* c) {
@@ -463,6 +496,7 @@
             if ((rc = fit_stacks(c, tallest)) != FT_OK) return rc;
         }
     }
+    if ((rc = build_ls_edges(c, f.ls_pairs, f.ls_nodes.size(), f.ls_tris.size())) != FT_OK) return rc;
     derive_launch_shape(c);
     c->committed = true;
     ++c->commit_serial; c->staged_hint = -1;
@@ -899,6 +933,9 @@
     if ((rc = upload(c, B[kLsPairs], f.ls_pairs)) != FT_OK) return rc;
     FT_HIP(c, hipStreamSynchronize(c->stream));
     ms[0] += since(t2);
+    const auto t3 = clock::now();
+    if (!jobs.empty() && (rc = build_ls_edges(c, f.ls_pairs, L.node_words, L.tri_doubles)) != FT_OK) return rc;
+    ms[1] += since(t3);
     c->zero_signature[0] = c->zero_signature[1] = 0;
     c->committed = true;
     ++c->commit_serial; c->staged_hint = -1;
diff --git a/functracer_amd/csrc/ft_context.h b/functracer_amd/csrc/ft_context.h
--- a/functracer_amd/csrc/ft_context.h
+++ b/functracer_amd/csrc/ft_context.h
@@ -84,6 +84,7 @@
     int64_t refit_rebuild_percent = 0;
     int64_t temporal_follow_deformed = 0;
     int64_t primary_mesh_kernel = 1;
+    int64_t edge_cull = 1;
     int64_t uniform_surface = 1;
 };
 
@@ -187,6 +188,7 @@
     struct FrameSlot {
         DeviceBuf d_block_pos, d_pos_block, d_fc;
         DeviceBuf d_list_heads, d_list_pool;
+        DeviceBuf d_list_edges;
         int32_t list_leaf = -1;
         ftk::Camera list_cam{};
         struct Classified { bool valid = false; ClassifyKey key; int64_t n_active = 0; uint64_t culled = 0; } kept;
@@ -202,7 +204,7 @@
         uint64_t rays_primary = 0; int64_t n_pix_total = 0; int32_t spp = 0, n_launches = 0, n_chunks = 0, format = 0; bool classify = false;
         std::chrono::steady_clock::time_point wall0;
         void release() {
-            d_block_pos.release(); d_pos_block.release(); d_fc.release(); d_list_heads.release(); d_list_pool.release();
+            d_block_pos.release(); d_pos_block.release(); d_fc.release(); d_list_heads.release(); d_list_pool.release(); d_list_edges.release();
             if (h_report) (void)hipHostFree(h_report);
             h_report = nullptr; d_report = nullptr;
             ev.release();
@@ -225,12 +227,13 @@
         size_t base_node_words = 0, base_tri_doubles = 0;
         bool ready = false;
         DeviceBuf d_order, d_first, d_cursor, d_idx, d_small, d_scan;
+        DeviceBuf d_edges;
         std::vector<DeviceBuf> d_ebox, d_counts;
         size_t node_words = 0, tri_doubles = 0;
         bool order_uploaded = false, rewritten = false;
         void reset() { pairs.clear(); order.clear(); ready = order_uploaded = rewritten = false; node_words = tri_doubles = base_node_words = base_tri_doubles = 0; }
         void release() {
-            for (DeviceBuf* b : {&d_order, &d_first, &d_cursor, &d_idx, &d_small, &d_scan}) b->release();
+            for (DeviceBuf* b : {&d_order, &d_first, &d_cursor, &d_idx, &d_small, &d_scan, &d_edges}) b->release();
             for (DeviceBuf& b : d_ebox) b.release();
             for (DeviceBuf& b : d_counts) b.release();
             d_ebox.clear(); d_counts.clear(); reset();
diff --git a/functracer_amd/csrc/ft_debug.cpp b/functracer_amd/csrc/ft_debug.cpp
--- a/functracer_amd/csrc/ft_debug.cpp
+++ b/functracer_amd/csrc/ft_debug.cpp
@@ -237,6 +237,35 @@
     return FT_OK;
 }
 
+int32_t ft_debug_edge_records(ft_context* c, int64_t sizes[2], float* grid_edges, float* list_edges) {
+    if (!c || !sizes) return FT_ERR_INVALID;
+    if (c->host_only) return FT_ERR_NO_DEVICE;
+    sizes[0] = sizes[1] = 0;
+    FT_HIP(c, hipSetDevice(c->device));
+    int32_t rc = retire_queued(c);
+    if (rc != FT_OK) return rc;
+    if ((rc = drain_frame_streams(c)) != FT_OK) return rc;
+    const size_t rec_bytes = ftk::kEdgeFloats * sizeof(float);
+    if (c->committed && c->lightspace.d_edges.p) {
+        const size_t n_recs = (c->lightspace.rewritten ? c->lightspace.tri_doubles : c->flat.ls_tris.size()) / 9;
+        if (c->lightspace.d_edges.bytes < n_recs * rec_bytes) { c->err = "ft_debug_edge_records: the edge array in device memory is smaller than recorded"; return FT_ERR_STATE; }
+        sizes[0] = (int64_t)n_recs;
+        if (grid_edges && n_recs) FT_HIP(c, hipMemcpy(grid_edges, c->lightspace.d_edges.p, n_recs * rec_bytes, hipMemcpyDeviceToHost));
+    }
+    if (c->last_classified_slot < 0) return FT_OK;
+    const ft_context::FrameSlot& F = c->slots[c->last_classified_slot];
+    if (F.list_leaf < 0 || !F.h_report) return FT_OK;
+    const size_t n_active = std::min<size_t>(F.h_report->n_pix_active / 64u, F.d_list_heads.bytes / 4);
+    std::vector<uint32_t> h(n_active);
+    if (n_active) FT_HIP(c, hipMemcpy(h.data(), F.d_list_heads.p, n_active * 4, hipMemcpyDeviceToHost));
+    size_t used = 0;
+    for (uint32_t v : h) if (v != ftk::kListNone) used = std::max<size_t>(used, (size_t)(v >> 7) + (v & 127u));
+    if (used * rec_bytes > F.d_list_edges.bytes) { c->err = "ft_debug_edge_records: a header points past the edge pool"; return FT_ERR_STATE; }
+    sizes[1] = (int64_t)used;
+    if (list_edges && used) FT_HIP(c, hipMemcpy(list_edges, F.d_list_edges.p, used * rec_bytes, hipMemcpyDeviceToHost));
+    return FT_OK;
+}
+
 int32_t ft_debug_classify_reuse(ft_context* c, int64_t out[4]) {
     if (!c || !out) return FT_ERR_INVALID;
     if (c->host_only) return FT_ERR_NO_DEVICE;
diff --git a/functracer_amd/csrc/ft_device.h b/functracer_amd/csrc/ft_device.h
--- a/functracer_amd/csrc/ft_device.h
+++ b/functracer_amd/csrc/ft_device.h
@@ -34,6 +34,7 @@
     const float* coarse_boxes;
     const uint32_t* item_pc;
     const double* cull_rows;
+    const float* ls_edges;
     int32_t n_leaves, n_lights, csg_cap, stack_cap;
     int32_t shadow_rays_per_hit;
     int32_t n_items, n_cull_rows;
@@ -110,6 +111,7 @@
     const uint32_t* block_map;
     int32_t group_log2;
     const uint32_t* list_heads; const uint32_t* list_pool; int32_t list_leaf;
+    const float* list_edges;
 };
 void launch_primary(const Launch& L, const DevScene& S, const Primary& gen, RayBuf next, double* acc, uint32_t acc_stride, int max_depth, FrameCounters* fc);
 int occupancy_blocks_primary(size_t lds_bytes, int* variant);
@@ -121,8 +123,8 @@
 constexpr int32_t kBlockRetired = -2;
 void launch_classify(const Launch& L, const DevScene& S, const Primary& gen_list, const ClassifyOut& out, double jitter_extent, uint32_t epoch, FrameCounters* fc,
                      const uint32_t* retired = nullptr, bool mask_only = false);
-constexpr uint32_t kListNone = 0xFFFFFFFFu, kListCap = 64, kListEntryWords = 6;
-struct BlockLists { uint32_t* heads; uint32_t* pool; uint32_t pool_entries; int32_t leaf; };
+constexpr uint32_t kListNone = 0xFFFFFFFFu, kListCap = 64, kListEntryWords = 6, kEdgeFloats = 9;
+struct BlockLists { uint32_t* heads; uint32_t* pool; uint32_t pool_entries; int32_t leaf; float* edges; };
 void launch_block_lists(const Launch& L, const DevScene& S, const Primary& gen_list, const uint32_t* pos_block, const BlockLists& out, double jitter_extent, FrameCounters* fc, const PixCount* counts);
 struct ResolveArgs {
     const double* acc; uint32_t acc_stride; const PixCount* counts; uint32_t first, n_pix_host; int32_t spp;
@@ -184,6 +186,7 @@
 hipError_t ls_grid_scan(hipStream_t stream, const uint32_t* counts, uint32_t* first, uint32_t n_cells, void* tmp, size_t* tmp_bytes);
 void ls_grid_emit(hipStream_t stream, const float* ebox, const double* tris, uint32_t n, float s, uint32_t nu, uint32_t nv, const uint32_t* counts, const uint32_t* first,
                   uint32_t* cursor, uint32_t* idx, uint32_t n_entries, uint32_t* ls_nodes, uint32_t at, double* ls_tris, uint32_t tri_at);
+void ls_edge_records(hipStream_t stream, const double* pair, const uint32_t* ls_nodes, uint32_t node_words, const double* ls_tris, uint32_t n_recs, uint32_t n_cells, float* edges);
 
 struct AovOut {
     double *t, *p, *n, *colour, *material;
diff --git a/functracer_amd/csrc/ft_edges.h b/functracer_amd/csrc/ft_edges.h
--- /dev/null
+++ b/functracer_amd/csrc/ft_edges.h
@@ -0,0 +1,54 @@
+#ifndef FT_EDGES_H
+#define FT_EDGES_H
+#include <hip/hip_runtime.h>
+
+#include "ft_device.h"
+
+namespace ftk {
+
+constexpr double kEdgeSliver = 2e-6, kEdgeFloatSlack = 1e-6, kEdgeMaxMargin = 5e-3;
+
+__device__ __forceinline__ void edge_record(const double (&x)[3], const double (&y)[3], double E, bool bounded, float (&rec)[kEdgeFloats]) {
+    const double w = fmax(x[0], fmax(x[1], x[2])) - fmin(x[0], fmin(x[1], x[2])), h = fmax(y[0], fmax(y[1], y[2])) - fmin(y[0], fmin(y[1], y[2]));
+    const double X = fmax(fabs(x[0]), fmax(fabs(x[1]), fabs(x[2]))) + E, Y = fmax(fabs(y[0]), fmax(fabs(y[1]), fabs(y[2]))) + E;
+    const double area2 = fabs(__dsub_rn(__dmul_rn(x[1] - x[0], y[2] - y[0]), __dmul_rn(x[2] - x[0], y[1] - y[0])));
+    double l2 = 0.0;
+    bool ok = bounded && E >= 0.0;
+#pragma unroll
+    for (int i = 0; i < 3; ++i) {
+        const int j = (i + 1) % 3, k = (i + 2) % 3;
+        const double ex = x[j] - x[i], ey = y[j] - y[i];
+        const double len2 = __dadd_rn(__dmul_rn(ex, ex), __dmul_rn(ey, ey));
+        l2 = fmax(l2, len2);
+        const double len = sqrt(len2);
+        double a = ey / len, b = -ex / len;
+        const double side = __dadd_rn(__dmul_rn(a, x[k] - x[i]), __dmul_rn(b, y[k] - y[i]));
+        if (side > 0.0) { a = -a; b = -b; }
+        const float af = (float)a, bf = (float)b;
+        double d = -__builtin_inf();
+#pragma unroll
+        for (int v = 0; v < 3; ++v) d = fmax(d, __dadd_rn(__dmul_rn((double)af, x[v]), __dmul_rn((double)bf, y[v])));
+        const double fa = fabs((double)af), fb = fabs((double)bf);
+        const double m = __dadd_rn(__dmul_rn(fa + fb, E), __dmul_rn(kEdgeFloatSlack, __dadd_rn(__dadd_rn(__dmul_rn(fa, X), __dmul_rn(fb, Y)), fabs(d))));
+        const double cd = -(d + m);
+        const float cf = (float)(cd - __dadd_rn(__dmul_rn(2.4e-7, fabs(cd)), 1e-37));
+        ok = ok && m < kEdgeMaxMargin * (w + h) && fabsf(af) + fabsf(bf) + fabsf(cf) < 3e38f;
+        rec[3 * i] = af; rec[3 * i + 1] = bf; rec[3 * i + 2] = cf;
+    }
+    ok = ok && area2 > kEdgeSliver * l2;
+    if (!ok) {
+#pragma unroll
+        for (uint32_t q = 0; q < kEdgeFloats; ++q) rec[q] = 0.0f;
+    }
+}
+
+__device__ __forceinline__ float edge_value(float a, float b, float c, float x0, float x1, float y0, float y1) {
+    return fminf(a * x0, a * x1) + fminf(b * y0, b * y1) + c;
+}
+__device__ __forceinline__ bool edges_outside(const float* rec, float x0, float x1, float y0, float y1) {
+    const float t0 = edge_value(rec[0], rec[1], rec[2], x0, x1, y0, y1), t1 = edge_value(rec[3], rec[4], rec[5], x0, x1, y0, y1), t2 = edge_value(rec[6], rec[7], rec[8], x0, x1, y0, y1);
+    return t0 > 0.0f || t1 > 0.0f || t2 > 0.0f;
+}
+
+}
+#endif
diff --git a/functracer_amd/csrc/ft_flat.h b/functracer_amd/csrc/ft_flat.h
--- a/functracer_amd/csrc/ft_flat.h
+++ b/functracer_amd/csrc/ft_flat.h
@@ -76,6 +76,7 @@
 constexpr uint32_t kLsMaxPairs = 64;
 constexpr uint32_t kLsMaxTris = 1u << 20;
 constexpr uint64_t kLsMaxBytes = 256ull << 20;
+constexpr uint64_t kLsEdgeMaxBytes = 128ull << 20;
 constexpr uint32_t kLsGridEntriesPerTri = 16;
 constexpr uint32_t kLsGridMaxCell = 256;
 constexpr uint32_t kLsGridWaveCells = 4;
diff --git a/functracer_amd/csrc/ft_frame.cpp b/functracer_amd/csrc/ft_frame.cpp
--- a/functracer_amd/csrc/ft_frame.cpp
+++ b/functracer_amd/csrc/ft_frame.cpp
@@ -310,7 +310,8 @@
     const ftk::Launch Lg{cs, c->n_cu * 8, 0, 0};
     if (!c->classified) FT_HIP(c, hipEventCreateWithFlags(&c->classified, hipEventDisableTiming));
     else FT_HIP(c, hipStreamWaitEvent(cs, c->classified, 0));
-    const ftk::BlockLists lists{F.d_list_heads.as<uint32_t>(), F.d_list_pool.as<uint32_t>(), (uint32_t)(F.d_list_pool.bytes / (ftk::kListEntryWords * 4)), p.list_leaf};
+    const ftk::BlockLists lists{F.d_list_heads.as<uint32_t>(), F.d_list_pool.as<uint32_t>(), (uint32_t)(F.d_list_pool.bytes / (ftk::kListEntryWords * 4)), p.list_leaf,
+                                F.d_list_edges.bytes / (ftk::kEdgeFloats * 4) >= F.d_list_pool.bytes / (ftk::kListEntryWords * 4) ? F.d_list_edges.as<float>() : nullptr};
     auto queue_lists = [&] { if (p.list_leaf >= 0) ftk::launch_block_lists(Lg, c->dev_scene, all, cls.pos_block, lists, p.jitter_extent, fc, kept); };
     if (ahead) {
         ftk::launch_classify(Lg, c->dev_scene, all, cls, p.jitter_extent, epoch, fc, retired, p.mask_only);
@@ -350,7 +351,8 @@
         ftk::Primary gen{p.cam, c->d_pixels.as<uint32_t>(), c->d_jitter.as<double>(), job.id_base, n_pix, p.spp, stride, (unsigned long long)q.seed,
                          1.0 / (double)n_pix, 1.0 / (double)stride, nullptr, nullptr};
         if (p.classify) { gen.counts = kept; gen.block_map = F.d_pos_block.as<uint32_t>(); }
-        if (p.list_leaf >= 0) { gen.list_heads = F.d_list_heads.as<uint32_t>(); gen.list_pool = F.d_list_pool.as<uint32_t>(); gen.list_leaf = p.list_leaf; }
+        if (p.list_leaf >= 0) { gen.list_heads = F.d_list_heads.as<uint32_t>(); gen.list_pool = F.d_list_pool.as<uint32_t>(); gen.list_leaf = p.list_leaf;
+                                 gen.list_edges = c->opt.edge_cull && F.d_list_edges.bytes / (ftk::kEdgeFloats * 4) >= F.d_list_pool.bytes / (ftk::kListEntryWords * 4) ? F.d_list_edges.as<float>() : nullptr; }
         gen.group_log2 = (n_pix % 64u == 0u) ? p.group_log2 : 0;
         const int at = c->acc_turn;
         double* const acc = c->d_acc[at].as<double>();
@@ -423,6 +425,7 @@
         if (p.list_leaf >= 0) {
             if ((rc = ensure(c, F.d_list_heads, n_blocks * 4)) != FT_OK) return rc;
             if ((rc = ensure(c, F.d_list_pool, (16 * n_blocks + 4096) * ftk::kListEntryWords * 4)) != FT_OK) return rc;
+            if ((rc = ensure(c, F.d_list_edges, F.d_list_pool.bytes / (ftk::kListEntryWords * 4) * ftk::kEdgeFloats * 4)) != FT_OK) return rc;
         }
         F.list_leaf = p.list_leaf; F.list_cam = p.cam;
         c->last_classified_slot = turn;
diff --git a/functracer_amd/csrc/ft_kernels.hip b/functracer_amd/csrc/ft_kernels.hip
--- a/functracer_amd/csrc/ft_kernels.hip
+++ b/functracer_amd/csrc/ft_kernels.hip
@@ -9,6 +9,7 @@
 #include <stdint.h>
 
 #include "ft_device.h"
+#include "ft_edges.h"
 #include "ft_filter.h"
 
 using namespace ftd;
@@ -64,6 +65,7 @@
     cdp ls_pairs;
     cup ls_nodes;
     cdp ls_tris;
+    const float* ls_edges;
     const uint8_t* tex_pixels;
     const float* cull_items;
     const float* coarse_boxes;
@@ -80,7 +82,7 @@
     s.program = to_const_as(g.program); s.meshes = to_const_as(reinterpret_cast<const int32_t*>(g.meshes));
     s.nodes = to_const_as(reinterpret_cast<const double*>(g.nodes)); s.bsp_leaves = to_const_as(reinterpret_cast<const uint32_t*>(g.bsp_leaves));
     s.tris = to_const_as(g.tris); s.culls = to_const_as(g.culls); s.tri_orig = to_const_as(g.tri_orig); s.wide = to_const_as(g.wide); s.mesh_wide = to_const_as(g.mesh_wide);
-    s.ls_pairs = to_const_as(g.ls_pairs); s.ls_nodes = to_const_as(g.ls_nodes); s.ls_tris = to_const_as(g.ls_tris);
+    s.ls_pairs = to_const_as(g.ls_pairs); s.ls_nodes = to_const_as(g.ls_nodes); s.ls_tris = to_const_as(g.ls_tris); s.ls_edges = g.ls_edges;
     s.tex_pixels = g.tex_pixels; s.cull_items = g.cull_items; s.coarse_boxes = g.coarse_boxes; s.cull_rows = to_const_as(g.cull_rows); s.item_pc = to_const_as(g.item_pc); s.n_items = g.n_items; s.n_cull_rows = g.n_cull_rows;
     s.n_leaves = g.n_leaves; s.n_lights = g.n_lights; s.csg_cap = g.csg_cap; s.stack_cap = g.stack_cap; s.csg_rows = g.csg_rows; s.lane_fold = g.lane_fold; s.n_simd = g.n_simd;
     return s;
@@ -848,7 +850,11 @@
                 const uint32_t e = base + lane_id();
                 const FT_CONST float* eb = bx + 5u * min(e, count - 1u);
                 const float eu0 = eb[0], eu1 = eb[1], ev0 = eb[2], ev1 = eb[3], ew = eb[4];
-                unsigned long long m = __ballot((e < count) & (eu0 <= u_max) & (eu1 >= u_min) & (ev0 <= v_max) & (ev1 >= v_min) & (ew >= w_min));
+                const bool in_rect = (e < count) & (eu0 <= u_max) & (eu1 >= u_min) & (ev0 <= v_max) & (ev1 >= v_min) & (ew >= w_min);
+                bool outside = false;
+                if (S.ls_edges) outside = edges_outside(S.ls_edges + (size_t)kEdgeFloats * (first + min(e, count - 1u)), u_min, u_max, v_min, v_max);
+                unsigned long long m = __ballot(in_rect && !outside);
+                FT_LIST_ADD(14, __popcll(__ballot(in_rect))); FT_LIST_ADD(15, __popcll(m));
                 while (m) {
                     const int k = (int)__builtin_ctzll(m);
                     m &= m - 1ull;
@@ -869,7 +875,7 @@
     }
 }
 
-struct ListQuery { const uint32_t* pool; uint32_t head; uint32_t leaf; float x0, x1, y0, y1; };
+struct ListQuery { const uint32_t* pool; uint32_t head; uint32_t leaf; float x0, x1, y0, y1; const float* edges; };
 FT_DEV void mesh_list_closest(const Scene& S, const ListQuery& Lq, const Ray& r, Query<false>& q, uint32_t leaf, bool lit) {
     const bool alive = q.active;
     const uint32_t count = Lq.head & 127u, first = Lq.head >> 7;
@@ -878,8 +884,11 @@
     const uint32_t* E = Lq.pool + (size_t)kListEntryWords * (first + min(lane_id(), count - 1u));
     const uint32_t tri_v = E[0], orig_v = E[1];
     const float ex0 = __uint_as_float(E[2]), ex1 = __uint_as_float(E[3]), ey0 = __uint_as_float(E[4]), ey1 = __uint_as_float(E[5]);
-    unsigned long long m = __ballot((lane_id() < count) & (ex0 <= Lq.x1) & (ex1 >= Lq.x0) & (ey0 <= Lq.y1) & (ey1 >= Lq.y0));
-    FT_LIST_ADD(3, __popcll(m));
+    const bool in_rect = (lane_id() < count) & (ex0 <= Lq.x1) & (ex1 >= Lq.x0) & (ey0 <= Lq.y1) & (ey1 >= Lq.y0);
+    bool outside = false;
+    if (Lq.edges) outside = edges_outside(Lq.edges + (size_t)kEdgeFloats * (first + min(lane_id(), count - 1u)), Lq.x0, Lq.x1, Lq.y0, Lq.y1);
+    unsigned long long m = __ballot(in_rect && !outside);
+    FT_LIST_ADD(11, __popcll(__ballot(in_rect))); FT_LIST_ADD(3, __popcll(m));
     double reach = alive ? q.best_t : -__builtin_inf();
     uint32_t best_tri = 0xFFFFFFFFu;
     bool found = false;
@@ -1648,7 +1657,7 @@
             if (active && !empty) ro = offset_ray(primary_ray_from(&Kb->gen, at_of(bi).s, pid, jxy));
             if (MESH && lq.head != kListNone && !empty) {
                 wave_rect(lq, jxy, active);
-                lq.pool = Kb->gen.list_pool; lq.leaf = (uint32_t)Kb->gen.list_leaf;
+                lq.pool = Kb->gen.list_pool; lq.leaf = (uint32_t)Kb->gen.list_leaf; lq.edges = Kb->gen.list_edges;
             }
         }
         Query<false> q = Query<false>::closest(active);
@@ -1772,7 +1781,7 @@
             if (active && !empty) ro = offset_ray(primary_ray_from(&Kb->gen, slot_at(px, bi, lane_id()).s, pid, jxy));
             if (lq.head != kListNone && !empty) {
                 wave_rect(lq, jxy, active);
-                lq.pool = Kb->gen.list_pool;
+                lq.pool = Kb->gen.list_pool; lq.edges = Kb->gen.list_edges;
             }
         }
         Query<false> q = Query<false>::closest(active);
@@ -2176,11 +2185,13 @@
 FT_DEV float round_up(double x) { return (float)(x + (2.4e-7 * fabs(x) + 1e-37)); }
 __global__ __launch_bounds__(kBlock) void k_block_lists(BlockListArgs) {
     __shared__ uint32_t sh_entries[kBlock / 64][kListCap * kListEntryWords];
+    __shared__ float sh_edges[kBlock / 64][kListCap * kEdgeFloats];
     const FT_CONST BlockListArgs* K = kernel_args<BlockListArgs>();
     const Scene S = scene_view(K->S);
     const PrimaryArg g = &K->gen;
     const uint32_t wave = (uint32_t)__builtin_amdgcn_readfirstlane((int)(threadIdx.x / 64u));
     uint32_t* mine = sh_entries[wave];
+    float* mine_edges = sh_edges[wave];
     const uint32_t n_active = to_const_as(K->counts)->n_pix / 64u;
     const uint32_t leaf = (uint32_t)K->out.leaf;
     const LeafHead Hm = leaf_head(S, leaf);
@@ -2237,6 +2248,7 @@
                     const double vx[3] = {T[0], T[0] + T[3], T[0] + T[6]}, vy[3] = {T[1], T[1] + T[4], T[1] + T[7]}, vz[3] = {T[2], T[2] + T[5], T[2] + T[8]};
                     double xl = __builtin_inf(), xh = -__builtin_inf(), yl = __builtin_inf(), yh = -__builtin_inf();
                     bool bounded = true;
+                    double pjx[3], pjy[3], e_max = 0.0;
 #pragma unroll
                     for (int v = 0; v < 3; ++v) {
                         const double px = vx[v] - omx, py = vy[v] - omy, pz = vz[v] - omz;
@@ -2248,6 +2260,7 @@
                         const double jx = b / a, jy = c / a, ex = (eb + fabs(jx) * ea) / am, ey = (ec + fabs(jy) * ea) / am;
                         bounded = bounded && am > 0.0 && fabs(jx) + fabs(jy) + ex + ey < 1e300;
                         xl = fmin(xl, jx - ex); xh = fmax(xh, jx + ex); yl = fmin(yl, jy - ey); yh = fmax(yh, jy + ey);
+                        pjx[v] = jx; pjy[v] = jy; e_max = fmax(e_max, fmax(ex, ey));
                     }
                     const double grow = 1e-3 * ((xh - xl) + (yh - yl));
                     const float inf = __builtin_inff();
@@ -2260,6 +2273,12 @@
                     if (keep) {
                         uint32_t* e = mine + kListEntryWords * (n + lanes_below(km));
                         e[0] = tri; e[1] = S.tri_orig[tri]; e[2] = __float_as_uint(tx0); e[3] = __float_as_uint(tx1); e[4] = __float_as_uint(ty0); e[5] = __float_as_uint(ty1);
+                        if (K->out.edges) {
+                            float rec[kEdgeFloats];
+                            edge_record(pjx, pjy, e_max + grow, bounded, rec);
+                            float* er = mine_edges + kEdgeFloats * (n + lanes_below(km));
+                            for (uint32_t q = 0; q < kEdgeFloats; ++q) er[q] = rec[q];
+                        }
                     }
                     n += n_keep;
                 }
@@ -2275,6 +2294,10 @@
                 __builtin_amdgcn_wave_barrier();
                 uint32_t* dst = K->out.pool + (size_t)kListEntryWords * at;
                 for (uint32_t w = lane_id(); w < kListEntryWords * n; w += 64u) dst[w] = mine[w];
+                if (K->out.edges) {
+                    float* de = K->out.edges + (size_t)kEdgeFloats * at;
+                    for (uint32_t w = lane_id(); w < kEdgeFloats * n; w += 64u) de[w] = mine_edges[w];
+                }
                 head = (at << 7) | n;
             }
         }
diff --git a/functracer_amd/csrc/ft_lightspace.hip b/functracer_amd/csrc/ft_lightspace.hip
--- a/functracer_amd/csrc/ft_lightspace.hip
+++ b/functracer_amd/csrc/ft_lightspace.hip
@@ -5,6 +5,7 @@
 #include <stdint.h>
 
 #include "ft_device.h"
+#include "ft_edges.h"
 
 using namespace ftd;
 
@@ -141,6 +142,43 @@
     }
 }
 
+__global__ __launch_bounds__(256) void k_ls_edges(const double* __restrict__ pair, const uint32_t* __restrict__ nodes, uint32_t node_words,
+                                                  const double* __restrict__ tris, uint32_t n_recs, uint32_t n_cells, float* __restrict__ edges) {
+    const uint32_t cell = blockIdx.x * 4u + (threadIdx.x >> 6), lane = threadIdx.x & 63u;
+    if (cell >= n_cells) return;
+    const uint32_t cells = reinterpret_cast<const uint32_t*>(pair + 14)[1];
+    if ((uint64_t)cells + 4ull * cell + 4ull > node_words) return;
+    const uint32_t* W = nodes + cells + 4ull * cell;
+    const uint32_t first = W[0], box = W[1];
+    uint32_t cnt = W[2];
+    if (cnt > kLsGridMaxCell) cnt = kLsGridMaxCell;
+    if ((uint64_t)first + cnt > n_recs || (uint64_t)box + 5ull * cnt > node_words) return;
+    LsFrame F;
+    for (int q = 0; q < 3; ++q) { F.U[q] = pair[q]; F.V[q] = pair[3 + q]; F.D[q] = pair[6 + q]; F.c[q] = pair[9 + q]; }
+    F.pad = 0.0;
+    for (uint32_t e = lane; e < cnt; e += 64u) {
+        const double* T = tris + 9ull * (first + e);
+        double x[3], y[3];
+        for (int v = 0; v < 3; ++v) {
+            double p[3];
+            for (int q = 0; q < 3; ++q) p[q] = __dadd_rn(__dsub_rn(T[q], F.c[q]), v == 1 ? T[3 + q] : v == 2 ? T[6 + q] : 0.0);
+            x[v] = dot_lr(p, F.U); y[v] = dot_lr(p, F.V);
+        }
+        const float* B = reinterpret_cast<const float*>(nodes + box + 5ull * e);
+        const double xl = fmin(x[0], fmin(x[1], x[2])), xh = fmax(x[0], fmax(x[1], x[2])), yl = fmin(y[0], fmin(y[1], y[2])), yh = fmax(y[0], fmax(y[1], y[2]));
+        const double E = fmax(fmax(xl - (double)B[0], (double)B[1] - xh), fmax(yl - (double)B[2], (double)B[3] - yh));
+        const bool bounded = fabs((double)B[0]) + fabs((double)B[1]) + fabs((double)B[2]) + fabs((double)B[3]) < 3e38;
+        float rec[kEdgeFloats];
+        edge_record(x, y, E, bounded, rec);
+        for (uint32_t q = 0; q < kEdgeFloats; ++q) edges[(size_t)kEdgeFloats * (first + e) + q] = rec[q];
+    }
+}
+
+}
+
+void ls_edge_records(hipStream_t stream, const double* pair, const uint32_t* ls_nodes, uint32_t node_words, const double* ls_tris, uint32_t n_recs, uint32_t n_cells, float* edges) {
+    if (n_cells == 0u) return;
+    hipLaunchKernelGGL(k_ls_edges, dim3((n_cells + 3u) / 4u), dim3(256), 0, stream, pair, ls_nodes, node_words, ls_tris, n_recs, n_cells, edges);
 }
 
 void ls_grid_entries(hipStream_t stream, const double* tris, uint32_t n, const LsFrame& F, float* ebox, uint32_t* ruv) {
diff --git a/include/functracer_hip.h b/include/functracer_hip.h
--- a/include/functracer_hip.h
+++ b/include/functracer_hip.h
@@ -215,6 +215,7 @@
 int32_t ft_debug_mesh_trees(ft_context* ctx, int64_t sizes[12], void* nodes, uint32_t* bsp_leaves, double* tris, uint32_t* tri_orig, uint32_t* tri_src,
                             double* wide, float* coarse_boxes, int32_t* meshes, uint32_t* jobs);
 int32_t ft_debug_block_lists(ft_context* ctx, int64_t sizes[4], double plane[4], uint32_t* heads, uint32_t* pos_block, uint32_t* entries);
+int32_t ft_debug_edge_records(ft_context* ctx, int64_t sizes[2], float* grid_edges, float* list_edges);
 int32_t ft_debug_classify_reuse(ft_context* ctx, int64_t out[4]);
 int32_t ft_debug_primary_kernels(ft_context* ctx, int64_t out[2]);
 int32_t ft_get_kernel_times(ft_context* ctx, double ms[5], int32_t launches[5]);
```
